# xd009642/xd-tts

Measured on AMD Instinct MI355X. Metric: mel-frames/s per GPU, 120-phoneme utterance (Tacotron2 decoder+postnet + 60-iter Griffin-Lim), end-to-end, higher is better.
Workload: dtype f32

## Files before the change

### include/xdtts.h

```cpp
#ifndef XDTTS_H
#define XDTTS_H

#include <stddef.h>
#include <stdint.h>

#ifdef __cplusplus
extern "C" {
#endif

typedef int32_t xdtts_status;
enum {
  XDTTS_OK = 0,
  XDTTS_ERR_BAD_ARG = 1,
  XDTTS_ERR_IO = 2,
  XDTTS_ERR_HIP = 3,
  XDTTS_ERR_OOM = 4,
  XDTTS_ERR_TOO_LONG = 5,
  XDTTS_ERR_NO_DEVICE = 6
};

typedef struct xdtts_tacotron2 xdtts_tacotron2;
typedef struct xdtts_griffinlim xdtts_griffinlim;

typedef struct {
  float gate_threshold;
  int32_t max_steps;
  int32_t fixed_steps;
  int32_t dropout_mode;
  uint32_t dropout_seed;
  int32_t max_chunk;
  uint32_t item_base;
  float fixed_frames_per_id;
  const uint8_t *dropout_masks;
  int32_t dropout_mask_steps;
} xdtts_infer_opts;

void xdtts_infer_opts_default(xdtts_infer_opts *opts);


xdtts_status xdtts_tacotron2_load(const char *dir, int32_t device_id, xdtts_tacotron2 **out);

#define XDTTS_DEVICE_DEFAULT (-1)
int32_t xdtts_default_device(void);

xdtts_status xdtts_model_dir_read(const char *dir, float *blob, size_t n_floats);

xdtts_status xdtts_model_dir_describe(const char *dir, char *buf, size_t cap, size_t *needed);

xdtts_status xdtts_tacotron2_load_synthetic(uint32_t seed, float rec_scale, int32_t device_id,
                                            xdtts_tacotron2 **out);

xdtts_status xdtts_tacotron2_load_blob(const float *blob, size_t n_floats, int32_t device_id,
                                       xdtts_tacotron2 **out);

xdtts_status xdtts_tacotron2_save(const xdtts_tacotron2 *h, const char *dir);

int32_t xdtts_tensor_count(void);
const char *xdtts_tensor_name(int32_t i);
int32_t xdtts_tensor_ndim(int32_t i);
int32_t xdtts_tensor_dim(int32_t i, int32_t d);
size_t xdtts_tensor_offset(int32_t i);
size_t xdtts_tensor_total(void);
xdtts_status xdtts_tacotron2_get_tensor(const xdtts_tacotron2 *h, int32_t i, float *out);

xdtts_status xdtts_tacotron2_infer_ids(xdtts_tacotron2 *h, const int64_t *ids, size_t n,
                                       const size_t *splits, size_t n_splits,
                                       const xdtts_infer_opts *opts, float **mel,
                                       size_t *n_frames);

xdtts_status xdtts_tacotron2_infer_batch(xdtts_tacotron2 *h, const int64_t *ids,
                                         const int32_t *lens, int32_t B, int32_t t_stride,
                                         const xdtts_infer_opts *opts,
                                         const int32_t *fixed_steps_per_item, float **mels,
                                         size_t *n_frames);

xdtts_status xdtts_tacotron2_encoder(xdtts_tacotron2 *h, const int64_t *ids, int32_t T,
                                     float *memory, float *processed_memory);
xdtts_status xdtts_tacotron2_decoder(xdtts_tacotron2 *h, const float *memory,
                                     const float *processed_memory, int32_t T, int32_t n_valid,
                                     const xdtts_infer_opts *opts, float *frames, float *gates,
                                     size_t *n_frames);
xdtts_status xdtts_tacotron2_decoder_step(xdtts_tacotron2 *h, const float *memory, const float *processed_memory,
                                          int32_t T, int32_t n_valid, const xdtts_infer_opts *opts, uint32_t step,
                                          const float *decoder_input, float *attention_hidden,
                                          float *attention_cell, float *decoder_hidden, float *decoder_cell,
                                          float *attention_weights, float *attention_weights_cum,
                                          float *attention_context, float *decoder_output,
                                          float *gate_prediction);

xdtts_status xdtts_tacotron2_decoder_steps(xdtts_tacotron2 *h, int32_t engine, int32_t B, const float *memory,
                                           const float *processed_memory, int32_t T, const int32_t *n_valid,
                                           const xdtts_infer_opts *opts, uint32_t step0, int32_t n_steps,
                                           const float *decoder_input, float *attention_hidden, float *attention_cell,
                                           float *decoder_hidden, float *decoder_cell, float *attention_weights,
                                           float *attention_weights_cum, float *attention_context, float *decoder_output,
                                           float *gate_prediction);

xdtts_status xdtts_tacotron2_engine_state(const xdtts_tacotron2 *h, int32_t *decoder_persistent,
                                          int32_t *encoder_cooperative, int32_t *batched_attention);
xdtts_status xdtts_tacotron2_engine_reset(xdtts_tacotron2 *h);
xdtts_status xdtts_tacotron2_small_batch_engine_state(const xdtts_tacotron2 *h, int32_t *state);

const char *xdtts_build_info(void);

xdtts_status xdtts_edge_floor_us(int32_t device_id, int32_t steps, int32_t T, int32_t tuned, double *us_per_step);

xdtts_status xdtts_tacotron2_postnet(xdtts_tacotron2 *h, const float *frames, int32_t F,
                                     float *mel_out);

xdtts_status xdtts_tacotron2_last_timings(const xdtts_tacotron2 *h, float ms[4], int32_t *steps);

void xdtts_tacotron2_free(xdtts_tacotron2 *h);


xdtts_status xdtts_mel_filter_bank(float sample_rate, size_t n_fft, size_t n_mels, float fmin,
                                   float fmax_or_nan, float *out);

xdtts_status xdtts_griffinlim_new(const float *mel_basis, size_t n_mels, size_t n_bins,
                                  size_t noverlap, float power, size_t iters, float momentum,
                                  int32_t device_id, xdtts_griffinlim **out);

typedef struct {
  int32_t nnls_iters;
  int32_t power_mode;
  int32_t mel_decompress;
  int32_t output_normalise;
  int32_t batch_shape;
  float rms_target;
} xdtts_griffinlim_opts;
void xdtts_griffinlim_opts_default(xdtts_griffinlim_opts *opts);
xdtts_status xdtts_griffinlim_set_opts(xdtts_griffinlim *g, const xdtts_griffinlim_opts *opts);
xdtts_status xdtts_griffinlim_get_opts(const xdtts_griffinlim *g, xdtts_griffinlim_opts *opts);

xdtts_status xdtts_griffinlim_set_seed(xdtts_griffinlim *g, uint32_t seed);

xdtts_status xdtts_griffinlim_infer(xdtts_griffinlim *g, const float *mel, size_t n_mels,
                                    size_t n_frames, float **audio, size_t *n_samples);

xdtts_status xdtts_griffinlim_infer_batch(xdtts_griffinlim *g, const float *const *mels, size_t n_mels,
                                          const size_t *n_frames, int32_t n_utt, float **audios,
                                          size_t *n_samples);

xdtts_status xdtts_griffinlim_infer_linear(xdtts_griffinlim *g, const float *S,
                                           const float *phase0, size_t n_frames, size_t iters,
                                           float **audio, size_t *n_samples);

xdtts_status xdtts_griffinlim_mel_to_linear(xdtts_griffinlim *g, const float *mel,
                                            size_t n_mels, size_t n_frames, float *S_out);

xdtts_status xdtts_griffinlim_step(xdtts_griffinlim *g, const float *S, float *angles,
                                   float *rebuilt, size_t n_frames, size_t n_iter);

xdtts_status xdtts_griffinlim_last_timings(const xdtts_griffinlim *g, float ms[3]);

void xdtts_griffinlim_free(xdtts_griffinlim *g);

xdtts_status xdtts_synthesize_ids(xdtts_tacotron2 *h, xdtts_griffinlim *g, const int64_t *ids,
                                  size_t n, const size_t *splits, size_t n_splits,
                                  const xdtts_infer_opts *opts, float **mel, size_t *n_frames,
                                  float **audio, size_t *n_samples);

xdtts_status xdtts_synthesize_batch(xdtts_tacotron2 *h, xdtts_griffinlim *g, const int64_t *ids,
                                    const int32_t *lens, int32_t B, int32_t t_stride,
                                    const int32_t *utt_chunks, int32_t n_utt,
                                    const xdtts_infer_opts *opts,
                                    const int32_t *fixed_steps_per_item, float **mels,
                                    size_t *n_frames, float **audios, size_t *n_samples);

xdtts_status xdtts_synthesize_sequence(xdtts_tacotron2 *h, xdtts_griffinlim *g, const int64_t *const *ids,
                                       const size_t *n_ids, const size_t *const *splits, const size_t *n_splits,
                                       int32_t n_utt, const xdtts_infer_opts *opts, float **mels,
                                       size_t *n_frames, float **audios, size_t *n_samples);

int32_t xdtts_symbol_count(void);
const char *xdtts_symbol_token(int32_t id);
int64_t xdtts_unit_id(const char *token, int32_t as_character);
int32_t xdtts_split_score(int64_t id);
xdtts_status xdtts_find_splits(const int64_t *ids, size_t n, size_t max_size, size_t *out,
                               size_t cap, size_t *n_out);

#define XDTTS_SAMPLE_RATE 22050
xdtts_status xdtts_audio_to_i16(const float *audio, size_t n, int16_t *pcm);
size_t xdtts_silence_samples(double seconds, uint32_t sample_rate);
size_t xdtts_silence_samples_duration(uint64_t secs, uint32_t nanos, uint32_t sample_rate);
xdtts_status xdtts_wav_write(const char *path, const int16_t *pcm, size_t n, uint32_t sample_rate);
xdtts_status xdtts_npy_write_f32(const char *path, const float *data, size_t rows, size_t cols);
double xdtts_real_time_factor(double compute_seconds, size_t n_samples);

void xdtts_free(void *p);
const char *xdtts_last_error(void);
int32_t xdtts_device_count(void);
xdtts_status xdtts_tacotron2_sync(xdtts_tacotron2 *h);

#ifdef __cplusplus
}
#endif
#endif
```

### xd-tts_amd/__init__.py

```python
import ctypes as C
import os

import numpy as np

_HERE = os.path.dirname(os.path.abspath(__file__))
LIB_PATH = os.environ.get("XDTTS_LIB") or os.path.join(_HERE, "libxdtts_hip.so")

N_MEL = 80
EMB = 512
ATT_DIM = 128

STATUS = {0: "OK", 1: "BAD_ARG", 2: "IO", 3: "HIP", 4: "OOM", 5: "TOO_LONG", 6: "NO_DEVICE"}
XDTTS_ERR_BAD_ARG, XDTTS_ERR_IO, XDTTS_ERR_HIP, XDTTS_ERR_OOM, XDTTS_ERR_TOO_LONG, XDTTS_ERR_NO_DEVICE = 1, 2, 3, 4, 5, 6


class XdttsError(RuntimeError):

    def __init__(self, status, message):
        super().__init__("xdtts status %d (%s): %s" % (status, STATUS.get(status, "?"), message))
        self.status = status


class GriffinLimOpts(C.Structure):

    _fields_ = [("nnls_iters", C.c_int32), ("power_mode", C.c_int32), ("mel_decompress", C.c_int32), ("output_normalise", C.c_int32), ("batch_shape", C.c_int32), ("rms_target", C.c_float)]


class InferOpts(C.Structure):
    _fields_ = [
        ("gate_threshold", C.c_float),
        ("max_steps", C.c_int32),
        ("fixed_steps", C.c_int32),
        ("dropout_mode", C.c_int32),
        ("dropout_seed", C.c_uint32),
        ("max_chunk", C.c_int32),
        ("item_base", C.c_uint32),
        ("fixed_frames_per_id", C.c_float),
        ("dropout_masks", C.c_void_p),
        ("dropout_mask_steps", C.c_int32),
    ]


_VP, _I32, _U32, _SZ, _F = C.c_void_p, C.c_int32, C.c_uint32, C.c_size_t, C.c_float
_PF = C.POINTER(C.c_float)
SYMBOLS = {
    "xdtts_infer_opts_default": (None, [C.POINTER(InferOpts)]),
    "xdtts_tacotron2_load": (_I32, [C.c_char_p, _I32, C.POINTER(_VP)]),
    "xdtts_model_dir_read": (_I32, [C.c_char_p, _VP, _SZ]),
    "xdtts_model_dir_describe": (_I32, [C.c_char_p, C.c_char_p, _SZ, C.POINTER(_SZ)]),
    "xdtts_tacotron2_load_synthetic": (_I32, [_U32, _F, _I32, C.POINTER(_VP)]),
    "xdtts_tacotron2_load_blob": (_I32, [_VP, _SZ, _I32, C.POINTER(_VP)]),
    "xdtts_tacotron2_save": (_I32, [_VP, C.c_char_p]),
    "xdtts_tensor_count": (_I32, []),
    "xdtts_tensor_name": (C.c_char_p, [_I32]),
    "xdtts_tensor_ndim": (_I32, [_I32]),
    "xdtts_tensor_dim": (_I32, [_I32, _I32]),
    "xdtts_tensor_offset": (_SZ, [_I32]),
    "xdtts_tensor_total": (_SZ, []),
    "xdtts_tacotron2_get_tensor": (_I32, [_VP, _I32, _VP]),
    "xdtts_tacotron2_infer_ids": (_I32, [_VP, _VP, _SZ, _VP, _SZ, C.POINTER(InferOpts), C.POINTER(_PF), C.POINTER(_SZ)]),
    "xdtts_tacotron2_infer_batch": (_I32, [_VP, _VP, _VP, _I32, _I32, C.POINTER(InferOpts), _VP, C.POINTER(_PF), C.POINTER(_SZ)]),
    "xdtts_tacotron2_encoder": (_I32, [_VP, _VP, _I32, _VP, _VP]),
    "xdtts_tacotron2_decoder": (_I32, [_VP, _VP, _VP, _I32, _I32, C.POINTER(InferOpts), _VP, _VP, C.POINTER(_SZ)]),
    "xdtts_tacotron2_decoder_step": (_I32, [_VP, _VP, _VP, _I32, _I32, C.POINTER(InferOpts), _U32] + [_VP] * 10),
    "xdtts_tacotron2_decoder_steps": (_I32, [_VP, _I32, _I32, _VP, _VP, _I32, _VP, C.POINTER(InferOpts), _U32, _I32] + [_VP] * 10),
    "xdtts_tacotron2_engine_state": (_I32, [_VP, C.POINTER(_I32), C.POINTER(_I32), C.POINTER(_I32)]),
    "xdtts_tacotron2_small_batch_engine_state": (_I32, [_VP, C.POINTER(_I32)]),
    "xdtts_tacotron2_engine_reset": (_I32, [_VP]),
    "xdtts_tacotron2_postnet": (_I32, [_VP, _VP, _I32, _VP]),
    "xdtts_tacotron2_last_timings": (_I32, [_VP, C.POINTER(C.c_float * 4), C.POINTER(_I32)]),
    "xdtts_tacotron2_free": (None, [_VP]),
    "xdtts_tacotron2_sync": (_I32, [_VP]),
    "xdtts_mel_filter_bank": (_I32, [_F, _SZ, _SZ, _F, _F, _VP]),
    "xdtts_griffinlim_new": (_I32, [_VP, _SZ, _SZ, _SZ, _F, _SZ, _F, _I32, C.POINTER(_VP)]),
    "xdtts_griffinlim_opts_default": (None, [_VP]),
    "xdtts_griffinlim_set_opts": (_I32, [_VP, _VP]),
    "xdtts_griffinlim_get_opts": (_I32, [_VP, _VP]),
    "xdtts_griffinlim_set_seed": (_I32, [_VP, _U32]),
    "xdtts_griffinlim_infer": (_I32, [_VP, _VP, _SZ, _SZ, C.POINTER(_PF), C.POINTER(_SZ)]),
    "xdtts_griffinlim_infer_batch": (_I32, [_VP, _VP, _SZ, _VP, _I32, _VP, _VP]),
    "xdtts_griffinlim_infer_linear": (_I32, [_VP, _VP, _VP, _SZ, _SZ, C.POINTER(_PF), C.POINTER(_SZ)]),
    "xdtts_griffinlim_mel_to_linear": (_I32, [_VP, _VP, _SZ, _SZ, _VP]),
    "xdtts_griffinlim_step": (_I32, [_VP, _VP, _VP, _VP, _SZ, _SZ]),
    "xdtts_griffinlim_last_timings": (_I32, [_VP, C.POINTER(C.c_float * 3)]),
    "xdtts_griffinlim_free": (None, [_VP]),
    "xdtts_synthesize_ids": (_I32, [_VP, _VP, _VP, _SZ, _VP, _SZ, C.POINTER(InferOpts), C.POINTER(_PF), C.POINTER(_SZ), C.POINTER(_PF), C.POINTER(_SZ)]),
    "xdtts_synthesize_batch": (_I32, [_VP, _VP, _VP, _VP, _I32, _I32, _VP, _I32, C.POINTER(InferOpts), _VP, _VP, _VP, _VP, _VP]),
    "xdtts_synthesize_sequence": (_I32, [_VP, _VP, _VP, _VP, _VP, _VP, _I32, C.POINTER(InferOpts), _VP, _VP, _VP, _VP]),
    "xdtts_symbol_count": (_I32, []),
    "xdtts_symbol_token": (C.c_char_p, [_I32]),
    "xdtts_unit_id": (C.c_int64, [C.c_char_p, _I32]),
    "xdtts_split_score": (_I32, [C.c_int64]),
    "xdtts_find_splits": (_I32, [_VP, _SZ, _SZ, _VP, _SZ, C.POINTER(_SZ)]),
    "xdtts_audio_to_i16": (_I32, [_VP, _SZ, _VP]),
    "xdtts_build_info": (C.c_char_p, []),
    "xdtts_edge_floor_us": (_I32, [C.c_int32, C.c_int32, C.c_int32, C.c_int32, C.POINTER(C.c_double)]),
    "xdtts_default_device": (C.c_int32, []),
    "xdtts_silence_samples": (_SZ, [C.c_double, _U32]),
    "xdtts_silence_samples_duration": (_SZ, [C.c_uint64, _U32, _U32]),
    "xdtts_wav_write": (_I32, [C.c_char_p, _VP, _SZ, _U32]),
    "xdtts_npy_write_f32": (_I32, [C.c_char_p, _VP, _SZ, _SZ]),
    "xdtts_real_time_factor": (C.c_double, [C.c_double, _SZ]),
    "xdtts_free": (None, [_VP]),
    "xdtts_last_error": (C.c_char_p, []),
    "xdtts_device_count": (_I32, []),
}


def _share_torch_hip_runtime():
    import importlib.util
    import sys

    if "torch" in sys.modules:
        return
    try:
        spec = importlib.util.find_spec("torch")
    except (ImportError, ValueError):
        spec = None
    if not spec or not spec.origin:
        return
    lib = os.path.join(os.path.dirname(spec.origin), "lib", "libamdhip64.so")
    if os.path.exists(lib):
        try:
            C.CDLL(lib, mode=C.RTLD_GLOBAL)
        except OSError:
            pass


def _load():
    _share_torch_hip_runtime()
    if not os.path.exists(LIB_PATH):
        raise ImportError(
            "%s not found: build it with `make -C %s` (or __graft_entry__.build()); there is no CPU fallback" % (LIB_PATH, _HERE)
        )
    lib = C.CDLL(LIB_PATH)
    for name, (res, args) in SYMBOLS.items():
        fn = getattr(lib, name)
        fn.restype = res
        fn.argtypes = args
    return lib


lib = _load()


def _check(status):
    if status != 0:
        raise XdttsError(status, lib.xdtts_last_error().decode("utf-8", "replace"))


def _ptr(a):
    return a.ctypes.data_as(C.c_void_p)


def default_opts(**kw):
    o = InferOpts()
    lib.xdtts_infer_opts_default(C.byref(o))
    masks = kw.pop("dropout_masks", None)
    for k, v in kw.items():
        setattr(o, k, v)
    if masks is not None:
        m = np.ascontiguousarray(masks, dtype=np.uint8)
        if m.ndim != 4 or m.shape[2:] != (2, 256):
            raise ValueError("dropout_masks must be (chunks, steps, 2, 256)")
        o._masks_keepalive = m
        o.dropout_masks = m.ctypes.data
        o.dropout_mask_steps = m.shape[1]
        o.dropout_mode = 2
    return o


def device_count():
    return lib.xdtts_device_count()


def tensor_table():
    out = []
    for i in range(lib.xdtts_tensor_count()):
        shape = tuple(lib.xdtts_tensor_dim(i, d) for d in range(lib.xdtts_tensor_ndim(i)))
        out.append((lib.xdtts_tensor_name(i).decode(), shape, lib.xdtts_tensor_offset(i)))
    return out


def read_model_dir(path):
    blob = np.empty(lib.xdtts_tensor_total(), dtype=np.float32)
    _check(lib.xdtts_model_dir_read(os.fsencode(path), _ptr(blob), blob.size))
    return {n: blob[off : off + int(np.prod(shape))].reshape(shape) for n, shape, off in tensor_table()}


def describe_model_dir(path):
    need = C.c_size_t()
    _check(lib.xdtts_model_dir_describe(os.fsencode(path), None, 0, C.byref(need)))
    buf = C.create_string_buffer(need.value)
    _check(lib.xdtts_model_dir_describe(os.fsencode(path), buf, need.value, None))
    out = {}
    for line in buf.value.decode().splitlines():
        f, rest = line.split(": inputs ", 1)
        i, o = rest.split(" ; outputs ", 1)
        out[f] = ([x for x in i.split(",") if x], [x for x in o.split(",") if x])
    return out


class _Pinned:

    def __init__(self, addr):
        self.addr = addr

    def __del__(self):
        if self.addr and lib is not None:
            lib.xdtts_free(C.cast(self.addr, _PF))
            self.addr = None


def _take(ptr, n, shape):
    addr = C.cast(ptr, C.c_void_p).value
    if not n or not addr:
        if addr:
            lib.xdtts_free(ptr)
        return np.zeros(shape, dtype=np.float32)
    buf = (C.c_float * int(n)).from_address(addr)
    buf._owner = _Pinned(addr)
    return np.frombuffer(buf, dtype=np.float32).reshape(shape)


def generate_id_list():
    return [lib.xdtts_symbol_token(i).decode() for i in range(lib.xdtts_symbol_count())]


def unit_id(token, as_character=False):
    i = lib.xdtts_unit_id(token.encode(), 1 if as_character else 0)
    return None if i < 0 else int(i)


def units_to_ids(tokens, as_character=False):
    out = [unit_id(t, as_character) for t in tokens]
    return np.array([i for i in out if i is not None], dtype=np.int64)


SAMPLE_RATE = 22050


def build_info():
    return dict(kv.split("=", 1) for kv in lib.xdtts_build_info().decode().split(" ") if "=" in kv)


def source_hash():
    import glob
    import hashlib

    here = os.path.dirname(os.path.abspath(__file__))
    files = sorted(glob.glob(os.path.join(here, "csrc", "*")) + [os.path.join(here, "..", "include", "xdtts.h")],
                   key=lambda p: os.path.relpath(p, here))
    h = hashlib.sha256()
    for f in files:
        with open(f, "rb") as fh:
            h.update(fh.read())
    return h.hexdigest()


DEVICE_DEFAULT = -1


def default_device():
    v = lib.xdtts_default_device()
    if v < 0:
        raise XdttsError(2, lib.xdtts_last_error().decode())
    return int(v)


def edge_floor_us(device_id=0, steps=2000, T=100, tuned=True):
    us = C.c_double()
    _check(lib.xdtts_edge_floor_us(device_id, steps, T, 1 if tuned else 0, C.byref(us)))
    return us.value


def audio_to_i16(audio):
    a = np.ascontiguousarray(audio, dtype=np.float32).ravel()
    out = np.empty(a.size, dtype=np.int16)
    _check(lib.xdtts_audio_to_i16(_ptr(a), a.size, _ptr(out)))
    return out


def silence_samples(seconds, sample_rate=SAMPLE_RATE):
    return int(lib.xdtts_silence_samples(float(seconds), int(sample_rate)))


def silence_samples_duration(secs, nanos, sample_rate=SAMPLE_RATE):
    return int(lib.xdtts_silence_samples_duration(int(secs), int(nanos), int(sample_rate)))


def write_wav(path, audio, sample_rate=SAMPLE_RATE):
    pcm = np.ascontiguousarray(audio) if np.asarray(audio).dtype == np.int16 else audio_to_i16(audio)
    _check(lib.xdtts_wav_write(os.fsencode(path), _ptr(pcm), pcm.size, int(sample_rate)))


def write_mel_npy(path, mel):
    m = np.ascontiguousarray(mel, dtype=np.float32)
    _check(lib.xdtts_npy_write_f32(os.fsencode(path), _ptr(m), m.shape[0], m.shape[1]))


def real_time_factor(compute_seconds, n_samples):
    return float(lib.xdtts_real_time_factor(float(compute_seconds), int(n_samples)))


def find_splits(ids, max_size=100):
    ids = np.ascontiguousarray(ids, dtype=np.int64)
    out = np.empty(max(ids.size, 1) + 2, dtype=np.uintp)
    n = C.c_size_t()
    _check(lib.xdtts_find_splits(_ptr(ids), ids.size, max_size, _ptr(out), out.size, C.byref(n)))
    return out[: n.value].astype(np.int64)


class Tacotron2:

    def __init__(self, handle):
        self._h = handle

    @classmethod
    def load(cls, path, device_id=0):
        h = C.c_void_p()
        _check(lib.xdtts_tacotron2_load(os.fsencode(path), device_id, C.byref(h)))
        return cls(h)

    @classmethod
    def synthetic(cls, seed=20240327, rec_scale=1.0, device_id=0):
        h = C.c_void_p()
        _check(lib.xdtts_tacotron2_load_synthetic(seed, rec_scale, device_id, C.byref(h)))
        return cls(h)

    @classmethod
    def from_blob(cls, blob, device_id=0):
        blob = np.ascontiguousarray(blob, dtype=np.float32)
        h = C.c_void_p()
        _check(lib.xdtts_tacotron2_load_blob(_ptr(blob), blob.size, device_id, C.byref(h)))
        return cls(h)

    def close(self):
        if self._h:
            lib.xdtts_tacotron2_free(self._h)
            self._h = None

    def __del__(self):
        try:
            self.close()
        except Exception:
            pass

    def save(self, path):
        _check(lib.xdtts_tacotron2_save(self._h, os.fsencode(path)))

    def blob(self):
        out = np.zeros(lib.xdtts_tensor_total(), dtype=np.float32)
        for i, (_n, shape, off) in enumerate(tensor_table()):
            t = np.empty(shape, dtype=np.float32)
            _check(lib.xdtts_tacotron2_get_tensor(self._h, i, _ptr(t)))
            out[off : off + t.size] = t.ravel()
        return out

    def get_tensor(self, name):
        for i, (n, shape, _off) in enumerate(tensor_table()):
            if n == name:
                out = np.empty(shape, dtype=np.float32)
                _check(lib.xdtts_tacotron2_get_tensor(self._h, i, _ptr(out)))
                return out
        raise KeyError(name)

    def infer(self, ids, splits=None, opts=None):
        ids = np.ascontiguousarray(ids, dtype=np.int64)
        sp = None if splits is None else np.ascontiguousarray(splits, dtype=np.uintp)
        mel, nf = _PF(), C.c_size_t()
        _check(
            lib.xdtts_tacotron2_infer_ids(
                self._h, _ptr(ids), ids.size, None if sp is None else _ptr(sp), 0 if sp is None else sp.size, C.byref(opts) if opts else None, C.byref(mel), C.byref(nf)
            )
        )
        return _take(mel, N_MEL * nf.value, (N_MEL, nf.value))

    def infer_units(self, tokens, opts=None, as_character=False):
        ids = units_to_ids(tokens, as_character)
        window = opts.max_chunk if opts else 100
        return self.infer(ids, splits=find_splits(ids, window), opts=opts)

    def infer_batch(self, ids_list, opts=None, fixed_steps=None):
        B = len(ids_list)
        lens = np.array([len(x) for x in ids_list], dtype=np.int32)
        stride = int(lens.max()) if B else 1
        ids = np.zeros((B, stride), dtype=np.int64)
        for b, x in enumerate(ids_list):
            ids[b, : len(x)] = x
        fs = None if fixed_steps is None else np.ascontiguousarray(fixed_steps, dtype=np.int32)
        mels = (_PF * B)()
        nf = (C.c_size_t * B)()
        _check(lib.xdtts_tacotron2_infer_batch(self._h, _ptr(ids), _ptr(lens), B, stride, C.byref(opts) if opts else None, None if fs is None else _ptr(fs), mels, nf))
        return [_take(mels[b], N_MEL * nf[b], (N_MEL, nf[b])) for b in range(B)]

    def encoder(self, ids):
        ids = np.ascontiguousarray(ids, dtype=np.int64)
        T = ids.size
        memory = np.empty((T, EMB), dtype=np.float32)
        pmem = np.empty((T, ATT_DIM), dtype=np.float32)
        _check(lib.xdtts_tacotron2_encoder(self._h, _ptr(ids), T, _ptr(memory), _ptr(pmem)))
        return memory, pmem

    def decoder(self, memory, pmem, n_valid, opts=None):
        memory = np.ascontiguousarray(memory, dtype=np.float32)
        pmem = np.ascontiguousarray(pmem, dtype=np.float32)
        o = opts if opts else default_opts()
        frames = np.empty((o.max_steps, N_MEL), dtype=np.float32)
        gates = np.empty(o.max_steps, dtype=np.float32)
        nf = C.c_size_t()
        _check(lib.xdtts_tacotron2_decoder(self._h, _ptr(memory), _ptr(pmem), memory.shape[0], n_valid, C.byref(o), _ptr(frames), _ptr(gates), C.byref(nf)))
        return frames[: nf.value].copy(), gates[: nf.value].copy()

    def decoder_step(self, memory, pmem, n_valid, state, decoder_input, step, opts=None):
        memory = np.ascontiguousarray(memory, dtype=np.float32)
        pmem = np.ascontiguousarray(pmem, dtype=np.float32)
        names = ("attention_hidden", "attention_cell", "decoder_hidden", "decoder_cell", "attention_weights", "attention_weights_cum", "attention_context")
        st = {k: np.array(state[k], dtype=np.float32, order="C") for k in names}
        din = np.ascontiguousarray(decoder_input, dtype=np.float32)
        out, gate = np.empty(N_MEL, dtype=np.float32), np.empty(1, dtype=np.float32)
        _check(lib.xdtts_tacotron2_decoder_step(self._h, _ptr(memory), _ptr(pmem), memory.shape[0], n_valid, C.byref(opts) if opts else None, step,
                                                _ptr(din), *[_ptr(st[k]) for k in names], _ptr(out), _ptr(gate)))
        return out, float(gate[0]), st

    ENGINES = {"launch": 0, "persistent": 1, "batched": 2, "persistent8": 3}

    def decoder_steps(self, engine, memory, pmem, n_valid, states, decoder_input, step0, n_steps=1, opts=None):
        memory = np.ascontiguousarray(memory, dtype=np.float32)
        pmem = np.ascontiguousarray(pmem, dtype=np.float32)
        B, T = memory.shape[0], memory.shape[1]
        nv = np.ascontiguousarray(n_valid, dtype=np.int32)
        names = ("attention_hidden", "attention_cell", "decoder_hidden", "decoder_cell", "attention_weights", "attention_weights_cum", "attention_context")
        st = {k: np.array(states[k], dtype=np.float32, order="C") for k in names}
        din = np.ascontiguousarray(decoder_input, dtype=np.float32)
        out, gate = np.empty((B, n_steps, N_MEL), dtype=np.float32), np.empty((B, n_steps), dtype=np.float32)
        _check(lib.xdtts_tacotron2_decoder_steps(self._h, self.ENGINES[engine], B, _ptr(memory), _ptr(pmem), T, _ptr(nv), C.byref(opts) if opts else None,
                                                 step0, n_steps, _ptr(din), *[_ptr(st[k]) for k in names], _ptr(out), _ptr(gate)))
        return out, gate, st

    def engine_state(self):
        a, b, c = C.c_int32(), C.c_int32(), C.c_int32()
        _check(lib.xdtts_tacotron2_engine_state(self._h, C.byref(a), C.byref(b), C.byref(c)))
        e = C.c_int32()
        _check(lib.xdtts_tacotron2_small_batch_engine_state(self._h, C.byref(e)))
        return {"decoder_persistent": a.value, "encoder_cooperative": b.value, "batched_attention": c.value, "decoder_persistent8": e.value}

    def engine_reset(self):
        _check(lib.xdtts_tacotron2_engine_reset(self._h))

    def postnet(self, frames):
        frames = np.ascontiguousarray(frames, dtype=np.float32)
        F = frames.shape[0]
        out = np.empty((N_MEL, F), dtype=np.float32)
        _check(lib.xdtts_tacotron2_postnet(self._h, _ptr(frames), F, _ptr(out)))
        return out

    def last_timings(self):
        ms = (C.c_float * 4)()
        steps = C.c_int32()
        _check(lib.xdtts_tacotron2_last_timings(self._h, C.byref(ms), C.byref(steps)))
        return {"encoder_ms": ms[0], "decoder_ms": ms[1], "postnet_ms": ms[2], "total_ms": ms[3], "steps": steps.value}


def create_mel_filter_bank(sample_rate, n_fft, n_mels, fmin, fmax=None):
    out = np.empty((n_mels, n_fft // 2 + 1), dtype=np.float32)
    _check(lib.xdtts_mel_filter_bank(sample_rate, n_fft, n_mels, fmin, float("nan") if fmax is None else fmax, _ptr(out)))
    return out


class GriffinLim:

    def __init__(self, mel_basis, noverlap, power, iters, momentum, device_id=0, seed=0):
        basis = np.ascontiguousarray(mel_basis, dtype=np.float32)
        self._h = C.c_void_p()
        _check(lib.xdtts_griffinlim_new(_ptr(basis), basis.shape[0], basis.shape[1], noverlap, power, iters, momentum, device_id, C.byref(self._h)))
        self.n_bins = basis.shape[1]
        self.set_seed(seed)

    def set_seed(self, seed):
        _check(lib.xdtts_griffinlim_set_seed(self._h, seed))

    def set_opts(self, **kw):
        o = self.get_opts()
        for k, v in kw.items():
            setattr(o, k, v)
        _check(lib.xdtts_griffinlim_set_opts(self._h, C.byref(o)))

    def get_opts(self):
        o = GriffinLimOpts()
        _check(lib.xdtts_griffinlim_get_opts(self._h, C.byref(o)))
        return o

    def close(self):
        if self._h:
            lib.xdtts_griffinlim_free(self._h)
            self._h = None

    def __del__(self):
        try:
            self.close()
        except Exception:
            pass

    def infer(self, mel):
        mel = np.ascontiguousarray(mel, dtype=np.float32)
        audio, n = _PF(), C.c_size_t()
        _check(lib.xdtts_griffinlim_infer(self._h, _ptr(mel), mel.shape[0], mel.shape[1], C.byref(audio), C.byref(n)))
        return _take(audio, n.value, (n.value,))

    def infer_batch(self, mels):
        ms = [np.ascontiguousarray(m, dtype=np.float32) for m in mels]
        n = len(ms)
        ptrs = (C.c_void_p * n)(*[m.ctypes.data for m in ms])
        nf = (C.c_size_t * n)(*[m.shape[1] for m in ms])
        audios = (_PF * n)()
        ns = (C.c_size_t * n)()
        _check(lib.xdtts_griffinlim_infer_batch(self._h, ptrs, ms[0].shape[0], nf, n, audios, ns))
        return [_take(audios[u], ns[u], (ns[u],)) for u in range(n)]

    def infer_linear(self, S, phase0=None, iters=0):
        S = np.ascontiguousarray(S, dtype=np.float32)
        p0 = None if phase0 is None else np.ascontiguousarray(phase0, dtype=np.float32)
        audio, n = _PF(), C.c_size_t()
        _check(lib.xdtts_griffinlim_infer_linear(self._h, _ptr(S), None if p0 is None else _ptr(p0), S.shape[1], iters, C.byref(audio), C.byref(n)))
        return _take(audio, n.value, (n.value,))

    def step(self, S, angles, rebuilt, n_iter=1):
        S = np.ascontiguousarray(S, dtype=np.float32)
        a = np.array(angles, dtype=np.float32, order="C")
        r = np.array(rebuilt, dtype=np.float32, order="C")
        _check(lib.xdtts_griffinlim_step(self._h, _ptr(S), _ptr(a), _ptr(r), S.shape[1], n_iter))
        return a, r

    def mel_to_linear(self, mel):
        mel = np.ascontiguousarray(mel, dtype=np.float32)
        S = np.empty((self.n_bins, mel.shape[1]), dtype=np.float32)
        _check(lib.xdtts_griffinlim_mel_to_linear(self._h, _ptr(mel), mel.shape[0], mel.shape[1], _ptr(S)))
        return S

    def last_timings(self):
        ms = (C.c_float * 3)()
        _check(lib.xdtts_griffinlim_last_timings(self._h, C.byref(ms)))
        return {"mel_to_linear_ms": ms[0], "iterations_ms": ms[1], "total_ms": ms[2]}


def create_griffin_lim(device_id=0, iters=30, seed=0):
    mel_basis = create_mel_filter_bank(22050.0, 1024, 80, 0.0, 8000.0)
    return GriffinLim(mel_basis, 1024 - 256, 1.7, iters, 0.99, device_id=device_id, seed=seed)


def synthesize(tacotron2, vocoder, ids, splits=None, opts=None):
    ids = np.ascontiguousarray(ids, dtype=np.int64)
    sp = None if splits is None else np.ascontiguousarray(splits, dtype=np.uintp)
    mel, nf, audio, ns = _PF(), C.c_size_t(), _PF(), C.c_size_t()
    _check(
        lib.xdtts_synthesize_ids(
            tacotron2._h, vocoder._h, _ptr(ids), ids.size, None if sp is None else _ptr(sp), 0 if sp is None else sp.size, C.byref(opts) if opts else None, C.byref(mel), C.byref(nf), C.byref(audio), C.byref(ns)
        )
    )
    return _take(mel, N_MEL * nf.value, (N_MEL, nf.value)), _take(audio, ns.value, (ns.value,))


def synthesize_batch(tacotron2, vocoder, utterance_chunks, opts=None, fixed_steps=None, want_mels=True):
    chunks = [c for u in utterance_chunks for c in u]
    B, n_utt = len(chunks), len(utterance_chunks)
    lens = np.array([len(x) for x in chunks], dtype=np.int32)
    stride = int(lens.max()) if B else 1
    ids = np.zeros((B, stride), dtype=np.int64)
    for b, x in enumerate(chunks):
        ids[b, : len(x)] = x
    uc = np.array([len(u) for u in utterance_chunks], dtype=np.int32)
    fs = None if fixed_steps is None else np.ascontiguousarray([s for u in fixed_steps for s in u], dtype=np.int32)
    mels = (_PF * n_utt)() if want_mels else None
    audios = (_PF * n_utt)()
    nf, ns = (C.c_size_t * n_utt)(), (C.c_size_t * n_utt)()
    _check(
        lib.xdtts_synthesize_batch(
            tacotron2._h, vocoder._h, _ptr(ids), _ptr(lens), B, stride, _ptr(uc), n_utt, C.byref(opts) if opts else None, None if fs is None else _ptr(fs), mels, nf, audios, ns
        )
    )
    out_m = [_take(mels[u], N_MEL * nf[u], (N_MEL, nf[u])) for u in range(n_utt)] if want_mels else None
    return out_m, [_take(audios[u], ns[u], (ns[u],)) for u in range(n_utt)]


def synthesize_sequence(tacotron2, vocoder, ids_list, splits_list=None, opts=None, want_mels=True):
    n = len(ids_list)
    idv = [np.ascontiguousarray(x, dtype=np.int64) for x in ids_list]
    spv = [None if (splits_list is None or splits_list[u] is None) else np.ascontiguousarray(splits_list[u], dtype=np.uintp) for u in range(n)]
    ids_p = (C.c_void_p * n)(*[x.ctypes.data for x in idv])
    n_ids = (C.c_size_t * n)(*[x.size for x in idv])
    sp_p = (C.c_void_p * n)(*[(None if s is None else s.ctypes.data) for s in spv])
    n_sp = (C.c_size_t * n)(*[(0 if s is None else s.size) for s in spv])
    mels = (_PF * n)() if want_mels else None
    audios = (_PF * n)()
    nf, ns = (C.c_size_t * n)(), (C.c_size_t * n)()
    _check(lib.xdtts_synthesize_sequence(tacotron2._h, vocoder._h, ids_p, n_ids, sp_p, n_sp, n, C.byref(opts) if opts else None, mels, nf, audios, ns))
    out_m = [_take(mels[u], N_MEL * nf[u], (N_MEL, nf[u])) for u in range(n)] if want_mels else None
    return out_m, [_take(audios[u], ns[u], (ns[u],)) for u in range(n)]
```

### xd-tts_amd/csrc/api_tacotron2.cpp

```cpp
#include <algorithm>
#include <cmath>
#include <memory>

#include "tacotron2_handle.h"

#include "edge_floor.hip"

using namespace xdtts;

extern "C" {

void xdtts_infer_opts_default(xdtts_infer_opts *o) {
  if (!o) return;
  o->gate_threshold = 0.6f;
  o->max_steps = 1000;
  o->fixed_steps = 0;
  o->dropout_mode = 1;
  o->dropout_seed = 0;
  o->max_chunk = 100;
  o->item_base = 0;
  o->fixed_frames_per_id = 0.f;
  o->dropout_masks = nullptr;
  o->dropout_mask_steps = 0;
}

const char *xdtts_last_error(void) { return last_error(); }

int32_t xdtts_device_count(void) {
  int n = 0;
  if (hipGetDeviceCount(&n) != hipSuccess) return 0;
  return n;
}

void xdtts_free(void *p) {
  if (p) pinned_release(p);
}

int32_t xdtts_tensor_count(void) { return (int32_t)tensor_table().size(); }
const char *xdtts_tensor_name(int32_t i) {
  return i >= 0 && i < xdtts_tensor_count() ? tensor_table()[i].name : nullptr;
}
int32_t xdtts_tensor_ndim(int32_t i) { return i >= 0 && i < xdtts_tensor_count() ? tensor_table()[i].ndim : 0; }
int32_t xdtts_tensor_dim(int32_t i, int32_t d) {
  return i >= 0 && i < xdtts_tensor_count() && d >= 0 && d < 3 ? tensor_table()[i].dims[d] : 0;
}
size_t xdtts_tensor_offset(int32_t i) { return i >= 0 && i < xdtts_tensor_count() ? tensor_table()[i].offset : 0; }
size_t xdtts_tensor_total(void) { return tensor_total(); }

static xdtts_status make_handle(std::vector<float> &&blob, int32_t device_id, xdtts_tacotron2 **out) {
  return guard([&] {
    if (!out) fail(XDTTS_ERR_BAD_ARG, "out handle pointer is null");
    *out = nullptr;
    auto h = std::make_unique<xdtts_tacotron2>();
    h->blob = std::move(blob);
    h->init(device_id);
    *out = h.release();
  });
}

xdtts_status xdtts_tacotron2_load(const char *dir, int32_t device_id, xdtts_tacotron2 **out) {
  std::vector<float> blob;
  xdtts_status st = guard([&] {
    if (!dir) fail(XDTTS_ERR_BAD_ARG, "dir is null");
    device_id = select_device(device_id);
    load_model_dir(dir, blob);
  });
  if (st != XDTTS_OK) return st;
  return make_handle(std::move(blob), device_id, out);
}

int32_t xdtts_default_device(void) {
  int32_t v = 0;
  return guard([&] { v = default_device(); }) == XDTTS_OK ? v : -1;
}

xdtts_status xdtts_model_dir_read(const char *dir, float *blob, size_t n_floats) {
  return guard([&] {
    if (!dir || !blob) fail(XDTTS_ERR_BAD_ARG, "null argument");
    if (n_floats != tensor_total()) fail(XDTTS_ERR_BAD_ARG, "blob has %zu floats, expected %zu", n_floats, tensor_total());
    std::vector<float> v;
    load_model_dir(dir, v);
    std::memcpy(blob, v.data(), v.size() * sizeof(float));
  });
}

xdtts_status xdtts_model_dir_describe(const char *dir, char *buf, size_t cap, size_t *needed) {
  return guard([&] {
    if (!dir || (!buf && cap)) fail(XDTTS_ERR_BAD_ARG, "null argument");
    const std::string d = describe_onnx_dir(dir);
    if (needed) *needed = d.size() + 1;
    if (cap) {
      const size_t n = std::min(cap - 1, d.size());
      std::memcpy(buf, d.data(), n);
      buf[n] = 0;
    }
  });
}

xdtts_status xdtts_tacotron2_load_synthetic(uint32_t seed, float rec_scale, int32_t device_id,
                                            xdtts_tacotron2 **out) {
  std::vector<float> blob;
  xdtts_status st = guard([&] {
    device_id = select_device(device_id);
    synthetic_blob(seed, rec_scale, blob);
  });
  if (st != XDTTS_OK) return st;
  return make_handle(std::move(blob), device_id, out);
}

xdtts_status xdtts_tacotron2_load_blob(const float *blob, size_t n_floats, int32_t device_id,
                                       xdtts_tacotron2 **out) {
  std::vector<float> v;
  xdtts_status st = guard([&] {
    if (!blob) fail(XDTTS_ERR_BAD_ARG, "blob is null");
    if (n_floats != tensor_total()) fail(XDTTS_ERR_BAD_ARG, "blob has %zu floats, expected %zu", n_floats, tensor_total());
    device_id = select_device(device_id);
    v.assign(blob, blob + n_floats);
  });
  if (st != XDTTS_OK) return st;
  return make_handle(std::move(v), device_id, out);
}

xdtts_status xdtts_tacotron2_save(const xdtts_tacotron2 *h, const char *dir) {
  return guard([&] {
    if (!h || !dir) fail(XDTTS_ERR_BAD_ARG, "null argument");
    save_container(dir, h->blob);
  });
}

xdtts_status xdtts_tacotron2_get_tensor(const xdtts_tacotron2 *h, int32_t i, float *out) {
  return guard([&] {
    if (!h || !out || i < 0 || i >= xdtts_tensor_count()) fail(XDTTS_ERR_BAD_ARG, "bad tensor request");
    const TensorInfo &t = tensor_table()[i];
    std::memcpy(out, h->blob.data() + t.offset, t.numel * sizeof(float));
  });
}

void xdtts_tacotron2_free(xdtts_tacotron2 *h) {
  if (!h) return;
  (void)hipSetDevice(h->device);
  if (h->stream) (void)hipStreamSynchronize(h->stream);
  delete h;
}

xdtts_status xdtts_tacotron2_sync(xdtts_tacotron2 *h) {
  return guard([&] {
    if (!h) fail(XDTTS_ERR_BAD_ARG, "null handle");
    HIP_CHECK(hipStreamSynchronize(h->stream));
  });
}

xdtts_status xdtts_tacotron2_infer_ids(xdtts_tacotron2 *h, const int64_t *ids, size_t n, const size_t *splits,
                                       size_t n_splits, const xdtts_infer_opts *opts, float **mel,
                                       size_t *n_frames) {
  return guard([&] {
    if (!h || !mel || !n_frames) fail(XDTTS_ERR_BAD_ARG, "null argument");
    *mel = nullptr;
    *n_frames = 0;
    std::lock_guard<std::mutex> lk(h->mu);
    const xdtts_infer_opts o = resolve_opts(opts);
    std::vector<int64_t> padded;
    std::vector<int> lens;
    chunks_from_splits(ids, n, splits, n_splits, o.max_chunk, padded, lens);
    int total = 0;
    h->infer_batch_device(padded.data(), lens.data(), (int)lens.size(), o.max_chunk, o, nullptr, &total);
    PinnedGuard host((size_t)N_MEL * total);
    HIP_CHECK(hipMemcpyAsync(host.p, h->mel_dev.p, (size_t)N_MEL * total * sizeof(float), hipMemcpyDeviceToHost, h->stream));
    h->finish_timings();
    *mel = host.release();
    *n_frames = (size_t)total;
  });
}

xdtts_status xdtts_tacotron2_infer_batch(xdtts_tacotron2 *h, const int64_t *ids, const int32_t *lens, int32_t B,
                                         int32_t t_stride, const xdtts_infer_opts *opts,
                                         const int32_t *fixed_steps_per_item, float **mels, size_t *n_frames) {
  return guard([&] {
    if (!h || !ids || !lens || !mels || !n_frames) fail(XDTTS_ERR_BAD_ARG, "null argument");
    std::lock_guard<std::mutex> lk(h->mu);
    const xdtts_infer_opts o = resolve_opts(opts);
    if (B <= 0) fail(XDTTS_ERR_BAD_ARG, "batch %d out of range", B);
    for (int b = 0; b < B; ++b) mels[b] = nullptr;
    const int T = o.max_chunk;
    if (t_stride <= 0) fail(XDTTS_ERR_BAD_ARG, "t_stride must be positive");
    const std::vector<int64_t> padded = pad_batch_ids(ids, lens, B, t_stride, T);
    int total = 0;
    std::vector<int> F = h->infer_batch_device(padded.data(), lens, B, T, o, fixed_steps_per_item, &total, true);
    PinnedSlab slab((size_t)N_MEL * total);
    Drain drain(h->stream);
    HIP_CHECK(hipMemcpyAsync(slab.base, h->mel_dev.p, (size_t)N_MEL * total * sizeof(float), hipMemcpyDeviceToHost, h->stream));
    h->finish_timings();
    size_t off = 0;
    for (int b = 0; b < B; ++b) {
      mels[b] = slab.piece(off);
      n_frames[b] = (size_t)F[b];
      off += (size_t)N_MEL * F[b];
    }
    slab.hand_over();
  });
}

xdtts_status xdtts_tacotron2_encoder(xdtts_tacotron2 *h, const int64_t *ids, int32_t T, float *memory,
                                     float *processed_memory) {
  return guard([&] {
    if (!h || !ids || !memory || !processed_memory) fail(XDTTS_ERR_BAD_ARG, "null argument");
    if (T <= 0 || T > T_MAX) fail(XDTTS_ERR_BAD_ARG, "T %d out of range", T);
    for (int t = 0; t < T; ++t)
      if (ids[t] < 0 || ids[t] >= N_SYMBOLS) fail(XDTTS_ERR_BAD_ARG, "id out of range");
    std::lock_guard<std::mutex> lk(h->mu);
    HIP_CHECK(hipSetDevice(h->device));
    h->ids.upload(ids, T, h->stream);
    std::lock_guard<ChipLock> chip(chip_mutex(h->device));
    h->run_encoder(1, T);
    HIP_CHECK(hipMemcpyAsync(memory, h->memory.p, (size_t)T * EMB * sizeof(float), hipMemcpyDeviceToHost, h->stream));
    HIP_CHECK(hipMemcpyAsync(processed_memory, h->pmem.p, (size_t)T * ATT_DIM * sizeof(float), hipMemcpyDeviceToHost, h->stream));
    HIP_CHECK(hipStreamSynchronize(h->stream));
    h->check_encoder_exchange();
  });
}

xdtts_status xdtts_tacotron2_decoder(xdtts_tacotron2 *h, const float *memory, const float *processed_memory,
                                     int32_t T, int32_t n_valid, const xdtts_infer_opts *opts, float *frames,
                                     float *gates, size_t *n_frames) {
  return guard([&] {
    if (!h || !memory || !processed_memory || !frames || !n_frames) fail(XDTTS_ERR_BAD_ARG, "null argument");
    if (T <= 0 || T > T_MAX || n_valid <= 0 || n_valid > T) fail(XDTTS_ERR_BAD_ARG, "bad T/n_valid");
    std::lock_guard<std::mutex> lk(h->mu);
    HIP_CHECK(hipSetDevice(h->device));
    const xdtts_infer_opts o = resolve_opts(opts);
    h->memory.upload(memory, (size_t)T * EMB, h->stream);
    h->pmem.upload(processed_memory, (size_t)T * ATT_DIM, h->stream);
    int nv = n_valid;
    h->n_valid.upload(&nv, 1, h->stream);
    HIP_CHECK(hipStreamSynchronize(h->stream));
    std::vector<int> lim(1, std::min(o.fixed_steps > 0 ? o.fixed_steps : o.max_steps, o.max_steps));
    h->upload_dropout_masks(o, 1, lim.data());
    DecoderBufs d = h->decoder_bufs(1, T, h->memory.p, h->pmem.p, o);
    HIP_CHECK(hipEventRecord(h->ev.e[0], h->stream));
    HIP_CHECK(hipEventRecord(h->ev.e[1], h->stream));
    h->last_steps = h->run_decoder(d, lim);
    HIP_CHECK(hipEventRecord(h->ev.e[2], h->stream));
    HIP_CHECK(hipEventRecord(h->ev.e[3], h->stream));
    const int F = h->host_ctl[xdtts_tacotron2::HOST_NF];
    HIP_CHECK(hipMemcpyAsync(frames, d.frames, (size_t)F * N_MEL * sizeof(float), hipMemcpyDeviceToHost, h->stream));
    if (gates) HIP_CHECK(hipMemcpyAsync(gates, d.gates, (size_t)F * sizeof(float), hipMemcpyDeviceToHost, h->stream));
    h->finish_timings();
    *n_frames = (size_t)F;
  });
}

xdtts_status xdtts_tacotron2_decoder_steps(xdtts_tacotron2 *h, int32_t engine, int32_t B, const float *memory, const float *processed_memory,
                                           int32_t T, const int32_t *n_valid, const xdtts_infer_opts *opts, uint32_t step0, int32_t n_steps,
                                           const float *decoder_input, float *attention_hidden, float *attention_cell, float *decoder_hidden,
                                           float *decoder_cell, float *attention_weights, float *attention_weights_cum, float *attention_context,
                                           float *decoder_output, float *gate_prediction) {
  return guard([&] {
    if (!h || !memory || !processed_memory || !n_valid || !decoder_input || !attention_hidden || !attention_cell || !decoder_hidden ||
        !decoder_cell || !attention_weights || !attention_weights_cum || !attention_context || !decoder_output || !gate_prediction)
      fail(XDTTS_ERR_BAD_ARG, "null argument");
    if (engine < 0 || engine > 3)
      fail(XDTTS_ERR_BAD_ARG, "engine %d out of range (0 launch-per-stage, 1 persistent, 2 batched MFMA, 3 persistent MFMA)", engine);
    if (engine == 3 && (B > P8_B_MAX || T > PERSIST_T_MAX))
      fail(XDTTS_ERR_BAD_ARG, "the persistent MFMA engine takes at most %d chunks of at most %d encoder steps", P8_B_MAX, PERSIST_T_MAX);
    if (B <= 0 || B > 64) fail(XDTTS_ERR_BAD_ARG, "batch %d out of range (1..64)", B);
    if (T <= 0 || T > T_MAX) fail(XDTTS_ERR_BAD_ARG, "T %d out of range", T);
    if (n_steps <= 0 || n_steps > 100000 || (uint64_t)step0 + (uint64_t)n_steps > (1u << 30)) fail(XDTTS_ERR_BAD_ARG, "bad step range");
    for (int b = 0; b < B; ++b)
      if (n_valid[b] <= 0 || n_valid[b] > T) fail(XDTTS_ERR_BAD_ARG, "chunk %d: bad n_valid %d", b, n_valid[b]);
    if (engine == 1 && (B > PERSIST_B_MAX || T > PERSIST_T_MAX))
      fail(XDTTS_ERR_BAD_ARG, "the persistent engine takes at most %d chunks of at most %d encoder steps", PERSIST_B_MAX, PERSIST_T_MAX);
    if (engine == 1) {
      for (int b = 0; b < B; ++b)
        for (int j = 0; j < EMB; ++j) {
          double c = 0;
          for (int t = 0; t < T; ++t) c += (double)attention_weights[(size_t)b * T + t] * memory[((size_t)b * T + t) * EMB + j];
          if (std::fabs(c - attention_context[(size_t)b * EMB + j]) > 1e-4 + 1e-4 * std::fabs(c))
            fail(XDTTS_ERR_BAD_ARG, "engine 1 needs attention_context = attention_weights . memory (chunk %d, column %d: %g vs %g)", b, j,
                 (double)attention_context[(size_t)b * EMB + j], c);
        }
    }
    std::lock_guard<std::mutex> lk(h->mu);
    HIP_CHECK(hipSetDevice(h->device));
    xdtts_infer_opts o = resolve_opts(opts);
    const int end = (int)step0 + n_steps;
    o.max_steps = end + 1;
    hipStream_t st = h->stream;
    h->memory.upload(memory, (size_t)B * T * EMB, st);
    h->pmem.upload(processed_memory, (size_t)B * T * ATT_DIM, st);
    h->n_valid.upload(n_valid, B, st);
    std::vector<int> lim((size_t)B, end);
    h->upload_dropout_masks(o, B, lim.data());
    if (engine == 2) h->w.ensure_batched_layout(h->blob, st);
    DecoderBufs d = h->decoder_bufs(B, T, h->memory.p, h->pmem.p, o, engine == 2 ? 1 : 0);
    d.use_gate = 0;
    h->limits.upload(lim.data(), lim.size(), st);
    h->lim_on_dev = lim;
    launch_decoder_init(d, h->limits.p, st);
    h->dec_in_dev.upload(decoder_input, (size_t)B * N_MEL, st);
    const size_t nh = (size_t)B * ATT_RNN, nt = (size_t)B * T, nc = (size_t)B * EMB;
    h->state_stage.alloc(4 * nh + 2 * nt + nc);
    float *s_ah = h->state_stage.p, *s_ac = s_ah + nh, *s_dh = s_ac + nh, *s_dc = s_dh + nh, *s_aw = s_dc + nh, *s_awc = s_aw + nt, *s_ctx = s_awc + nt;
    auto up = [&](float *dst, const float *src, size_t n) { HIP_CHECK(hipMemcpyAsync(dst, src, n * sizeof(float), hipMemcpyHostToDevice, st)); };
    auto dd = [&](float *dst, const float *src, size_t n) { HIP_CHECK(hipMemcpyAsync(dst, src, n * sizeof(float), hipMemcpyDeviceToDevice, st)); };
    up(s_ah, attention_hidden, nh);
    up(s_ac, attention_cell, nh);
    up(s_dh, decoder_hidden, nh);
    up(s_dc, decoder_cell, nh);
    up(s_aw, attention_weights, nt);
    up(s_awc, attention_weights_cum, nt);
    up(s_ctx, attention_context, nc);
    const int s0 = (int)step0;
    HIP_CHECK(hipMemcpyAsync(d.ctl, &s0, sizeof(int), hipMemcpyHostToDevice, st));
    HIP_CHECK(hipStreamSynchronize(st));
    dd(d.aw, s_aw, nt);
    dd(d.awc, s_awc, nt);
    dd(d.ctx, s_ctx, nc);
    if (engine == 2) {
      launch_frag_convert(s_ah, d.att_hf[0], B, d.Bpad, ATT_RNN, 0, st);
      launch_frag_convert(s_dh, d.dec_hf[0], B, d.Bpad, DEC_RNN, 0, st);
      launch_frag_convert(s_ac, d.att_c, B, d.Bpad, ATT_RNN, 0, st);
      launch_frag_convert(s_dc, d.dec_c, B, d.Bpad, DEC_RNN, 0, st);
      launch_frag_convert(s_ctx, d.ctxf, B, d.Bpad, EMB, 0, st);
    } else {
      dd(d.att_h[0], s_ah, nh);
      dd(d.att_c, s_ac, nh);
      dd(d.dec_h[0], s_dh, nh);
      dd(d.dec_c, s_dc, nh);
    }
    d.dec_in = h->dec_in_dev.p;
    int fin = 0;
    if (engine == 1) {
      if (!decoder_persistent_supported(h->device, PERSIST_B_MAX, PERSIST_T_MAX))
        fail(XDTTS_ERR_HIP, "persistent engine not available on this device (its 256-workgroup grid cannot be co-resident)");
      std::lock_guard<ChipLock> chip(chip_mutex(h->device));
      launch_decoder_prenet(d, h->w, st);
      d.dec_in = nullptr;
      h->dec_exchange.alloc(persist_granule_words(B));
      PersistBufs g = persist_bufs(h->dec_exchange.p, h->dec_err.p, B);
      launch_persist_seed_at(d, g, h->limits.p, s0, st);
      try {
        launch_decoder_persistent(d, h->w, g, n_steps, st);
      } catch (const CoopRefused &) {
        (void)hipStreamSynchronize(st);
        fail(XDTTS_ERR_HIP, "persistent engine not available on this device (cooperative launch refused)");
      }
      if (fetch_and_clear_error_word(h->dec_err.p, st)) fail(XDTTS_ERR_HIP, "persistent decoder exchange timed out (grid not co-resident)");
    } else if (engine == 3) {
      if (!decoder_p8_supported(h->device, B, PERSIST_T_MAX))
        fail(XDTTS_ERR_HIP, "persistent MFMA engine not available on this device (its 256-workgroup grid cannot be co-resident)");
      std::lock_guard<ChipLock> chip(chip_mutex(h->device));
      launch_decoder_prenet(d, h->w, st);
      d.dec_in = nullptr;
      h->dec_exchange.alloc(p8_exchange_words(B, n_steps));
      P8Bufs g = p8_bufs(h->dec_exchange.p, h->dec_err.p, B, n_steps);
      launch_p8_seed_at(d, g, h->limits.p, s0, st);
      try {
        launch_decoder_p8(d, h->w, g, n_steps, st);
      } catch (const CoopRefused &) {
        (void)hipStreamSynchronize(st);
        fail(XDTTS_ERR_HIP, "persistent MFMA engine not available on this device (cooperative launch refused)");
      }
      if (fetch_and_clear_error_word(h->dec_err.p, st)) fail(XDTTS_ERR_HIP, "persistent MFMA decoder exchange timed out (grid not co-resident)");
    } else {
      std::unique_lock<ChipLock> chip;
      if (d.hg) chip = std::unique_lock<ChipLock>(chip_mutex(h->device));
      if (engine == 0) launch_decoder_location(d, h->w, st);
      launch_decoder_early(d, h->w, 0, st);
      launch_decoder_prologue(d, h->w, st);
      for (int i = 0; i < n_steps; ++i) {
        launch_decoder_step_at(d, h->w, i, st);
        d.dec_in = nullptr;
      }
      launch_decoder_advance(d, n_steps, st);
      launch_decoder_flush(d, h->w, st);
      fin = n_steps & 1;
      if (d.ep_g && fetch_and_clear_error_word(h->dec_err.p, st)) fail(XDTTS_ERR_HIP, "batched attention exchange timed out (grid not co-resident)");
    }
    if (engine == 2) {
      launch_frag_convert(s_ah, d.att_hf[fin], B, d.Bpad, ATT_RNN, 1, st);
      launch_frag_convert(s_dh, d.dec_hf[fin], B, d.Bpad, DEC_RNN, 1, st);
      launch_frag_convert(s_ac, d.att_c, B, d.Bpad, ATT_RNN, 1, st);
      launch_frag_convert(s_dc, d.dec_c, B, d.Bpad, DEC_RNN, 1, st);
    }
    auto down = [&](float *dst, const float *src, size_t n) { HIP_CHECK(hipMemcpyAsync(dst, src, n * sizeof(float), hipMemcpyDeviceToHost, st)); };
    down(attention_hidden, engine == 2 ? s_ah : d.att_h[fin], nh);
    down(attention_cell, engine == 2 ? s_ac : d.att_c, nh);
    down(decoder_hidden, engine == 2 ? s_dh : d.dec_h[fin], nh);
    down(decoder_cell, engine == 2 ? s_dc : d.dec_c, nh);
    down(attention_weights, d.aw, nt);
    down(attention_weights_cum, engine == 2 && (n_steps & 1) ? d.awc2 : d.awc, nt);
    down(attention_context, d.ctx, nc);
    for (int b = 0; b < B; ++b) {
      down(decoder_output + (size_t)b * n_steps * N_MEL, d.frames + ((size_t)b * d.max_steps + step0) * N_MEL, (size_t)n_steps * N_MEL);
      down(gate_prediction + (size_t)b * n_steps, d.gates + (size_t)b * d.max_steps + step0, (size_t)n_steps);
    }
    HIP_CHECK(hipStreamSynchronize(st));
  });
}

xdtts_status xdtts_tacotron2_decoder_step(xdtts_tacotron2 *h, const float *memory, const float *processed_memory, int32_t T,
                                          int32_t n_valid, const xdtts_infer_opts *opts, uint32_t step, const float *decoder_input,
                                          float *attention_hidden, float *attention_cell, float *decoder_hidden, float *decoder_cell,
                                          float *attention_weights, float *attention_weights_cum, float *attention_context,
                                          float *decoder_output, float *gate_prediction) {
  return xdtts_tacotron2_decoder_steps(h, 0, 1, memory, processed_memory, T, &n_valid, opts, step, 1, decoder_input, attention_hidden,
                                       attention_cell, decoder_hidden, decoder_cell, attention_weights, attention_weights_cum,
                                       attention_context, decoder_output, gate_prediction);
}

xdtts_status xdtts_tacotron2_engine_state(const xdtts_tacotron2 *h, int32_t *decoder_persistent, int32_t *encoder_cooperative,
                                          int32_t *batched_attention) {
  return guard([&] {
    if (!h) fail(XDTTS_ERR_BAD_ARG, "null handle");
    std::lock_guard<std::mutex> lk(h->mu);
    if (decoder_persistent) *decoder_persistent = h->pair_gate.abi_state();
    if (encoder_cooperative) *encoder_cooperative = h->enc_gate.state != EngineGate::OFF ? 1 : 0;
    if (batched_attention) *batched_attention = h->att_fused();
  });
}

xdtts_status xdtts_tacotron2_small_batch_engine_state(const xdtts_tacotron2 *h, int32_t *state) {
  return guard([&] {
    if (!h || !state) fail(XDTTS_ERR_BAD_ARG, "null argument");
    std::lock_guard<std::mutex> lk(h->mu);
    *state = h->p8_gate.abi_state();
  });
}

xdtts_status xdtts_tacotron2_engine_reset(xdtts_tacotron2 *h) {
  return guard([&] {
    if (!h) fail(XDTTS_ERR_BAD_ARG, "null handle");
    std::lock_guard<std::mutex> lk(h->mu);
    h->pair_gate.reset();
    h->p8_gate.reset();
    h->enc_gate.reset();
    h->att_gate.reset();
    h->att_form = env::int_or(env::ATT_FUSED, 2);
  });
}

xdtts_status xdtts_edge_floor_us(int32_t device_id, int32_t steps, int32_t T, int32_t tuned, double *us_per_step) {
  return guard([&] {
    if (!us_per_step || steps < 1 || steps > 1000000 || T < 1 || T > 128) fail(XDTTS_ERR_BAD_ARG, "bad argument");
    device_id = select_device(device_id);
    std::lock_guard<ChipLock> chip(chip_mutex(device_id));
    const double us = xdtts_edge_floor::measure(device_id, steps, T, xdtts_edge_floor::kernel_delays(tuned ? 1 : 0), 5, false);
    if (us < 0) fail(XDTTS_ERR_HIP, "edge-floor skeleton: grid not co-resident on this device, or an exchange failed");
    *us_per_step = us;
  });
}

xdtts_status xdtts_tacotron2_postnet(xdtts_tacotron2 *h, const float *frames, int32_t F, float *mel_out) {
  return guard([&] {
    if (!h || !frames || !mel_out || F <= 0) fail(XDTTS_ERR_BAD_ARG, "bad argument");
    std::lock_guard<std::mutex> lk(h->mu);
    HIP_CHECK(hipSetDevice(h->device));
    h->frames.upload(frames, (size_t)F * N_MEL, h->stream);
    HIP_CHECK(hipStreamSynchronize(h->stream));
    h->mel_dev.alloc((size_t)N_MEL * F);
    const long zero = 0;
    h->run_postnet(h->frames.p, 0, &F, &zero, 1, h->mel_dev.p, F);
    HIP_CHECK(hipMemcpyAsync(mel_out, h->mel_dev.p, (size_t)N_MEL * F * sizeof(float), hipMemcpyDeviceToHost, h->stream));
    HIP_CHECK(hipStreamSynchronize(h->stream));
  });
}

xdtts_status xdtts_tacotron2_last_timings(const xdtts_tacotron2 *h, float ms[4], int32_t *steps) {
  return guard([&] {
    if (!h || !ms) fail(XDTTS_ERR_BAD_ARG, "null argument");
    for (int i = 0; i < 4; ++i) ms[i] = h->last_ms[i];
    if (steps) *steps = h->last_steps;
  });
}

}
```

### xd-tts_amd/csrc/decoder_persistent.hip

```cpp
#include <type_traits>

#include "device_utils.h"
#include "kernels.h"

namespace xdtts {

namespace {

typedef unsigned long long u64;

constexpr int PT = 512;
constexpr int NW = PT / 64;
constexpr int P_NCU = ATT_RNN / 4;
constexpr int TP = PERSIST_T_MAX;
constexpr int ATTN_CU = 8, PRE_CU = 16;
constexpr int EP_LD = TP, MEL_GL = 96;
#ifndef XDTTS_MEL_ST
#define XDTTS_MEL_ST 1
#endif
constexpr int MEL_ST = XDTTS_MEL_ST;
constexpr int GS = PERSIST_B_MAX;
constexpr unsigned P_SPIN_LIMIT = 1u << 21;
constexpr unsigned ACT_BIT = 0x80000000u;
constexpr int PERSIST_LAZY_DEFAULT = 9;

constexpr int WPAD = TP + 32;
static_assert(ATT_RNN == DEC_RNN && P_NCU == 256, "one workgroup per 4 + 4 hidden units");

__device__ __forceinline__ void publish(u64 *slot, unsigned tag, float v) {
  __hip_atomic_store(slot, ((u64)tag << 32) | (u64)__float_as_uint(v), __ATOMIC_RELAXED, __HIP_MEMORY_SCOPE_AGENT);
}
__device__ __forceinline__ u64 peek(const u64 *slot) {
  return __hip_atomic_load(slot, __ATOMIC_RELAXED, __HIP_MEMORY_SCOPE_AGENT);
}
struct PollCtl {
  int *err;
  unsigned limit;
};
__device__ __forceinline__ bool give_up(unsigned &spins, const PollCtl &pc) {
  if (++spins > pc.limit || ((spins & 127u) == 0 && __hip_atomic_load(pc.err, __ATOMIC_RELAXED, __HIP_MEMORY_SCOPE_AGENT))) {
    atomicExch(pc.err, 1);
    return true;
  }
  __builtin_amdgcn_s_sleep(1);
  return false;
}
template <int N, bool PRE = false>
__device__ __forceinline__ unsigned gather(const u64 *base, unsigned idx, unsigned stride, unsigned want,
                                           const bool (&need)[N], float (&out)[N], unsigned (&tag)[N], const PollCtl &err,
                                           const u64 *pre = nullptr) {
  bool done[N];
#pragma unroll
  for (int i = 0; i < N; ++i) {
    done[i] = !need[i];
    out[i] = 0.f;
    tag[i] = 0u;
  }
  if (PRE) {
    bool all = true;
#pragma unroll
    for (int i = 0; i < N; ++i)
      if (!done[i]) {
        const unsigned t = (unsigned)(pre[i] >> 32);
        if ((t & ~ACT_BIT) == want) {
          out[i] = __uint_as_float((unsigned)pre[i]);
          tag[i] = t;
          done[i] = true;
        } else {
          all = false;
        }
      }
    if (all) return 0u;
  }
  unsigned spins = 0;
  for (;;) {
    u64 v[N];
#pragma unroll
    for (int i = 0; i < N; ++i)
      if (!done[i]) v[i] = peek(base + (idx + (unsigned)i * stride));
    bool all = true;
#pragma unroll
    for (int i = 0; i < N; ++i)
      if (!done[i]) {
        const unsigned t = (unsigned)(v[i] >> 32);
        if ((t & ~ACT_BIT) == want) {
          out[i] = __uint_as_float((unsigned)v[i]);
          tag[i] = t;
          done[i] = true;
        } else {
          all = false;
        }
      }
    if (all || give_up(spins, err)) return spins;
  }
}

__device__ __forceinline__ void lazy_wait(int n) {
  for (int i = 0; i < n; ++i) __builtin_amdgcn_s_sleep(4);
}
__device__ __forceinline__ void straggle(bool me, int s, int at) {
  if (me && s % 6 == at)
    for (int i = 0; i < 2; ++i) __builtin_amdgcn_s_sleep(127);
}
__device__ __forceinline__ float4 lds4(const float *p) { return *reinterpret_cast<const float4 *>(p); }
__device__ __forceinline__ void chunk_fence() { asm volatile("" ::: "memory"); }
__device__ __forceinline__ unsigned opaque(unsigned v) {
  asm volatile("" : "+v"(v));
  return v;
}

constexpr int persist_lds_floats(int pb) {
  const int common = pb * (PRENET + TP + ATT_RNN + DEC_RNN + 16) + 8 + 32 + 16 * pb;
  const int attn = 2 * TP * 16 + 2 * TP + 16 + NW * 64 + 2 * WPAD + 62 * 16 + 64 + 16 + 8 * PT * 4;
  const int pre = N_MEL * PRENET + MEL_GL + 2 * PRENET + 8 + 6 * PT * 4;
  return common + (attn > pre ? attn : pre);
}

#ifdef XDTTS_PERSIST_PROFILE
#define PROF_MARK(i)                                       \
  do {                                                     \
    if (tid == 0) {                                        \
      const u64 now_ = wall_clock64();                     \
      s_prof[i] += now_ - prof_last;                       \
      prof_last = now_;                                    \
    }                                                      \
  } while (0)
#define PROF_POLLS(e, n)                                                   \
  do {                                                                     \
    const float m_ = wave_max((float)(n));                                 \
    if ((tid & 63) == 0) atomicAdd(&s_prof[16 + (e)], (u64)m_);            \
  } while (0)
#define PROF_WHEN(e)                                       \
  do {                                                     \
    if (tid == 0) s_prof[20 + (e)] += wall_clock64();      \
  } while (0)
#else
#define PROF_MARK(i) do { } while (0)
#define PROF_POLLS(e, n) do { (void)(n); } while (0)
#define PROF_WHEN(e) do { } while (0)
#endif

struct PersistWeights {
  const float4 *att_w, *dec_w, *q_w, *proj_w;
  const float *att_b, *dec_b, *v_w, *loc_fused, *proj_b, *pre0T, *pre1T;
};

template <int PB, bool SKEW = false, bool GATE = false>
__global__ __launch_bounds__(PT) void k_decoder_persistent(DecoderBufs d, PersistBufs g, PersistWeights w, int nsteps) {
  __shared__ __attribute__((aligned(16))) float smem[persist_lds_floats(PB)];
  const int c = blockIdx.x, tid = threadIdx.x, lane = tid & 63, wave = tid >> 6;
  const int T = d.T;
  const PollCtl pc{g.err, g.spins > 0 ? (unsigned)g.spins : P_SPIN_LIMIT};
  if (g.fault && c == g.fault - 1) return;
  const unsigned L4 = opaque(4u * (unsigned)lane);
  float *s_x = smem;
  float *s_e = s_x + PB * PRENET;
  float *s_hatt = s_e + PB * TP;
  float *s_hdec = s_hatt + PB * ATT_RNN;
  float *s_g = s_hdec + PB * DEC_RNN;
  int *s_act = reinterpret_cast<int *>(s_g + PB * 16);
  float *s_bias = s_g + PB * 16 + 8;
  float *s_cell = s_bias + 32;
  float *role = s_cell + 16 * PB;
  float *s_pm = role;
  float *s_loc = s_pm + TP * 16;
  float *s_aw = s_loc + TP * 16;
  float *s_awc = s_aw + TP;
  float *s_q = s_awc + TP;
  float *s_part = s_q + 16;
  float *s_wpad = s_part + NW * 64;
  float *s_G = s_wpad + 2 * WPAD;
  float *s_cown = s_G + 62 * 16;
  float *s_vv = s_cown + 64;
  float *s_qw = s_vv + 16;
  float *s_W0 = role;
  float *s_mel = s_W0 + N_MEL * PRENET;
  float *s_l1 = s_mel + MEL_GL;
  float *s_pb = s_l1 + 2 * PRENET;
  float *s_pw = s_pb + 8;

  float4 wa[2][ATT_COLS / 256], wd[2][DEC_COLS / 256];
#pragma unroll
  for (int r = 0; r < 2; ++r) {
    const int row = 16 * c + wave + NW * r;
#pragma unroll
    for (int k = 0; k < ATT_COLS / 256; ++k) wa[r][k] = ld_stream(w.att_w + (size_t)row * (ATT_COLS / 4) + lane + 64 * k);
#pragma unroll
    for (int k = 0; k < DEC_COLS / 256; ++k) wd[r][k] = ld_stream(w.dec_w + (size_t)row * (DEC_COLS / 4) + lane + 64 * k);
    if (lane == 0) {
      s_bias[wave + NW * r] = w.att_b[row];
      s_bias[16 + wave + NW * r] = w.dec_b[row];
    }
  }
  const bool attn = c < ATTN_CU * PB, pre = !attn && c < (ATTN_CU + PRE_CU) * PB;
  const int rb = attn ? c / ATTN_CU : (pre ? (c - ATTN_CU * PB) / PRE_CU : 0);
  const int rk = attn ? c % ATTN_CU : (c - ATTN_CU * PB) % PRE_CU;
  const int prow = rk + 16 * wave;
  const bool prow_ok = pre && wave < 6 && prow <= N_MEL;

  const int step0 = d.ctl[0];
  if (GATE && PB == 1 && !(step0 < d.nframes[0])) return;
  if (tid < PB) {
    s_act[tid] = 0;
    s_act[2 + tid] = step0 < d.nframes[tid];
  }
#pragma unroll
  for (int b = 0; b < PB; ++b) {
#pragma unroll
    for (int h = 0; h < 2; ++h) {
      s_hatt[b * ATT_RNN + tid + PT * h] = d.att_h[0][b * ATT_RNN + tid + PT * h];
      s_hdec[b * DEC_RNN + tid + PT * h] = d.dec_h[0][b * DEC_RNN + tid + PT * h];
    }
  }
  float wreg[PB][2];
  int nv[PB];
#pragma unroll
  for (int b = 0; b < PB; ++b) {
    wreg[b][0] = lane < T ? d.aw[b * T + lane] : 0.f;
    wreg[b][1] = lane + 64 < T ? d.aw[b * T + lane + 64] : 0.f;
    nv[b] = d.n_valid[b];
  }
  const int cb = tid >> 2, cu = tid & 3;
  const bool cell = tid < 4 * PB;
  if (cell) {
    s_cell[tid] = d.att_c[cb * ATT_RNN + 4 * c + cu];
    s_cell[4 * PB + tid] = d.dec_c[cb * DEC_RNN + 4 * c + cu];
    s_cell[8 * PB + tid] = d.att_h[0][cb * ATT_RNN + 4 * c + cu];
    s_cell[12 * PB + tid] = d.dec_h[0][cb * DEC_RNN + 4 * c + cu];
  }
  int nf_r = 0;
  if (attn) {
    for (int i = tid; i < TP * 16; i += PT) {
      const int t = i >> 4, dd = i & 15;
      s_pm[i] = t < T ? d.pmem[((size_t)rb * T + t) * ATT_DIM + 16 * rk + dd] : 0.f;
    }
    if (tid < TP) {
      s_aw[tid] = tid < T ? d.aw[rb * T + tid] : 0.f;
      s_awc[tid] = tid < T ? d.awc[rb * T + tid] : 0.f;
    }
    for (int i = tid; i < 62 * 16; i += PT) s_G[i] = w.loc_fused[(size_t)(i >> 4) * ATT_DIM + 16 * rk + (i & 15)];
    if (tid < 16) s_vv[tid] = w.v_w[16 * rk + tid];
#pragma unroll
    for (int r = 0; r < 2; ++r)
#pragma unroll
      for (int j = 0; j < 4; ++j)
        *reinterpret_cast<float4 *>(s_qw + 4 * ((4 * r + j) * PT + tid)) = w.q_w[(unsigned)((16 * rk + wave + NW * r) * (ATT_RNN / 4) + lane + 64 * j)];
  }
  if (pre) {
    for (int i = tid; i < N_MEL * PRENET; i += PT) s_W0[(((i / PRENET) >> 2) * PRENET + i % PRENET) * 4 + ((i / PRENET) & 3)] = w.pre0T[i];
    if (prow_ok) {
      if (lane == 0) s_pb[wave] = w.proj_b[prow];
#pragma unroll
      for (int j = 0; j < 6; ++j)
        *reinterpret_cast<float4 *>(s_pw + 4 * (j * PT + tid)) = w.proj_w[(unsigned)(prow * (PROJ_IN / 4) + lane + 64 * j)];
    }
    nf_r = d.nframes[rb];
  }
  constexpr bool ROLE_REGS = PB == 1;
  float rw[ROLE_REGS ? 40 : 1];
  if (ROLE_REGS) {
#pragma unroll
    for (int k = 0; k < 40; ++k) rw[ROLE_REGS ? k : 0] = 0.f;
    if (attn) {
#pragma unroll
      for (int r = 0; r < 2; ++r)
#pragma unroll
        for (int j = 0; j < 4; ++j) {
          const float4 q = w.q_w[(unsigned)((16 * rk + wave + NW * r) * (ATT_RNN / 4) + lane + 64 * j)];
          rw[ROLE_REGS ? 16 * r + 4 * j + 0 : 0] = q.x;
          rw[ROLE_REGS ? 16 * r + 4 * j + 1 : 0] = q.y;
          rw[ROLE_REGS ? 16 * r + 4 * j + 2 : 0] = q.z;
          rw[ROLE_REGS ? 16 * r + 4 * j + 3 : 0] = q.w;
        }
    } else if (pre) {
#pragma unroll
      for (int k = 0; k < N_MEL / 2; ++k) rw[ROLE_REGS ? k : 0] = w.pre0T[(unsigned)(((tid >> 8) * (N_MEL / 2) + k) * PRENET + (tid & 255))];
    }
  }
  float w1r[2][4];
#pragma unroll
  for (int r = 0; r < 2; ++r)
#pragma unroll
    for (int k = 0; k < 4; ++k) w1r[r][k] = pre ? w.pre1T[(unsigned)((lane + 64 * k) * PRENET + 16 * rk + wave + NW * r)] : 0.f;
  const uint32_t item = d.item_base + (uint32_t)rb;
  __syncthreads();

  float pma[PB][2][2], pmd[PB][2][2], pmp[2] = {0.f, 0.f};
  if (d.ctx_fold) {
#pragma unroll
    for (int b = 0; b < PB; ++b)
#pragma unroll
      for (int h = 0; h < 2; ++h) {
        const int t = lane + 64 * h;
        const float *F = d.ctx_fold + (size_t)b * CTXF_ROWS * CTXF_LD + t;
#pragma unroll
        for (int r = 0; r < 2; ++r) {
          const int row = 16 * c + wave + NW * r;
          pma[b][r][h] = t < T ? F[(size_t)row * CTXF_LD] : 0.f;
          pmd[b][r][h] = t < T ? F[(size_t)(4 * ATT_RNN + row) * CTXF_LD] : 0.f;
        }
        if (prow_ok && b == rb) pmp[h] = t < T ? F[(size_t)(4 * ATT_RNN + 4 * DEC_RNN + prow) * CTXF_LD] : 0.f;
      }
  } else {
    float4 pw4 = make_float4(0.f, 0.f, 0.f, 0.f), pw5 = pw4;
    if (prow_ok) {
      pw4 = lds4(s_pw + 4 * (4 * PT + tid));
      pw5 = lds4(s_pw + 4 * (5 * PT + tid));
    }
#pragma unroll
    for (int b = 0; b < PB; ++b) {
      const float4 *m4 = reinterpret_cast<const float4 *>(d.memory + (size_t)b * T * EMB);
#pragma unroll
      for (int h = 0; h < 2; ++h) {
        float ra[2] = {0.f, 0.f}, rd[2] = {0.f, 0.f}, rp = 0.f;
        for (int tt = 0; tt < 64 && tt + 64 * h < T; ++tt) {
          const int t = tt + 64 * h;
          const float4 m0 = m4[(size_t)t * (EMB / 4) + lane], m1 = m4[(size_t)t * (EMB / 4) + 64 + lane];
#pragma unroll
          for (int r = 0; r < 2; ++r) {
            const float va = wave_sum(dot4(wa[r][2], m1, dot4(wa[r][1], m0, 0.f)));
            const float vd = wave_sum(dot4(wd[r][5], m1, dot4(wd[r][4], m0, 0.f)));
            if (lane == tt) {
              ra[r] = va;
              rd[r] = vd;
            }
          }
          if (pre && b == rb) {
            const float vp = wave_sum(dot4(pw5, m1, dot4(pw4, m0, 0.f)));
            if (lane == tt) rp = vp;
          }
        }
#pragma unroll
        for (int r = 0; r < 2; ++r) {
          pma[b][r][h] = ra[r];
          pmd[b][r][h] = rd[r];
        }
        if (pre && b == rb) pmp[h] = rp;
      }
    }
  }

  float aacc[PB][2], dacc[PB][2];
  auto att_bulk = [&](unsigned L4, bool all) {
#pragma unroll
    for (int b = 0; b < PB; ++b) {
      if (!all && !s_act[b]) continue;
      const float w0 = wreg[b][0], w1 = wreg[b][1];
      float a0 = fmaf(pma[b][0][1], w1, pma[b][0][0] * w0), a1 = fmaf(pma[b][1][1], w1, pma[b][1][0] * w0);
#pragma unroll
      for (int k = 3; k < 7; ++k) {
        const float4 v = lds4(s_hatt + b * ATT_RNN + 256 * (k - 3) + L4);
        a0 = dot4(wa[0][k], v, a0);
        a1 = dot4(wa[1][k], v, a1);
      }
      aacc[b][0] = a0;
      aacc[b][1] = a1;
      chunk_fence();
    }
  };
  auto dec_bulk_h = [&](unsigned L4, bool all) {
#pragma unroll
    for (int b = 0; b < PB; ++b) {
      if (!all && !s_act[b]) continue;
      float a0 = 0.f, a1 = 0.f;
#pragma unroll
      for (int k = 6; k < 10; ++k) {
        const float4 v = lds4(s_hdec + b * DEC_RNN + 256 * (k - 6) + L4);
        a0 = dot4(wd[0][k], v, a0);
        a1 = dot4(wd[1][k], v, a1);
      }
      dacc[b][0] = a0;
      dacc[b][1] = a1;
      chunk_fence();
    }
  };
  auto location = [&](int tid) {
    typedef float f32x4 __attribute__((ext_vector_type(4)));
    for (int i = tid; i < 2 * WPAD; i += PT) {
      const int ch = i / WPAD, t = i % WPAD - (LOC_K - 1) / 2;
      s_wpad[i] = (t >= 0 && t < T) ? (ch ? s_awc[t] : s_aw[t]) : 0.f;
    }
    __syncthreads();
    {
      const unsigned l = (unsigned)tid & 63u, li = l & 15u, lg = l >> 4, t0 = 16u * ((unsigned)tid >> 6);
      float av[16], bv[16];
#pragma unroll
      for (int kk = 0; kk < 16; ++kk) {
        const unsigned q = 4u * kk + lg, qa = q < 2u * LOC_K ? q : 2u * LOC_K - 1u, ch = qa >= (unsigned)LOC_K ? 1u : 0u;
        av[kk] = s_wpad[ch * WPAD + t0 + li + (qa - ch * LOC_K)];
        bv[kk] = q < 2u * LOC_K ? s_G[qa * 16u + li] : 0.f;
      }
      f32x4 acc0 = (f32x4){0.f, 0.f, 0.f, 0.f}, acc1 = acc0;
#pragma unroll
      for (int kk = 0; kk < 16; kk += 2) {
        acc0 = __builtin_amdgcn_mfma_f32_16x16x4f32(av[kk], bv[kk], acc0, 0, 0, 0);
        acc1 = __builtin_amdgcn_mfma_f32_16x16x4f32(av[kk + 1], bv[kk + 1], acc1, 0, 0, 0);
      }
#pragma unroll
      for (int j = 0; j < 4; ++j) s_loc[(t0 + 4u * lg + j) * 16u + li] = acc0[j] + acc1[j];
    }
    __syncthreads();
  };
  att_bulk(L4, true);
  dec_bulk_h(L4, true);
  if (attn) location(tid);

#ifdef XDTTS_PERSIST_PROFILE
  __shared__ u64 s_prof[24];
  if (tid < 24) s_prof[tid] = 0;
  u64 prof_last = wall_clock64();
  __syncthreads();
#endif
  int s = step0;
  const int s_stop = step0 + nsteps;
  if constexpr (SKEW) {
    static_assert(PB == 2, "the skewed loop is the pair kernel");
    const int tid_k = tid;
    const bool lag = g.slow && c == g.slow - 1;
    unsigned drop1 = 0u, drop2 = 0u;
    u64 pf[2] = {0ull, 0ull};
    auto issue_x = [&](auto B, int s) {
      constexpr int b = decltype(B)::value;
      const int tid = tid_k + (int)opaque(0u);
      pf[0] = tid < 256 ? peek(g.x + (unsigned)(((s & 1) * GS + b) * PRENET + (tid & 255))) : 0ull;
      pf[1] = 0ull;
    };
    auto issue_h = [&](const u64 *base, auto B, int s) {
      constexpr int b = decltype(B)::value;
      const int tid = tid_k + (int)opaque(0u);
      pf[0] = peek(base + (unsigned)(((s & 1) * GS + b) * ATT_RNN + tid));
      pf[1] = peek(base + (unsigned)(((s & 1) * GS + b) * ATT_RNN + tid + PT));
    };
    auto issue_ep = [&](auto B, int s) {
      constexpr int b = decltype(B)::value;
      const int tid = tid_k + (int)opaque(0u), t = tid >> 2, j = tid & 3;
      pf[0] = t < T ? peek(g.ep + (unsigned)((((s & 1) * GS + b) * ATTN_CU + j) * EP_LD + t)) : 0ull;
      pf[1] = t < T ? peek(g.ep + (unsigned)((((s & 1) * GS + b) * ATTN_CU + j + 4) * EP_LD + t)) : 0ull;
    };
    auto issue_mel = [&](auto B, int s) {
      constexpr int b = decltype(B)::value;
      const int tid = tid_k + (int)opaque(0u);
      pf[0] = (pre && rb == b && tid < N_MEL + 1) ? peek(g.mel + (unsigned)((((s & 1) * GS + b) * MEL_GL + tid) * MEL_ST)) : 0ull;
      pf[1] = 0ull;
    };
    auto I0 = std::integral_constant<int, 0>{};
    auto I1 = std::integral_constant<int, 1>{};
    auto att_bulk1 = [&](auto B, unsigned L4) {
      constexpr int b = decltype(B)::value;
      const float w0 = wreg[b][0], w1 = wreg[b][1];
      float a0 = fmaf(pma[b][0][1], w1, pma[b][0][0] * w0), a1 = fmaf(pma[b][1][1], w1, pma[b][1][0] * w0);
#pragma unroll
      for (int k = 3; k < 7; ++k) {
        const float4 v = lds4(s_hatt + b * ATT_RNN + 256 * (k - 3) + L4);
        a0 = dot4(wa[0][k], v, a0);
        a1 = dot4(wa[1][k], v, a1);
      }
      aacc[b][0] = a0;
      aacc[b][1] = a1;
    };
    auto dec_bulk_h1 = [&](auto B, unsigned L4) {
      constexpr int b = decltype(B)::value;
      float a0 = 0.f, a1 = 0.f;
#pragma unroll
      for (int k = 6; k < 10; ++k) {
        const float4 v = lds4(s_hdec + b * DEC_RNN + 256 * (k - 6) + L4);
        a0 = dot4(wd[0][k], v, a0);
        a1 = dot4(wd[1][k], v, a1);
      }
      dacc[b][0] = a0;
      dacc[b][1] = a1;
    };
    auto ph1 = [&](auto B, int s, auto nxt) -> bool {
      constexpr int b = decltype(B)::value;
      const int tid = tid_k + (int)opaque(0u), lane = tid & 63, wave = tid >> 6;
      const unsigned L4 = 4u * (unsigned)lane;
      const int p = s & 1;
      const unsigned want = (unsigned)(s + 1);
      if (b == 0) straggle(lag, s, 0);
      {
        const int i = tid & 255;
        const bool need[1] = {tid < 256};
        float v[1];
        unsigned tg[1];
        gather<1, true>(g.x, (unsigned)((p * GS + b) * PRENET + i), 0u, want, need, v, tg, pc, pf);
        if (need[0]) {
          s_x[b * PRENET + i] = v[0];
          if (i == 0) s_act[b] = (tg[0] & ACT_BIT) ? 1 : 0;
        }
        if (tid == PT - 1) s_act[4] = __hip_atomic_load(g.err, __ATOMIC_RELAXED, __HIP_MEMORY_SCOPE_AGENT);
      }
      __syncthreads();
      const bool on = s_act[b] != 0 && s_act[4] == 0;
      if (!on) return false;
      {
        const float4 v = lds4(s_x + b * PRENET + L4);
        const float a0 = wave_sum(dot4(wa[0][0], v, aacc[b][0]));
        const float a1 = wave_sum(dot4(wa[1][0], v, aacc[b][1]));
        if (lane == 0) {
          s_g[b * 16 + wave] = a0 + s_bias[wave];
          s_g[b * 16 + wave + NW] = a1 + s_bias[wave + NW];
        }
      }
      __syncthreads();
      if (tid < 4 * PB && (tid >> 2) == b) {
        const int cu = tid & 3;
        const float *gp = s_g + b * 16 + 4 * cu;
        const float ig = fast_sigmoid(gp[0]), fg = fast_sigmoid(gp[1]), gg = fast_tanh(gp[2]), og = fast_sigmoid(gp[3]);
        const float cn = fmaf(fg, s_cell[tid], ig * gg), hn = og * fast_tanh(cn);
        publish(g.hatt + (unsigned)((p * GS + b) * ATT_RNN + 4 * c + cu), want, hn);
        s_cell[tid] = cn;
        s_cell[8 * PB + tid] = hn;
      }
      nxt();
      PROF_MARK(5 * b + 0);
      if (b == 0) straggle(lag, s, 1);
      __builtin_amdgcn_sched_barrier(0);
      return true;
    };
    auto ph2 = [&](auto B, int s, auto nxt) {
      constexpr int b = decltype(B)::value;
      const int tid = tid_k + (int)opaque(0u), lane = tid & 63, wave = tid >> 6;
      const unsigned L4 = 4u * (unsigned)lane, TID = (unsigned)tid;
      const int p = s & 1;
      const unsigned want = (unsigned)(s + 1);
      const bool mine = attn && rb == b;
      float4 lp4 = make_float4(0.f, 0.f, 0.f, 0.f), v4 = lp4;
      if (mine) {
        const float4 l4 = lds4(s_loc + 4 * TID), p4 = lds4(s_pm + 4 * TID);
        lp4 = make_float4(l4.x + p4.x, l4.y + p4.y, l4.z + p4.z, l4.w + p4.w);
        v4 = lds4(s_vv + 4 * (tid & 3));
      }
      {
        const bool need[2] = {true, true};
        float v[2];
        unsigned tg[2];
        gather<2, true>(g.hatt, (unsigned)((p * GS + b) * ATT_RNN + tid), PT, want, need, v, tg, pc, pf);
        s_hatt[b * ATT_RNN + TID] = v[0];
        s_hatt[b * ATT_RNN + TID + PT] = v[1];
      }
      __syncthreads();
      if (mine) {
        float q0 = 0.f, q1 = 0.f;
#pragma unroll
        for (int j = 0; j < 4; ++j) {
          const float4 v = lds4(s_hatt + b * ATT_RNN + 256 * j + L4);
          q0 = dot4(lds4(s_qw + 4 * (j * PT + TID)), v, q0);
          q1 = dot4(lds4(s_qw + 4 * ((4 + j) * PT + TID)), v, q1);
        }
        q0 = wave_sum(q0);
        q1 = wave_sum(q1);
        if (lane == 0) {
          s_q[wave] = q0;
          s_q[wave + NW] = q1;
        }
        __syncthreads();
        const int t = tid >> 2, dq = 4 * (tid & 3);
        const float4 q4 = lds4(s_q + dq);
        float e = v4.x * fast_tanh(q4.x + lp4.x);
        e = fmaf(v4.y, fast_tanh(q4.y + lp4.y), e);
        e = fmaf(v4.z, fast_tanh(q4.z + lp4.z), e);
        e = fmaf(v4.w, fast_tanh(q4.w + lp4.w), e);
        e += dpp_move<0xB1, 0xf>(0.f, e);
        e += dpp_move<0x4E, 0xf>(0.f, e);
        if ((tid & 3) == 0 && t < T) publish(g.ep + (unsigned)(((p * GS + b) * ATTN_CU + rk) * EP_LD + t), want, e);
      }
      {
        float a0 = dacc[b][0], a1 = dacc[b][1];
#pragma unroll
        for (int k = 0; k < 4; ++k) {
          const float4 v = lds4(s_hatt + b * ATT_RNN + 256 * k + L4);
          a0 = dot4(wd[0][k], v, a0);
          a1 = dot4(wd[1][k], v, a1);
        }
        dacc[b][0] = a0;
        dacc[b][1] = a1;
      }
      nxt();
      PROF_MARK(5 * b + 1);
      if (b == 0) straggle(lag, s, 2);
      __builtin_amdgcn_sched_barrier(0);
    };
    auto ph3 = [&](auto B, int s, auto nxt) {
      constexpr int b = decltype(B)::value;
      const int tid = tid_k + (int)opaque(0u), lane = tid & 63, wave = tid >> 6;
      const unsigned L4 = 4u * (unsigned)lane;
      const int p = s & 1;
      const unsigned want = (unsigned)(s + 1);
      const bool mine = attn && rb == b;
      {
        const int t = tid >> 2, j = tid & 3;
        const bool need[2] = {t < T, t < T};
        float v[2];
        unsigned tg[2];
        gather<2, true>(g.ep, (unsigned)(((p * GS + b) * ATTN_CU + j) * EP_LD + t), 4u * EP_LD, want, need, v, tg, pc, pf);
        float e = v[0] + v[1];
        e += dpp_move<0xB1, 0xf>(0.f, e);
        e += dpp_move<0x4E, 0xf>(0.f, e);
        if (j == 0) s_e[b * TP + t] = (t < T && t < nv[b]) ? e : -INFINITY;
      }
      __syncthreads();
      {
        const float e0 = s_e[b * TP + lane], e1 = s_e[b * TP + lane + 64];
        const float m = wave_max(fmaxf(e0, e1));
        const float x0 = fast_exp(e0 - m), x1 = fast_exp(e1 - m);
        const float rs = __builtin_amdgcn_rcpf(wave_sum(x0 + x1));
        wreg[b][0] = x0 * rs;
        wreg[b][1] = x1 * rs;
      }
      if (mine && wave == 0) {
        s_aw[lane] = wreg[b][0];
        s_awc[lane] += wreg[b][0];
        s_aw[lane + 64] = wreg[b][1];
        s_awc[lane + 64] += wreg[b][1];
      }
      if (b == 0) straggle(lag, s, 3);
      {
        const float w0 = wreg[b][0], w1 = wreg[b][1];
        float a0 = fmaf(pmd[b][0][1], w1, fmaf(pmd[b][0][0], w0, dacc[b][0]));
        float a1 = fmaf(pmd[b][1][1], w1, fmaf(pmd[b][1][0], w0, dacc[b][1]));
        a0 = wave_sum(a0);
        a1 = wave_sum(a1);
        if (lane == 0) {
          s_g[b * 16 + wave] = a0 + s_bias[16 + wave];
          s_g[b * 16 + wave + NW] = a1 + s_bias[16 + wave + NW];
        }
      }
      __syncthreads();
      if (tid < 4 * PB && (tid >> 2) == b) {
        const int cu = tid & 3;
        const float *gp = s_g + b * 16 + 4 * cu;
        const float ig = fast_sigmoid(gp[0]), fg = fast_sigmoid(gp[1]), gg = fast_tanh(gp[2]), og = fast_sigmoid(gp[3]);
        const float cn = fmaf(fg, s_cell[4 * PB + tid], ig * gg), hn = og * fast_tanh(cn);
        publish(g.hdec + (unsigned)((p * GS + b) * DEC_RNN + 4 * c + cu), want, hn);
        s_cell[4 * PB + tid] = cn;
        s_cell[12 * PB + tid] = hn;
      }
      att_bulk1(B, L4);
      nxt();
      PROF_MARK(5 * b + 2);
      if (b == 0) straggle(lag, s, 4);
      __builtin_amdgcn_sched_barrier(0);
    };
    auto ph4 = [&](auto B, int s, auto nxt) {
      constexpr int b = decltype(B)::value;
      const int tid = tid_k + (int)opaque(0u), lane = tid & 63, wave = tid >> 6;
      const unsigned L4 = 4u * (unsigned)lane, TID = (unsigned)tid;
      const int p = s & 1;
      const unsigned want = (unsigned)(s + 1);
      const bool mine = pre && rb == b;
      const int prow = rk + 16 * wave;
      const bool prow_ok = mine && wave < 6 && prow <= N_MEL;
      if (mine) {
        drop1 = 0u;
        drop2 = 0u;
        if (d.dropout_mode) {
#pragma unroll
          for (int k = 0; k < 4; ++k)
            drop1 |= (prenet_dropped(d.dropout_mode, d.dropout_seed, item, d.drop_masks, d.drop_steps, rb, s + 1, 0, lane + 64 * k) ? 1u : 0u) << k;
#pragma unroll
          for (int r = 0; r < 2; ++r)
            drop2 |= (prenet_dropped(d.dropout_mode, d.dropout_seed, item, d.drop_masks, d.drop_steps, rb, s + 1, 1, 16 * rk + wave + NW * r) ? 1u : 0u) << r;
        }
      }
      {
        const bool need[2] = {true, true};
        float v[2];
        unsigned tg[2];
        gather<2, true>(g.hdec, (unsigned)((p * GS + b) * DEC_RNN + tid), PT, want, need, v, tg, pc, pf);
        s_hdec[b * DEC_RNN + TID] = v[0];
        s_hdec[b * DEC_RNN + TID + PT] = v[1];
      }
      __syncthreads();
      if (prow_ok) {
        float a = 0.f;
#pragma unroll
        for (int j = 0; j < 4; ++j) a = dot4(lds4(s_pw + 4 * (j * PT + TID)), lds4(s_hdec + b * DEC_RNN + 256 * j + L4), a);
        a = fmaf(pmp[1], wreg[b][1], fmaf(pmp[0], wreg[b][0], a));
        a = wave_sum(a);
        if (lane == 0) publish(g.mel + (unsigned)(((p * GS + b) * MEL_GL + prow) * MEL_ST), want, a + s_pb[wave]);
      }
      dec_bulk_h1(B, L4);
      nxt();
      if (attn && rb == b) location(tid);
      PROF_MARK(5 * b + 3);
      if (b == 0) straggle(lag, s, 5);
      __builtin_amdgcn_sched_barrier(0);
    };
    auto ph5 = [&](auto B, int s, auto nxt) {
      constexpr int b = decltype(B)::value;
      if (!(pre && rb == b)) {
        nxt();
        return;
      }
      PROF_MARK(10 + 3 * b);
      const int tid = tid_k + (int)opaque(0u), lane = tid & 63, wave = tid >> 6;
      const unsigned L4 = 4u * (unsigned)lane, TID = (unsigned)tid;
      const int p = s & 1;
      const unsigned want = (unsigned)(s + 1);
      if (tid < N_MEL + 1) {
        const bool need[1] = {true};
        float v[1];
        unsigned tg[1];
        gather<1, true>(g.mel, (unsigned)(((p * GS + b) * MEL_GL + tid) * MEL_ST), 0, want, need, v, tg, pc, pf);
        s_mel[tid] = v[0];
      }
      __syncthreads();
      PROF_MARK(11 + 3 * b);
      const float gate = s_mel[N_MEL];
      const bool fired = GATE ? gate_fires(gate, d.gate_lo, d.gate_hi, d.gate_threshold) : (d.use_gate && gate_sigmoid(gate) > d.gate_threshold);
      if (rk == 0) {
        if (tid < N_MEL) d.frames[((size_t)b * d.max_steps + s) * N_MEL + tid] = s_mel[tid];
        if (tid == 0) {
          d.gates[(size_t)b * d.max_steps + s] = gate;
          if (fired) d.nframes[b] = s + 1;
        }
      }
      if (fired) nf_r = s + 1;
      const bool more = s + 1 < nf_r;
      float xo[2] = {0.f, 0.f};
      if (more) {
        const unsigned HM = (unsigned)((tid >> 8) * (N_MEL / 2));
        float acc = 0.f;
#pragma unroll
        for (int k = 0; k < N_MEL / 2; k += 4) {
          const float4 w4 = lds4(s_W0 + 4u * (((HM + k) >> 2) * PRENET + (TID & 255u))), m = lds4(s_mel + HM + k);
          acc = fmaf(w4.x, m.x, acc);
          acc = fmaf(w4.y, m.y, acc);
          acc = fmaf(w4.z, m.z, acc);
          acc = fmaf(w4.w, m.w, acc);
        }
        s_l1[TID] = acc;
        __syncthreads();
        float pk[4];
#pragma unroll
        for (int k = 0; k < 4; ++k) {
          const float v = fmaxf(s_l1[(L4 >> 2) + 64 * k] + s_l1[PRENET + (L4 >> 2) + 64 * k], 0.f);
          pk[k] = (drop1 >> k) & 1u ? 0.f : (d.dropout_mode ? 2.f * v : v);
        }
#pragma unroll
        for (int r = 0; r < 2; ++r) {
          float a = 0.f;
#pragma unroll
          for (int k = 0; k < 4; ++k) a = fmaf(w1r[r][k], pk[k], a);
          a = fmaxf(wave_sum(a), 0.f);
          xo[r] = (drop2 >> r) & 1u ? 0.f : (d.dropout_mode ? 2.f * a : a);
        }
      }
      if (lane < 2) s_mel[MEL_GL - 16 + wave + NW * lane] = lane ? xo[1] : xo[0];
      __syncthreads();
      if (tid < 16)
        publish(g.x + (unsigned)(((p ^ 1) * GS + b) * PRENET + 16 * rk + tid), (want + 1u) | (more ? ACT_BIT : 0u),
                s_mel[MEL_GL - 16 + tid]);
      nxt();
      PROF_MARK(5 * b + 4);
    };
    bool tail1 = false;
    if (s_act[2] != 0 && s_act[3] != 0) {
      issue_x(I0, s);
      for (;; ++s) {
        bool a0 = s < s_stop;
        if (a0) a0 = ph1(I0, s, [&] { if (tail1) issue_h(g.hdec, I1, s - 1); else issue_h(g.hatt, I0, s); });
        if (tail1) ph4(I1, s - 1, [&] { if (a0) issue_h(g.hatt, I0, s); });
        if (a0) ph2(I0, s, [&] { if (tail1) issue_mel(I1, s - 1); else issue_ep(I0, s); });
        if (tail1) {
          ph5(I1, s - 1, [&] { if (a0) issue_ep(I0, s); });
          tail1 = false;
        }
        if (!a0) break;
        ph3(I0, s, [&] { issue_x(I1, s); });
        const bool a1 = ph1(I1, s, [&] { issue_h(g.hdec, I0, s); });
        if (!a1) issue_h(g.hdec, I0, s);
        ph4(I0, s, [&] { if (a1) issue_h(g.hatt, I1, s); else issue_mel(I0, s); });
        if (a1) ph2(I1, s, [&] { issue_mel(I0, s); });
        ph5(I0, s, [&] { if (a1) issue_ep(I1, s); });
        if (!a1) {
          ++s;
          break;
        }
        ph3(I1, s, [&] { issue_x(I0, s + 1); });
        tail1 = true;
      }
    }
  } else
  for (; s < s_stop; ++s) {
    const int tid_it = tid + (int)opaque(0u);
    {
    const int tid = tid_it, lane = tid & 63, wave = tid >> 6;
    const unsigned L4 = 4u * (unsigned)lane, TID = (unsigned)tid;
    const int cb = tid >> 2, cu = tid & 3;
    const bool cell = tid < 4 * PB;
    const int prow = rk + 16 * wave;
    const bool prow_ok = pre && wave < 6 && prow <= N_MEL;
    const int p = s & 1;
    const unsigned want = (unsigned)(s + 1);
    const bool lag = g.slow && c == g.slow - 1;
    straggle(lag, s, 0);
    PROF_MARK(0);
    {
      const int b0 = tid >> 8, i = tid & 255;
      const bool need[2] = {b0 < PB && s_act[2 + (b0 < PB ? b0 : 0)] != 0, false};
      float v[2];
      unsigned tg[2];
      lazy_wait(pre ? g.xfirst : g.xlazy);
      const unsigned np_ = gather<2>(g.x, (unsigned)((p * GS + b0) * PRENET + i), 2u * PRENET, want, need, v, tg, pc);
      PROF_POLLS(0, np_);
#pragma unroll
      for (int j = 0; j < 2; ++j)
        if (need[j]) {
          s_x[(b0 + 2 * j) * PRENET + i] = v[j];
          if (i == 0) s_act[b0 + 2 * j] = (tg[j] & ACT_BIT) ? 1 : 0;
        }
      if (tid == PT - 1) s_act[4] = __hip_atomic_load(g.err, __ATOMIC_RELAXED, __HIP_MEMORY_SCOPE_AGENT);
    }
    __syncthreads();
    bool act[PB], any = false;
#pragma unroll
    for (int b = 0; b < PB; ++b) {
      act[b] = s_act[b] != 0;
      any = any || act[b];
    }
    if (tid < PB) s_act[2 + tid] = s_act[tid];
    PROF_MARK(1);
    PROF_WHEN(2);
    if (!any || s_act[4] != 0 || (PB == 2 && g.shrink && !(act[0] && act[1]))) break;
    const bool act_r = s_act[rb] != 0;
#pragma unroll
    for (int b = 0; b < PB; ++b)
      if (act[b]) {
        const float4 v = lds4(s_x + b * PRENET + L4);
        const float a0 = wave_sum(dot4(wa[0][0], v, aacc[b][0]));
        const float a1 = wave_sum(dot4(wa[1][0], v, aacc[b][1]));
        if (lane == 0) {
          s_g[b * 16 + wave] = a0 + s_bias[wave];
          s_g[b * 16 + wave + NW] = a1 + s_bias[wave + NW];
        }
      }
    __syncthreads();
    if (cell && s_act[cb]) {
      const float *gp = s_g + cb * 16 + 4 * cu;
      const float ig = fast_sigmoid(gp[0]), fg = fast_sigmoid(gp[1]), gg = fast_tanh(gp[2]), og = fast_sigmoid(gp[3]);
      const float cn = fmaf(fg, s_cell[tid], ig * gg), hn = og * fast_tanh(cn);
      publish(g.hatt + (unsigned)((p * GS + cb) * ATT_RNN + 4 * c + cu), want, hn);
      s_cell[tid] = cn;
      s_cell[8 * PB + tid] = hn;
    }
    PROF_MARK(2);
    PROF_WHEN(0);
    straggle(lag, s, 1);
    __builtin_amdgcn_sched_barrier(0);
    float4 lp4 = make_float4(0.f, 0.f, 0.f, 0.f), v4 = lp4;
    if (attn && act_r) {
      const float4 l4 = lds4(s_loc + 4 * TID), p4 = lds4(s_pm + 4 * TID);
      lp4 = make_float4(l4.x + p4.x, l4.y + p4.y, l4.z + p4.z, l4.w + p4.w);
      v4 = lds4(s_vv + 4 * (tid & 3));
    }
    {
      bool need[2 * PB];
#pragma unroll
      for (int i = 0; i < 2 * PB; ++i) need[i] = act[i >> 1];
      float v[2 * PB];
      unsigned tg[2 * PB];
      lazy_wait(attn ? g.first : g.lazy);
      const unsigned np_ = gather<2 * PB>(g.hatt, (unsigned)(p * GS * ATT_RNN + tid), PT, want, need, v, tg, pc);
      PROF_POLLS(1, np_);
#pragma unroll
      for (int i = 0; i < 2 * PB; ++i)
        if (need[i]) s_hatt[TID + PT * i] = v[i];
    }
    __syncthreads();
    PROF_MARK(3);
    if (attn && act_r) {
      float q0 = 0.f, q1 = 0.f;
#pragma unroll
      for (int j = 0; j < 4; ++j) {
        const float4 v = lds4(s_hatt + rb * ATT_RNN + 256 * j + L4);
        if (ROLE_REGS) {
          q0 = dot4(make_float4(rw[ROLE_REGS ? 4 * j : 0], rw[ROLE_REGS ? 4 * j + 1 : 0], rw[ROLE_REGS ? 4 * j + 2 : 0], rw[ROLE_REGS ? 4 * j + 3 : 0]), v, q0);
          q1 = dot4(make_float4(rw[ROLE_REGS ? 16 + 4 * j : 0], rw[ROLE_REGS ? 17 + 4 * j : 0], rw[ROLE_REGS ? 18 + 4 * j : 0], rw[ROLE_REGS ? 19 + 4 * j : 0]), v, q1);
        } else {
          q0 = dot4(lds4(s_qw + 4 * (j * PT + TID)), v, q0);
          q1 = dot4(lds4(s_qw + 4 * ((4 + j) * PT + TID)), v, q1);
        }
      }
      q0 = wave_sum(q0);
      q1 = wave_sum(q1);
      if (lane == 0) {
        s_q[wave] = q0;
        s_q[wave + NW] = q1;
      }
      __syncthreads();
      PROF_MARK(15);
      const int t = tid >> 2, dq = 4 * (tid & 3);
      const float4 q4 = lds4(s_q + dq);
      float e = v4.x * fast_tanh(q4.x + lp4.x);
      e = fmaf(v4.y, fast_tanh(q4.y + lp4.y), e);
      e = fmaf(v4.z, fast_tanh(q4.z + lp4.z), e);
      e = fmaf(v4.w, fast_tanh(q4.w + lp4.w), e);
      e += dpp_move<0xB1, 0xf>(0.f, e);
      e += dpp_move<0x4E, 0xf>(0.f, e);
      if ((tid & 3) == 0 && t < T) publish(g.ep + (unsigned)(((p * GS + rb) * ATTN_CU + rk) * EP_LD + t), want, e);
    }
#pragma unroll
    for (int b = 0; b < PB; ++b)
      if (act[b]) {
        float a0 = dacc[b][0], a1 = dacc[b][1];
#pragma unroll
        for (int k = 0; k < 4; ++k) {
          const float4 v = lds4(s_hatt + b * ATT_RNN + 256 * k + L4);
          a0 = dot4(wd[0][k], v, a0);
          a1 = dot4(wd[1][k], v, a1);
        }
        dacc[b][0] = a0;
        dacc[b][1] = a1;
        chunk_fence();
      }
    PROF_MARK(4);
    straggle(lag, s, 2);
    __builtin_amdgcn_sched_barrier(0);
    {
      const int t = tid >> 2, j = tid & 3;
      bool need[2 * PB];
#pragma unroll
      for (int i = 0; i < 2 * PB; ++i) need[i] = act[i >> 1] && t < T;
      float v[2 * PB];
      unsigned tg[2 * PB];
      lazy_wait(attn ? g.efirst : g.clazy);
      const unsigned np_ = gather<2 * PB>(g.ep, (unsigned)((p * GS * ATTN_CU + j) * EP_LD + t), 4u * EP_LD, want, need, v, tg, pc);
      PROF_POLLS(2, np_);
#pragma unroll
      for (int b = 0; b < PB; ++b) {
        float e = v[2 * b] + v[2 * b + 1];
        e += dpp_move<0xB1, 0xf>(0.f, e);
        e += dpp_move<0x4E, 0xf>(0.f, e);
        if (j == 0 && act[b]) s_e[b * TP + t] = (t < T && t < nv[b]) ? e : -INFINITY;
      }
    }
    __syncthreads();
    PROF_MARK(5);
    PROF_WHEN(3);
#pragma unroll
    for (int b = 0; b < PB; ++b)
      if (act[b]) {
        const float e0 = s_e[b * TP + lane], e1 = s_e[b * TP + lane + 64];
        const float m = wave_max(fmaxf(e0, e1));
        const float x0 = fast_exp(e0 - m), x1 = fast_exp(e1 - m);
        const float rs = __builtin_amdgcn_rcpf(wave_sum(x0 + x1));
        wreg[b][0] = x0 * rs;
        wreg[b][1] = x1 * rs;
      }
    if (attn && act_r && wave == 0) {
      s_aw[lane] = wreg[rb][0];
      s_awc[lane] += wreg[rb][0];
      s_aw[lane + 64] = wreg[rb][1];
      s_awc[lane + 64] += wreg[rb][1];
    }
    PROF_MARK(6);
    straggle(lag, s, 3);
    __builtin_amdgcn_sched_barrier(0);
#pragma unroll
    for (int b = 0; b < PB; ++b)
      if (act[b]) {
        const float w0 = wreg[b][0], w1 = wreg[b][1];
        float a0 = fmaf(pmd[b][0][1], w1, fmaf(pmd[b][0][0], w0, dacc[b][0]));
        float a1 = fmaf(pmd[b][1][1], w1, fmaf(pmd[b][1][0], w0, dacc[b][1]));
        a0 = wave_sum(a0);
        a1 = wave_sum(a1);
        if (lane == 0) {
          s_g[b * 16 + wave] = a0 + s_bias[16 + wave];
          s_g[b * 16 + wave + NW] = a1 + s_bias[16 + wave + NW];
        }
      }
    __syncthreads();
    if (cell && s_act[cb]) {
      const float *gp = s_g + cb * 16 + 4 * cu;
      const float ig = fast_sigmoid(gp[0]), fg = fast_sigmoid(gp[1]), gg = fast_tanh(gp[2]), og = fast_sigmoid(gp[3]);
      const float cn = fmaf(fg, s_cell[4 * PB + tid], ig * gg), hn = og * fast_tanh(cn);
      publish(g.hdec + (unsigned)((p * GS + cb) * DEC_RNN + 4 * c + cu), want, hn);
      s_cell[4 * PB + tid] = cn;
      s_cell[12 * PB + tid] = hn;
    }
    att_bulk(L4, false);
    PROF_MARK(7);
    PROF_WHEN(1);
    straggle(lag, s, 4);
    __builtin_amdgcn_sched_barrier(0);
    unsigned drop1 = 0u, drop2 = 0u;
    if (pre && act_r) {
      if (d.dropout_mode) {
#pragma unroll
        for (int k = 0; k < 4; ++k)
          drop1 |= (prenet_dropped(d.dropout_mode, d.dropout_seed, item, d.drop_masks, d.drop_steps, rb, s + 1, 0, lane + 64 * k) ? 1u : 0u) << k;
#pragma unroll
        for (int r = 0; r < 2; ++r)
          drop2 |= (prenet_dropped(d.dropout_mode, d.dropout_seed, item, d.drop_masks, d.drop_steps, rb, s + 1, 1, 16 * rk + wave + NW * r) ? 1u : 0u) << r;
      }
    }
    {
      bool need[2 * PB];
#pragma unroll
      for (int i = 0; i < 2 * PB; ++i) need[i] = act[i >> 1];
      float v[2 * PB];
      unsigned tg[2 * PB];
      lazy_wait(pre ? g.pfirst : g.lazy);
      const unsigned np_ = gather<2 * PB>(g.hdec, (unsigned)(p * GS * DEC_RNN + tid), PT, want, need, v, tg, pc);
      PROF_POLLS(3, np_);
#pragma unroll
      for (int i = 0; i < 2 * PB; ++i)
        if (need[i]) s_hdec[TID + PT * i] = v[i];
    }
    __syncthreads();
    PROF_MARK(8);
    if (prow_ok && act_r) {
      float a = 0.f;
#pragma unroll
      for (int j = 0; j < 4; ++j) a = dot4(lds4(s_pw + 4 * (j * PT + TID)), lds4(s_hdec + rb * DEC_RNN + 256 * j + L4), a);
      a = fmaf(pmp[1], wreg[rb][1], fmaf(pmp[0], wreg[rb][0], a));
      a = wave_sum(a);
      if (lane == 0) publish(g.mel + (unsigned)(((p * GS + rb) * MEL_GL + prow) * MEL_ST), want, a + s_pb[wave]);
    }
    dec_bulk_h(L4, false);
    if (attn && act_r) location(tid);
    PROF_MARK(9);
    straggle(lag, s, 5);
    __builtin_amdgcn_sched_barrier(0);
    if (pre && act_r) {
      bool nxt = false;
      if (act_r) {
        if (tid < N_MEL + 1) {
          const bool need[1] = {true};
          float v[1];
          unsigned tg[1];
          gather<1>(g.mel, (unsigned)(((p * GS + rb) * MEL_GL + tid) * MEL_ST), 0, want, need, v, tg, pc);
          s_mel[tid] = v[0];
        }
        __syncthreads();
        PROF_MARK(11);
        const float gate = s_mel[N_MEL];
        const bool fired = GATE ? gate_fires(gate, d.gate_lo, d.gate_hi, d.gate_threshold) : (d.use_gate && gate_sigmoid(gate) > d.gate_threshold);
        if (rk == 0) {
          if (tid < N_MEL) d.frames[((size_t)rb * d.max_steps + s) * N_MEL + tid] = s_mel[tid];
          if (tid == 0) {
            d.gates[(size_t)rb * d.max_steps + s] = gate;
            if (fired) d.nframes[rb] = s + 1;
          }
        }
        if (fired) nf_r = s + 1;
        nxt = s + 1 < nf_r;
      }
      float xo[2] = {0.f, 0.f};
      if (nxt) {
        const unsigned HM = (unsigned)((tid >> 8) * (N_MEL / 2));
        float acc = 0.f;
        if (ROLE_REGS) {
#pragma unroll
          for (int k = 0; k < N_MEL / 2; k += 4) {
            const float4 m = lds4(s_mel + HM + k);
            acc = fmaf(rw[ROLE_REGS ? k : 0], m.x, acc);
            acc = fmaf(rw[ROLE_REGS ? k + 1 : 0], m.y, acc);
            acc = fmaf(rw[ROLE_REGS ? k + 2 : 0], m.z, acc);
            acc = fmaf(rw[ROLE_REGS ? k + 3 : 0], m.w, acc);
          }
        } else {
#pragma unroll
          for (int k = 0; k < N_MEL / 2; k += 4) {
            const float4 w4 = lds4(s_W0 + 4u * (((HM + k) >> 2) * PRENET + (TID & 255u))), m = lds4(s_mel + HM + k);
            acc = fmaf(w4.x, m.x, acc);
            acc = fmaf(w4.y, m.y, acc);
            acc = fmaf(w4.z, m.z, acc);
            acc = fmaf(w4.w, m.w, acc);
          }
        }
        PROF_MARK(12);
        s_l1[TID] = acc;
        __syncthreads();
        PROF_MARK(13);
        float pk[4];
#pragma unroll
        for (int k = 0; k < 4; ++k) {
          const float v = fmaxf(s_l1[(L4 >> 2) + 64 * k] + s_l1[PRENET + (L4 >> 2) + 64 * k], 0.f);
          pk[k] = (drop1 >> k) & 1u ? 0.f : (d.dropout_mode ? 2.f * v : v);
        }
#pragma unroll
        for (int r = 0; r < 2; ++r) {
          float a = 0.f;
#pragma unroll
          for (int k = 0; k < 4; ++k) a = fmaf(w1r[r][k], pk[k], a);
          a = fmaxf(wave_sum(a), 0.f);
          xo[r] = (drop2 >> r) & 1u ? 0.f : (d.dropout_mode ? 2.f * a : a);
        }
      }
      PROF_MARK(14);
      if (lane < 2) s_mel[MEL_GL - 16 + wave + NW * lane] = lane ? xo[1] : xo[0];
      __syncthreads();
      if (tid < 16)
        publish(g.x + (unsigned)(((p ^ 1) * GS + rb) * PRENET + 16 * rk + tid), (want + 1u) | (nxt ? ACT_BIT : 0u),
                s_mel[MEL_GL - 16 + tid]);
    }
    PROF_MARK(10);
    }
  }
#ifdef XDTTS_PERSIST_PROFILE
  __syncthreads();
  if (g.prof && tid < 24) g.prof[c * 24 + tid] = s_prof[tid];
#endif

  if (cell) {
    d.att_c[cb * ATT_RNN + 4 * c + cu] = s_cell[tid];
    d.dec_c[cb * DEC_RNN + 4 * c + cu] = s_cell[4 * PB + tid];
    d.att_h[0][cb * ATT_RNN + 4 * c + cu] = s_cell[8 * PB + tid];
    d.dec_h[0][cb * DEC_RNN + 4 * c + cu] = s_cell[12 * PB + tid];
  }
  if (attn) {
    {
      const int col = tid & 63, q = tid >> 6;
      float acc = 0.f;
      for (int t = q; t < T; t += NW) acc = fmaf(s_aw[t], d.memory[((size_t)rb * T + t) * EMB + 64 * rk + col], acc);
      __syncthreads();
      s_part[tid] = acc;
      __syncthreads();
      if (tid < 64) {
        float v = 0.f;
#pragma unroll
        for (int u = 0; u < NW; ++u) v += s_part[u * 64 + tid];
        d.ctx[rb * EMB + 64 * rk + tid] = v;
      }
    }
    if (rk == 0 && tid < T) {
      d.aw[rb * T + tid] = s_aw[tid];
      d.awc[rb * T + tid] = s_awc[tid];
    }
  }
  if (c == 0 && tid == 0) d.ctl[0] = s;
}

__global__ void k_persist_seed(PersistBufs g, const int *limits, int B, unsigned words) {
  const int b = blockIdx.x, i = threadIdx.x;
  for (unsigned w = (unsigned)(b * PRENET + i); w < words; w += (unsigned)(B * PRENET)) g.x[w] = 0ull;
  publish(g.x + (size_t)b * PRENET + i, 1u | (limits[b] > 0 ? ACT_BIT : 0u), 0.f);
}

__global__ void k_persist_seed_at(PersistBufs g, const int *limits, const float *x, int step) {
  const int b = blockIdx.x, i = threadIdx.x;
  publish(g.x + (size_t)(((step & 1) * GS + b) * PRENET + i), (unsigned)(step + 1) | (limits[b] > step ? ACT_BIT : 0u), x[b * PRENET + i]);
}

__global__ void k_pack_ctx_rows(const float4 *__restrict__ att_w, const float4 *__restrict__ dec_w, const float4 *__restrict__ proj_w,
                                float4 *__restrict__ out) {
  const int n = blockIdx.x, q = threadIdx.x;
  float4 v = make_float4(0.f, 0.f, 0.f, 0.f);
  if (n < 4 * ATT_RNN) v = att_w[(size_t)n * (ATT_COLS / 4) + PRENET / 4 + q];
  else if (n < 4 * ATT_RNN + 4 * DEC_RNN) v = dec_w[(size_t)(n - 4 * ATT_RNN) * (DEC_COLS / 4) + ATT_RNN / 4 + q];
  else if (n <= 4 * ATT_RNN + 4 * DEC_RNN + N_MEL) v = proj_w[(size_t)(n - 4 * ATT_RNN - 4 * DEC_RNN) * (PROJ_IN / 4) + DEC_RNN / 4 + q];
  out[(size_t)n * (EMB / 4) + q] = v;
}

template <int PB, bool SKEW = false>
void launch_pb(const DecoderBufs &d, const PersistBufs &g, const PersistWeights &pw, int nsteps, hipStream_t s) {
  const void *fn = d.use_gate ? reinterpret_cast<const void *>(k_decoder_persistent<PB, SKEW, true>) : reinterpret_cast<const void *>(k_decoder_persistent<PB, SKEW, false>);
  COOP_CHECK(launch_coresident(true, fn, dim3(P_NCU), dim3(PT), 0, s, d, g, pw, nsteps));
}

}

void launch_pack_ctx_rows(const float *att_w, const float *dec_w, const float *proj_w, float *ctx_w, hipStream_t s) {
  static_assert(CTXF_ROWS >= 4 * ATT_RNN + 4 * DEC_RNN + N_MEL + 1 && CTXF_LD >= PERSIST_T_MAX, "context-fold table shape");
  hipLaunchKernelGGL(k_pack_ctx_rows, dim3(CTXF_ROWS), dim3(EMB / 4), 0, s, reinterpret_cast<const float4 *>(att_w),
                     reinterpret_cast<const float4 *>(dec_w), reinterpret_cast<const float4 *>(proj_w), reinterpret_cast<float4 *>(ctx_w));
  HIP_CHECK(hipGetLastError());
}

size_t persist_granule_words(int B) {
  (void)B;
  return (size_t)2 * GS * (PRENET + ATT_RNN + ATTN_CU * EP_LD + DEC_RNN + MEL_GL * MEL_ST);
}

PersistBufs persist_bufs(unsigned long long *base, int *err, int B) {
  PersistBufs g{};
  g.x = base;
  (void)B;
  g.hatt = g.x + (size_t)2 * GS * PRENET;
  g.ep = g.hatt + (size_t)2 * GS * ATT_RNN;
  g.hdec = g.ep + (size_t)2 * GS * ATTN_CU * EP_LD;
  g.mel = g.hdec + (size_t)2 * GS * DEC_RNN;
  g.err = err;
  g.lazy = PERSIST_LAZY_DEFAULT;
  g.xlazy = 0;
  g.clazy = 4;
  g.shrink = 0;
  g.spins = 0;
  g.fault = 0;
  g.slow = 0;
  g.pfirst = 0;
  g.xfirst = 4;
  g.efirst = 3;
  g.skew = 1;
  g.both_run = 0;
  g.first = 4;
  return g;
}

PersistBufs persist_view(const PersistBufs &g, int b0) {
  PersistBufs v = g;
  v.x += (size_t)b0 * PRENET;
  v.hatt += (size_t)b0 * ATT_RNN;
  v.ep += (size_t)b0 * ATTN_CU * EP_LD;
  v.hdec += (size_t)b0 * DEC_RNN;
  v.mel += (size_t)b0 * MEL_GL * MEL_ST;
  return v;
}

bool decoder_persistent_supported(int device, int B, int T) {
  if (B < 1 || B > PERSIST_B_MAX || T > PERSIST_T_MAX) return false;
  hipDeviceProp_t prop;
  if (hipGetDeviceProperties(&prop, device) != hipSuccess) return false;
  if (prop.multiProcessorCount < P_NCU) return false;
  int per_cu = 0;
  if (hipOccupancyMaxActiveBlocksPerMultiprocessor(&per_cu, k_decoder_persistent<PERSIST_B_MAX, false, true>, PT, 0) != hipSuccess)
    return false;
  return per_cu >= 1;
}

void launch_persist_seed(const DecoderBufs &d, const PersistBufs &g, const int *limits_dev, hipStream_t s) {
  hipLaunchKernelGGL(k_persist_seed, dim3(d.B), dim3(PRENET), 0, s, g, limits_dev, d.B, (unsigned)persist_granule_words(d.B));
  HIP_CHECK(hipGetLastError());
}

void launch_persist_seed_at(const DecoderBufs &d, const PersistBufs &g, const int *limits_dev, int step, hipStream_t s) {
  HIP_CHECK(hipMemsetAsync(g.x, 0, persist_granule_words(d.B) * sizeof(unsigned long long), s));
  hipLaunchKernelGGL(k_persist_seed_at, dim3(d.B), dim3(PRENET), 0, s, g, limits_dev, d.x, step);
  HIP_CHECK(hipGetLastError());
}

void launch_decoder_persistent(const DecoderBufs &d, const DeviceWeights &w, const PersistBufs &g, int nsteps,
                               hipStream_t s) {
  PersistWeights pw{};
  pw.att_w = reinterpret_cast<const float4 *>(w.att_w.p);
  pw.dec_w = reinterpret_cast<const float4 *>(w.dec_w.p);
  pw.q_w = reinterpret_cast<const float4 *>(w.q_w.p);
  pw.proj_w = reinterpret_cast<const float4 *>(w.proj_w.p);
  pw.att_b = w.att_b.p;
  pw.dec_b = w.dec_b.p;
  pw.v_w = w.v_w.p;
  pw.loc_fused = w.loc_fused.p;
  pw.proj_b = w.proj_b.p;
  pw.pre0T = w.pre0T.p;
  pw.pre1T = w.pre1T.p;
  switch (d.B) {
    case 1: launch_pb<1>(d, g, pw, nsteps, s); break;
    case 2:
      if (g.skew && (g.shrink || g.both_run)) launch_pb<2, true>(d, g, pw, nsteps, s);
      else launch_pb<2>(d, g, pw, nsteps, s);
      break;
    default: fail(XDTTS_ERR_BAD_ARG, "persistent decoder: %d chunks (max %d)", d.B, PERSIST_B_MAX);
  }
}

}
```

### xd-tts_amd/csrc/edge_floor.hip

```cpp
#include <hip/hip_runtime.h>
#include <cstdio>
#include <cstdlib>

namespace xdtts_edge_floor {
typedef unsigned long long u64;
constexpr int NCU = 256, NT = 512, NATT = 8, NPRE = 16, EP_LD = 128;
constexpr unsigned SPIN_LIMIT = 1u << 20;

struct Gran {
  u64 *x, *hatt, *ep, *hdec, *mel;
  int *err;
  float *sink;
};
__device__ __forceinline__ float expect(int step, int kind, int idx) { return (float)((step * 31 + kind * 7 + idx) & 1023); }
__device__ __forceinline__ void publish(u64 *slot, int step, float v) {
  __hip_atomic_store(slot, ((u64)(unsigned)(step + 1) << 32) | (u64)__float_as_uint(v), __ATOMIC_RELAXED, __HIP_MEMORY_SCOPE_AGENT);
}
template <int N>
__device__ __forceinline__ void gather(const u64 *base, int idx, int stride, int step, float (&out)[N], int *err) {
  bool done[N];
#pragma unroll
  for (int i = 0; i < N; ++i) done[i] = false;
  unsigned spins = 0;
  for (;;) {
    u64 v[N];
#pragma unroll
    for (int i = 0; i < N; ++i)
      if (!done[i]) v[i] = __hip_atomic_load(base + idx + i * stride, __ATOMIC_RELAXED, __HIP_MEMORY_SCOPE_AGENT);
    bool all = true;
#pragma unroll
    for (int i = 0; i < N; ++i)
      if (!done[i]) {
        if ((unsigned)(v[i] >> 32) == (unsigned)(step + 1)) {
          out[i] = __uint_as_float((unsigned)v[i]);
          done[i] = true;
        } else {
          all = false;
        }
      }
    if (all) return;
    if (++spins > SPIN_LIMIT || ((spins & 127u) == 0 && __hip_atomic_load(err, __ATOMIC_RELAXED, __HIP_MEMORY_SCOPE_AGENT))) {
      atomicExch(err, 1);
      return;
    }
    __builtin_amdgcn_s_sleep(1);
  }
}

struct Delays {
  int tuned, lazy, first, clazy, efirst, pfirst, xfirst, xlazy;
};
__device__ __forceinline__ void pause(int n) {
  for (int i = 0; i < n; ++i) __builtin_amdgcn_s_sleep(4);
}
__global__ __launch_bounds__(NT) void k_skeleton5(Gran g, int nsteps, int T, Delays dl) {
  const int c = blockIdx.x, tid = threadIdx.x;
  __shared__ float s_x[256], s_hatt[1024], s_hdec[1024], s_e[EP_LD], s_mel[96];
  const bool attn = c < NATT, pre = c >= NATT && c < NATT + NPRE;
  const int rk = attn ? c : c - NATT;
  float bad = 0.f;
  for (int s = 0; s < nsteps; ++s) {
    const int p = s & 1;
    if (dl.tuned) pause(pre ? dl.xfirst : dl.xlazy);
    if (tid < 256) {
      float v[1];
      gather<1>(g.x, p * 256 + tid, 0, s, v, g.err);
      bad += fabsf(v[0] - expect(s, 0, tid));
      s_x[tid] = v[0];
    }
    __syncthreads();
    if (tid < 4) publish(g.hatt + p * 1024 + 4 * c + tid, s, expect(s, 1, 4 * c + tid) + 0.f * s_x[tid]);
    if (dl.tuned) pause(attn ? dl.first : dl.lazy);
    {
      float v[2];
      gather<2>(g.hatt, p * 1024 + tid, NT, s, v, g.err);
      bad += fabsf(v[0] - expect(s, 1, tid)) + fabsf(v[1] - expect(s, 1, tid + NT));
      s_hatt[tid] = v[0];
      s_hatt[tid + NT] = v[1];
    }
    __syncthreads();
    if (attn && tid < T) publish(g.ep + (p * NATT + rk) * EP_LD + tid, s, expect(s, 2, rk * EP_LD + tid) + 0.f * s_hatt[tid]);
    if (dl.tuned) pause(attn ? dl.efirst : dl.clazy);
    {
      const int t = tid >> 2, j = tid & 3;
      float v[2] = {0.f, 0.f};
      if (t < T) {
        gather<2>(g.ep, (p * NATT + j) * EP_LD + t, 4 * EP_LD, s, v, g.err);
        bad += fabsf(v[0] - expect(s, 2, j * EP_LD + t)) + fabsf(v[1] - expect(s, 2, (j + 4) * EP_LD + t));
      }
      if (j == 0 && t < EP_LD) s_e[t] = v[0] + v[1];
    }
    __syncthreads();
    if (tid < 4) publish(g.hdec + p * 1024 + 4 * c + tid, s, expect(s, 3, 4 * c + tid) + 0.f * s_e[tid]);
    if (dl.tuned) pause(pre ? dl.pfirst : dl.lazy);
    {
      float v[2];
      gather<2>(g.hdec, p * 1024 + tid, NT, s, v, g.err);
      bad += fabsf(v[0] - expect(s, 3, tid)) + fabsf(v[1] - expect(s, 3, tid + NT));
      s_hdec[tid] = v[0];
      s_hdec[tid + NT] = v[1];
    }
    __syncthreads();
    if (pre) {
      if (tid < 6 && rk + 16 * tid < 81) publish(g.mel + p * 96 + rk + 16 * tid, s, expect(s, 4, rk + 16 * tid) + 0.f * s_hdec[tid]);
      if (tid < 81) {
        float v[1];
        gather<1>(g.mel, p * 96 + tid, 0, s, v, g.err);
        bad += fabsf(v[0] - expect(s, 4, tid));
        s_mel[tid] = v[0];
      }
      __syncthreads();
      if (tid < 16) publish(g.x + (p ^ 1) * 256 + 16 * rk + tid, s + 1, expect(s + 1, 0, 16 * rk + tid) + 0.f * s_mel[tid]);
    }
  }
  if (bad != 0.f) atomicExch(g.err, 2);
  g.sink[c * NT + tid] = bad;
}

__global__ void k_seed(Gran g) {
  publish(g.x + threadIdx.x, 0, expect(0, 0, threadIdx.x));
}


inline double measure(int device, int nsteps, int T, Delays dl, int reps, bool verbose) {
#define EF_CK(x) do { if ((x) != hipSuccess) return -1.0; } while (0)
  hipDeviceProp_t prop;
  EF_CK(hipSetDevice(device));
  EF_CK(hipGetDeviceProperties(&prop, device));
  int per_cu = 0;
  EF_CK(hipOccupancyMaxActiveBlocksPerMultiprocessor(&per_cu, k_skeleton5, NT, 0));
  if (prop.multiProcessorCount < NCU || per_cu < 1 || T < 1 || T > EP_LD || nsteps < 1) return -1.0;
  const size_t words = 2 * (256 + 1024 + NATT * EP_LD + 1024 + 96);
  u64 *buf = nullptr;
  int *err = nullptr;
  float *sink = nullptr;
  hipEvent_t e0 = nullptr, e1 = nullptr;
  hipStream_t st = nullptr;
  double best = 1e30;
  bool ok = hipStreamCreateWithFlags(&st, hipStreamNonBlocking) == hipSuccess && hipMalloc(&buf, words * 8) == hipSuccess &&
            hipMalloc(&err, 4) == hipSuccess && hipMalloc(&sink, sizeof(float) * NCU * NT) == hipSuccess &&
            hipEventCreate(&e0) == hipSuccess && hipEventCreate(&e1) == hipSuccess;
  Gran g{};
  if (ok) {
    g.x = buf;
    g.hatt = g.x + 2 * 256;
    g.ep = g.hatt + 2 * 1024;
    g.hdec = g.ep + 2 * NATT * EP_LD;
    g.mel = g.hdec + 2 * 1024;
    g.err = err;
    g.sink = sink;
  }
  for (int rep = 0; ok && rep < reps + 1; ++rep) {
    ok = hipMemsetAsync(buf, 0, words * 8, st) == hipSuccess && hipMemsetAsync(err, 0, 4, st) == hipSuccess;
    if (!ok) break;
    hipLaunchKernelGGL(k_seed, dim3(1), dim3(256), 0, st, g);
    ok = hipStreamSynchronize(st) == hipSuccess && hipEventRecord(e0, st) == hipSuccess;
    if (!ok) break;
    hipLaunchKernelGGL(k_skeleton5, dim3(NCU), dim3(NT), 0, st, g, nsteps, T, dl);
    float ms = 0;
    int herr = 0;
    ok = hipEventRecord(e1, st) == hipSuccess && hipStreamSynchronize(st) == hipSuccess && hipEventElapsedTime(&ms, e0, e1) == hipSuccess &&
         hipMemcpyAsync(&herr, err, 4, hipMemcpyDeviceToHost, st) == hipSuccess && hipStreamSynchronize(st) == hipSuccess;
    if (!ok) break;
    const double us = ms * 1e3 / nsteps;
    if (verbose)
      printf("rep %d: %d steps (T = %d), %.3f ms, %.3f us per step (5 edges: %.3f us per edge), err=%d\n", rep, nsteps, T, ms, us, us / 5, herr);
    if (herr) ok = false;
    if (rep > 0 && !herr && us < best) best = us;
  }
  if (buf) (void)hipFree(buf);
  if (err) (void)hipFree(err);
  if (sink) (void)hipFree(sink);
  if (e0) (void)hipEventDestroy(e0);
  if (e1) (void)hipEventDestroy(e1);
  if (st) (void)hipStreamDestroy(st);
#undef EF_CK
  return ok && best < 1e29 ? best : -1.0;
}
inline Delays kernel_delays(int tuned) { return Delays{tuned, 9, 4, 4, 3, 0, 4, 0}; }

}
```

### xd-tts_amd/csrc/kernels.h

```cpp
#pragma once
#include "common.h"
#include "weights.h"

namespace xdtts {

struct DecoderBufs {
  int B, T;
  const float *memory;
  const float *pmem;
  const int *n_valid;
  float *att_h[2];
  float *att_c;
  float *dec_h[2];
  float *dec_c;
  float *aw, *awc;
  float *ctx;
  float *x;
  float *loc;
  float *e_part;
  float *pmel;
  float *frames;
  float *gates;
  int *nframes;
  int *ctl;
  int max_steps;
  int use_gate;
  float gate_threshold;
  float gate_lo, gate_hi;
  int dropout_mode;
  uint32_t dropout_seed, item_base;
  const unsigned char *drop_masks;
  int drop_steps;
  float *xf, *ctxf, *att_hf[2], *dec_hf[2];
  int Bpad;
  float *awc2;
  const int *item_perm;
  const float *ctx_fold;
  const float *dec_in;
  const float *pmem_t;
  unsigned long long *ep_g;
  int *att_err;
  unsigned long long *hg;
  float *att_part;
  unsigned long long *hdg, *melg;
  float *dec_part;
  int att_spins, att_fault;
  int tail_fault;
  int att_slow;
};
constexpr int ATT_EXCHANGE_BLOCKS = 8;
void launch_dimgroup_transpose(const float *in, float *out, int B, int T, hipStream_t s);

void launch_decoder_steps(const DecoderBufs &d, const DeviceWeights &w, int nsteps, hipStream_t s);
void launch_decoder_step_at(const DecoderBufs &d, const DeviceWeights &w, int i, hipStream_t s);
void launch_decoder_advance(const DecoderBufs &d, int n, hipStream_t s);
void launch_decoder_early(const DecoderBufs &d, const DeviceWeights &w, int i, hipStream_t s);
bool decoder_two_launch(const DecoderBufs &d);
void launch_decoder_prologue(const DecoderBufs &d, const DeviceWeights &w, hipStream_t s);
void launch_decoder_location(const DecoderBufs &d, const DeviceWeights &w, hipStream_t s);
void launch_decoder_prenet(const DecoderBufs &d, const DeviceWeights &w, hipStream_t s);
void launch_frag_convert(float *rowmajor, float *frag, int B, int Bpad, int n, int dir, hipStream_t s);
void launch_decoder_flush(const DecoderBufs &d, const DeviceWeights &w, hipStream_t s);
size_t decoder_pmel_floats(int B);
void launch_decoder_init(const DecoderBufs &d, const int *limits_dev, hipStream_t s);

constexpr int CTXF_ROWS = 2 * 4096 + 128, CTXF_LD = 128;
void launch_pack_ctx_rows(const float *att_w, const float *dec_w, const float *proj_w, float *ctx_w, hipStream_t s);
constexpr int PERSIST_B_MAX = 2;
constexpr int PERSIST_T_MAX = 128;
struct PersistBufs {
  unsigned long long *x, *hatt, *ep, *hdec, *mel;
  int *err;
  int spins, fault;
  int slow;
  int skew;
  int both_run;
  int shrink;
  int first;
  int efirst;
  int xfirst;
  int pfirst;
  int xlazy, clazy;
  int lazy;
  unsigned long long *prof;
};
size_t persist_granule_words(int B);
PersistBufs persist_bufs(unsigned long long *base, int *err, int B);
PersistBufs persist_view(const PersistBufs &g, int b0);
bool decoder_persistent_supported(int device, int B, int T);
void launch_persist_seed(const DecoderBufs &d, const PersistBufs &g, const int *limits_dev, hipStream_t s);
void launch_persist_seed_at(const DecoderBufs &d, const PersistBufs &g, const int *limits_dev, int step, hipStream_t s);
void launch_decoder_persistent(const DecoderBufs &d, const DeviceWeights &w, const PersistBufs &g, int nsteps,
                               hipStream_t s);

constexpr int P8_B_MAX = 16;
constexpr int P8_STEPS_MAX = 16384;
struct P8Bufs {
  unsigned *rx, *rhatt, *rctx, *rhdec;
  unsigned long long *ep, *mel;
  int *err;
  int spins, fault;
  int delay[6];
  int ring_steps;
  unsigned long long *prof;
};
size_t p8_exchange_words(int B, int nsteps);
P8Bufs p8_bufs(unsigned long long *base, int *err, int B, int nsteps);
bool decoder_p8_supported(int device, int B, int T);
void launch_p8_seed(const DecoderBufs &d, const P8Bufs &g, const int *limits_dev, hipStream_t s);
void launch_p8_seed_at(const DecoderBufs &d, const P8Bufs &g, const int *limits_dev, int step, hipStream_t s);
void launch_decoder_p8(const DecoderBufs &d, const DeviceWeights &w, const P8Bufs &g, int nsteps, hipStream_t s);
struct P8Weights {
  const float4 *att_w, *dec_w, *q_w, *proj_w;
  const float *att_b, *dec_b, *v_w, *loc_fused, *proj_b, *pre0T, *pre1T;
};
bool decoder_p16_supported(int device, int T);
void launch_decoder_p16(const DecoderBufs &d, const P8Weights &w, const P8Bufs &g, int nsteps, hipStream_t s);

struct GemmArgs {
  const float *A;
  long lda, strideA;
  const float *W;
  const float *bias;
  float *C;
  long ldc, strideC;
  const float *R;
  long ldr, strideR;
  int M, N, K, batch;
  int ragged;
  int Mz[64];
  long Cz[64];
  int act;
  int transpose_out;
  int ldc_rows;
  float p;
  float alpha, beta;
  int r_before_act;
  int xcd_rows;
  int splitk;
  float *ws;
  unsigned *cnt;
  int tile;
};
int gemm_splitk_plan(const GemmArgs &g, size_t *ws_floats, size_t *tiles, int *tile);
constexpr int GEMM_RAGGED_MAX = 64;
void launch_gemm_nt(const GemmArgs &g, hipStream_t s);

void launch_embed(const int64_t *ids, const float *emb, float *xpad, int B, int T, int pad, hipStream_t s);
void launch_bilstm(const float *xproj, const float *whhT_fwd, const float *whhT_bwd, float *memory,
                   int B, int T, hipStream_t s);

size_t bilstm_coop_exchange_words(int B);
void launch_bilstm_coop(const float *xproj, const float *whhT_fwd, const float *whhT_bwd, float *memory,
                        unsigned long long *exchange, int *err, int B, int T, int group, hipStream_t s);

struct GlBufs {
  int F, n_fft, hop, nb;
  float *S;
  float2 *ang, *ang2;
  float2 *tprev;
  float *frames;
  float *wss_inv;
  const float2 *tw;
  const float *win;
};
constexpr int GLP_TF_MAX = 8;
struct GlSeg {
  int fbase;
  int F;
  int f0;
  int n_own;
  int first;
  int last;
  int abase;
  int pad;
};
struct GlPersist {
  const GlSeg *segs;
  unsigned long long *xch;
  int *err;
  unsigned epoch;
  int nblk, TF;
  int per_cu;
  int spins;
  int slow;
  int poll_delay;
  int gen_phase;
  unsigned seed;
  float2 *ang_out, *tprev_out;
  unsigned long long *prof;
};
bool gl_persistent_plan(int F, int n_cu, int *TF, int *nblk);
size_t gl_persistent_xch_words(int nblk);
bool gl_persistent_supported(int device, int *n_cu, int *per_cu4);
void launch_gl_persistent(const GlBufs &g, const GlPersist &p, const float2 *ang_in, const float2 *tprev_in, int n_iter,
                          float alpha, float *audio, hipStream_t s);
void launch_gl_exp_transpose(const float *mel_80xF, float *out_Fx80, int n_mels, int F, int mode, hipStream_t s);
void launch_gl_pow_rows(const float *in, int ld, float *out, int nb, int F, float p, hipStream_t s);
constexpr int GLN_PARTS = 64;
constexpr int GLN_SCRATCH = 2 * GLN_PARTS;
void launch_gl_output_normalise(float *y, const int2 *tab_dev, int n_utt, int first, int n_max, int mode, float target,
                                float *parts, hipStream_t s);
void launch_gl_phase_init(const GlBufs &g, uint32_t seed, const float *phase0_dev, hipStream_t s);
void launch_gl_phase_init_batch(const GlBufs &g, uint32_t seed, const int *frame_local, hipStream_t s);
void launch_gl_prepare(const GlBufs &g, hipStream_t s);
void launch_gl_iterations(const GlBufs &g, int n_iter, float alpha, float *audio, hipStream_t s);
const float2 *launch_gl_iterate(const GlBufs &g, int n_iter, float alpha, hipStream_t s);
void launch_gl_final(const GlBufs &g, const float2 *ang, float *audio, hipStream_t s);
void launch_gl_state_import(const GlBufs &g, const float *ang_in, const float *reb_in, hipStream_t s);
void launch_gl_state_export(const GlBufs &g, const float2 *ang, const float2 *tprev, float *ang_out, float *reb_out,
                            hipStream_t s);
void launch_transpose(const float *in, float *out, int rows, int cols, hipStream_t s);
void launch_copy_rows(const float *src, size_t src_stride, float *dst, size_t dst_stride, const int *rows, int n, int cols,
                      hipStream_t s);

}
```

### xd-tts_amd/csrc/weights.cpp

```cpp
#include "weights.h"
#include "kernels.h"

#include <cmath>
#include <fstream>

namespace xdtts {

namespace {

struct TableBuilder {
  std::vector<TensorInfo> t;
  size_t total = 0;
  void add(const std::string &name, int ndim, int d0, int d1, int d2, double fan_in, int kind,
           int rec) {
    TensorInfo ti{};
    std::snprintf(ti.name, sizeof ti.name, "%s", name.c_str());
    ti.ndim = ndim;
    ti.dims[0] = d0;
    ti.dims[1] = d1;
    ti.dims[2] = d2;
    ti.numel = (size_t)d0 * (ndim > 1 ? d1 : 1) * (ndim > 2 ? d2 : 1);
    ti.offset = total;
    ti.bound = (float)(1.0 / std::sqrt(fan_in));
    ti.kind = kind;
    ti.rec = rec;
    total += ti.numel;
    t.push_back(ti);
  }
  void conv_bn(const std::string &p, int co, int ci, int k) {
    double fan = (double)ci * k;
    add(p + ".conv.weight", 3, co, ci, k, fan, 0, 0);
    add(p + ".conv.bias", 1, co, 1, 1, fan, 0, 0);
    add(p + ".bn.weight", 1, co, 1, 1, 1, 1, 0);
    add(p + ".bn.bias", 1, co, 1, 1, 1, 2, 0);
    add(p + ".bn.running_mean", 1, co, 1, 1, 1, 3, 0);
    add(p + ".bn.running_var", 1, co, 1, 1, 1, 4, 0);
  }
  void lstm(const std::string &p, int hidden, int in, int rec) {
    add(p + ".weight_ih", 2, 4 * hidden, in, 1, hidden, 0, 0);
    add(p + ".weight_hh", 2, 4 * hidden, hidden, 1, hidden, 0, rec);
    add(p + ".bias_ih", 1, 4 * hidden, 1, 1, hidden, 0, 0);
    add(p + ".bias_hh", 1, 4 * hidden, 1, 1, hidden, 0, 0);
  }
};

TableBuilder build_table() {
  TableBuilder b;
  b.add("embedding.weight", 2, N_SYMBOLS, EMB, 1, (double)(N_SYMBOLS + EMB) / 6.0, 0, 0);
  for (int i = 0; i < ENC_CONVS; ++i)
    b.conv_bn("encoder.convolutions." + std::to_string(i), EMB, EMB, ENC_K);
  b.lstm("encoder.lstm.fwd", ENC_H, EMB, 0);
  b.lstm("encoder.lstm.bwd", ENC_H, EMB, 0);
  b.add("attention.memory_layer.weight", 2, ATT_DIM, EMB, 1, EMB, 0, 0);
  b.add("prenet.0.weight", 2, PRENET, N_MEL, 1, N_MEL, 0, 0);
  b.add("prenet.1.weight", 2, PRENET, PRENET, 1, PRENET, 0, 0);
  b.lstm("attention_rnn", ATT_RNN, ATT_IN, 1);
  b.add("attention.query_layer.weight", 2, ATT_DIM, ATT_RNN, 1, ATT_RNN, 0, 0);
  b.add("attention.v.weight", 1, ATT_DIM, 1, 1, ATT_DIM, 0, 0);
  b.add("attention.location_conv.weight", 3, LOC_F, 2, LOC_K, 2.0 * LOC_K, 0, 0);
  b.add("attention.location_dense.weight", 2, ATT_DIM, LOC_F, 1, LOC_F, 0, 0);
  b.lstm("decoder_rnn", DEC_RNN, DEC_IN, 1);
  b.add("linear_projection.weight", 2, N_MEL, PROJ_IN, 1, PROJ_IN, 0, 0);
  b.add("linear_projection.bias", 1, N_MEL, 1, 1, PROJ_IN, 0, 0);
  b.add("gate_layer.weight", 1, PROJ_IN, 1, 1, PROJ_IN, 0, 0);
  b.add("gate_layer.bias", 1, 1, 1, 1, PROJ_IN, 0, 0);
  for (int i = 0; i < POST_CONVS; ++i) {
    int ci = i == 0 ? N_MEL : POST_CH;
    int co = i == POST_CONVS - 1 ? N_MEL : POST_CH;
    b.conv_bn("postnet.convolutions." + std::to_string(i), co, ci, POST_K);
  }
  return b;
}

const TableBuilder &table() {
  static const TableBuilder b = build_table();
  return b;
}

const float *T(const std::vector<float> &blob, const std::string &name) {
  int i = tensor_index(name.c_str());
  if (i < 0) fail(XDTTS_ERR_BAD_ARG, "unknown tensor %s", name.c_str());
  return blob.data() + tensor_table()[i].offset;
}

void fold_conv(const std::vector<float> &blob, const std::string &p, int co, int ci, int k,
               ConvGemm &out, hipStream_t s) {
  const float *w = T(blob, p + ".conv.weight"), *b = T(blob, p + ".conv.bias");
  const float *g = T(blob, p + ".bn.weight"), *be = T(blob, p + ".bn.bias");
  const float *mu = T(blob, p + ".bn.running_mean"), *var = T(blob, p + ".bn.running_var");
  std::vector<float> wg((size_t)co * k * ci), bg(co);
  for (int o = 0; o < co; ++o) {
    double scale = (double)g[o] / std::sqrt((double)var[o] + 1e-5);
    for (int c = 0; c < ci; ++c)
      for (int j = 0; j < k; ++j)
        wg[((size_t)o * k + j) * ci + c] = (float)((double)w[((size_t)o * ci + c) * k + j] * scale);
    bg[o] = (float)(((double)b[o] - (double)mu[o]) * scale + (double)be[o]);
  }
  out.co = co;
  out.ci = ci;
  out.k = k;
  out.w.upload(wg.data(), wg.size(), s);
  out.b.upload(bg.data(), bg.size(), s);
  HIP_CHECK(hipStreamSynchronize(s));
}

void pack_lstm(const std::vector<float> &blob, const std::string &p, int hidden, int nin,
               DevBuf<float> &w, DevBuf<float> &b, hipStream_t s) {
  const float *wih = T(blob, p + ".weight_ih"), *whh = T(blob, p + ".weight_hh");
  const float *bih = T(blob, p + ".bias_ih"), *bhh = T(blob, p + ".bias_hh");
  const int cols = nin + hidden;
  std::vector<float> pw((size_t)hidden * 4 * cols), pb((size_t)hidden * 4);
  for (int u = 0; u < hidden; ++u)
    for (int g = 0; g < 4; ++g) {
      float *dst = pw.data() + ((size_t)u * 4 + g) * cols;
      const int r = g * hidden + u;
      std::memcpy(dst, wih + (size_t)r * nin, sizeof(float) * nin);
      std::memcpy(dst + nin, whh + (size_t)r * hidden, sizeof(float) * hidden);
      pb[(size_t)u * 4 + g] = bih[r] + bhh[r];
    }
  w.upload(pw.data(), pw.size(), s);
  b.upload(pb.data(), pb.size(), s);
  HIP_CHECK(hipStreamSynchronize(s));
}

void upload_transposed(const float *src, int rows, int cols, DevBuf<float> &dst, hipStream_t s) {
  std::vector<float> t((size_t)rows * cols);
  for (int r = 0; r < rows; ++r)
    for (int c = 0; c < cols; ++c) t[(size_t)c * rows + r] = src[(size_t)r * cols + c];
  dst.upload(t.data(), t.size(), s);
  HIP_CHECK(hipStreamSynchronize(s));
}

constexpr char MAGIC[8] = {'X', 'D', 'T', 'W', '0', '0', '0', '1'};
struct DiskEntry {
  char name[64];
  uint32_t ndim;
  uint32_t dims[3];
  uint64_t offset, numel;
};

}

const std::vector<TensorInfo> &tensor_table() { return table().t; }
size_t tensor_total() { return table().total; }
int tensor_index(const char *name) {
  const auto &t = tensor_table();
  for (size_t i = 0; i < t.size(); ++i)
    if (!std::strcmp(t[i].name, name)) return (int)i;
  return -1;
}

void synthetic_blob(uint32_t seed, float rec_scale, std::vector<float> &blob) {
  const auto &tab = tensor_table();
  blob.resize(tensor_total());
  for (size_t i = 0; i < tab.size(); ++i) {
    const TensorInfo &t = tab[i];
    float *w = blob.data() + t.offset;
    for (size_t j = 0; j < t.numel; ++j) {
      const float u = rng_uniform(seed, (uint32_t)i, (uint32_t)j);
      const float s = 2.0f * u - 1.0f;
      float v;
      switch (t.kind) {
        case 0: v = t.bound * s; break;
        case 1: v = std::fmaf(0.1f, s, 1.0f); break;
        case 2: v = 0.1f * s; break;
        case 3: v = 0.1f * s; break;
        default: v = std::fmaf(0.2f, u, 1.0f); break;
      }
      if (t.rec) v *= rec_scale;
      w[j] = v;
    }
  }
}

void save_container(const std::string &dir, const std::vector<float> &blob) {
  const auto &tab = tensor_table();
  std::ofstream f(dir + "/tacotron2.xdtw", std::ios::binary);
  if (!f) fail(XDTTS_ERR_IO, "cannot open %s/tacotron2.xdtw for writing", dir.c_str());
  uint32_t n = (uint32_t)tab.size();
  f.write(MAGIC, 8);
  f.write((const char *)&n, 4);
  for (const auto &t : tab) {
    DiskEntry e{};
    std::memcpy(e.name, t.name, sizeof e.name);
    e.ndim = (uint32_t)t.ndim;
    for (int d = 0; d < 3; ++d) e.dims[d] = (uint32_t)t.dims[d];
    e.offset = t.offset;
    e.numel = t.numel;
    f.write((const char *)&e, sizeof e);
  }
  f.write((const char *)blob.data(), (std::streamsize)(blob.size() * sizeof(float)));
  if (!f) fail(XDTTS_ERR_IO, "short write to %s/tacotron2.xdtw", dir.c_str());
}

void load_model_dir(const std::string &dir, std::vector<float> &blob) {
  if (std::ifstream(dir + "/tacotron2.xdtw", std::ios::binary)) return load_container(dir, blob);
  if (onnx_model_dir(dir)) return load_onnx_dir(dir, blob);
  fail(XDTTS_ERR_IO, "loading tacotron2 weights: %s holds neither tacotron2.xdtw nor encoder.onnx / decoder_iter.onnx / postnet.onnx "
                     "(the reference's model directory, src/tacotron2/mod.rs:246-259)", dir.c_str());
}

void load_container(const std::string &dir, std::vector<float> &blob) {
  const std::string path = dir + "/tacotron2.xdtw";
  std::ifstream f(path, std::ios::binary);
  if (!f) fail(XDTTS_ERR_IO, "loading tacotron2 weights: cannot open %s", path.c_str());
  char magic[8];
  uint32_t n = 0;
  f.read(magic, 8);
  f.read((char *)&n, 4);
  if (!f || std::memcmp(magic, MAGIC, 8) != 0 || n == 0 || n > 4096)
    fail(XDTTS_ERR_IO, "loading tacotron2 weights: %s is not an XDTW0001 container", path.c_str());
  std::vector<DiskEntry> ent(n);
  f.read((char *)ent.data(), (std::streamsize)(sizeof(DiskEntry) * n));
  if (!f) fail(XDTTS_ERR_IO, "loading tacotron2 weights: truncated header in %s", path.c_str());
  const std::streamoff data0 = f.tellg();
  const auto &tab = tensor_table();
  blob.assign(tensor_total(), 0.0f);
  std::vector<char> seen(tab.size(), 0);
  for (const auto &e : ent) {
    char nm[65];
    std::memcpy(nm, e.name, 64);
    nm[64] = 0;
    int i = tensor_index(nm);
    if (i < 0) continue;
    const TensorInfo &t = tab[i];
    bool ok = (int)e.ndim == t.ndim && e.numel == t.numel;
    for (int d = 0; d < t.ndim && ok; ++d) ok = (int)e.dims[d] == t.dims[d];
    if (!ok) fail(XDTTS_ERR_IO, "loading tacotron2 weights: tensor %s has the wrong shape", nm);
    f.seekg(data0 + (std::streamoff)(e.offset * sizeof(float)));
    f.read((char *)(blob.data() + t.offset), (std::streamsize)(t.numel * sizeof(float)));
    if (!f) fail(XDTTS_ERR_IO, "loading tacotron2 weights: tensor %s is truncated", nm);
    seen[i] = 1;
  }
  for (size_t i = 0; i < tab.size(); ++i)
    if (!seen[i]) fail(XDTTS_ERR_IO, "loading tacotron2 weights: tensor %s is missing", tab[i].name);
}

namespace {
void pack_lstm_mfma(const std::vector<float> &blob, const std::string &p, int hidden, int nin, DevBuf<float> &out,
                    hipStream_t s) {
  const float *wih = T(blob, p + ".weight_ih"), *whh = T(blob, p + ".weight_hh");
  const int cols = nin + hidden, KW = cols / MFMA_WAVES, JJ = KW / 16;
  std::vector<float> m((size_t)hidden * 4 * cols);
  auto W = [&](int unit, int gate, int c) {
    const int r = gate * hidden + unit;
    return c < nin ? wih[(size_t)r * nin + c] : whh[(size_t)r * hidden + (c - nin)];
  };
  for (int blk = 0; blk < hidden / 4; ++blk)
    for (int wv = 0; wv < MFMA_WAVES; ++wv)
      for (int jj = 0; jj < JJ; ++jj)
        for (int lane = 0; lane < 64; ++lane) {
          const int i = lane & 15, g4 = lane >> 4;
          float *dst = m.data() + ((((size_t)blk * MFMA_WAVES + wv) * JJ + jj) * 64 + lane) * 4;
          for (int c = 0; c < 4; ++c) dst[c] = W(blk * 4 + (i >> 2), i & 3, wv * KW + 16 * jj + 4 * g4 + c);
        }
  out.upload(m.data(), m.size(), s);
  HIP_CHECK(hipStreamSynchronize(s));
}
}

void DeviceWeights::ensure_batched_layout(const std::vector<float> &blob, hipStream_t s) {
  if (att_wm.p && dec_wm.p) return;
  pack_lstm_mfma(blob, "attention_rnn", ATT_RNN, ATT_IN, att_wm, s);
  pack_lstm_mfma(blob, "decoder_rnn", DEC_RNN, DEC_IN, dec_wm, s);
}

void DeviceWeights::upload(const std::vector<float> &blob, hipStream_t s) {
  if (blob.size() != tensor_total())
    fail(XDTTS_ERR_BAD_ARG, "weight blob has %zu floats, expected %zu", blob.size(), tensor_total());
  emb.upload(T(blob, "embedding.weight"), (size_t)N_SYMBOLS * EMB, s);
  for (int i = 0; i < ENC_CONVS; ++i)
    fold_conv(blob, "encoder.convolutions." + std::to_string(i), EMB, EMB, ENC_K, enc_conv[i], s);
  for (int d = 0; d < 2; ++d) {
    const std::string p = d ? "encoder.lstm.bwd" : "encoder.lstm.fwd";
    enc_wih[d].upload(T(blob, p + ".weight_ih"), (size_t)4 * ENC_H * EMB, s);
    std::vector<float> b(4 * ENC_H);
    const float *bih = T(blob, p + ".bias_ih"), *bhh = T(blob, p + ".bias_hh");
    for (int r = 0; r < 4 * ENC_H; ++r) b[r] = bih[r] + bhh[r];
    enc_bias[d].upload(b.data(), b.size(), s);
    HIP_CHECK(hipStreamSynchronize(s));
    upload_transposed(T(blob, p + ".weight_hh"), 4 * ENC_H, ENC_H, enc_whhT[d], s);
  }
  mem_w.upload(T(blob, "attention.memory_layer.weight"), (size_t)ATT_DIM * EMB, s);
  upload_transposed(T(blob, "prenet.0.weight"), PRENET, N_MEL, pre0T, s);
  upload_transposed(T(blob, "prenet.1.weight"), PRENET, PRENET, pre1T, s);
  pack_lstm(blob, "attention_rnn", ATT_RNN, ATT_IN, att_w, att_b, s);
  q_w.upload(T(blob, "attention.query_layer.weight"), (size_t)ATT_DIM * ATT_RNN, s);
  {
    const float *wq = T(blob, "attention.query_layer.weight");
    std::vector<float> q4((size_t)256 * ATT_DIM * 4);
    for (int blk = 0; blk < 256; ++blk)
      for (int a = 0; a < ATT_DIM; ++a)
        for (int i = 0; i < 4; ++i) q4[((size_t)blk * ATT_DIM + a) * 4 + i] = wq[(size_t)a * ATT_RNN + 4 * blk + i];
    q_w4.upload(q4.data(), q4.size(), s);
    HIP_CHECK(hipStreamSynchronize(s));
  }
  v_w.upload(T(blob, "attention.v.weight"), ATT_DIM, s);
  upload_transposed(T(blob, "attention.location_conv.weight"), LOC_F, 2 * LOC_K, loc_conv, s);
  upload_transposed(T(blob, "attention.location_dense.weight"), ATT_DIM, LOC_F, loc_denseT, s);
  {
    const float *cv = T(blob, "attention.location_conv.weight"), *dn = T(blob, "attention.location_dense.weight");
    std::vector<float> gf((size_t)2 * LOC_K * ATT_DIM);
    for (int ck = 0; ck < 2 * LOC_K; ++ck)
      for (int a = 0; a < ATT_DIM; ++a) {
        double acc = 0.0;
        for (int f = 0; f < LOC_F; ++f) acc += (double)dn[(size_t)a * LOC_F + f] * (double)cv[(size_t)f * 2 * LOC_K + ck];
        gf[(size_t)ck * ATT_DIM + a] = (float)acc;
      }
    loc_fused.upload(gf.data(), gf.size(), s);
    HIP_CHECK(hipStreamSynchronize(s));
  }
  pack_lstm(blob, "decoder_rnn", DEC_RNN, DEC_IN, dec_w, dec_b, s);
  {
    std::vector<float> pw((size_t)(N_MEL + 1) * PROJ_IN), pb(N_MEL + 1);
    std::memcpy(pw.data(), T(blob, "linear_projection.weight"), sizeof(float) * N_MEL * PROJ_IN);
    std::memcpy(pw.data() + (size_t)N_MEL * PROJ_IN, T(blob, "gate_layer.weight"), sizeof(float) * PROJ_IN);
    std::memcpy(pb.data(), T(blob, "linear_projection.bias"), sizeof(float) * N_MEL);
    pb[N_MEL] = T(blob, "gate_layer.bias")[0];
    proj_w.upload(pw.data(), pw.size(), s);
    std::vector<float> wh4((size_t)256 * 84 * 4, 0.f), wc((size_t)8 * (N_MEL + 1) * 64);
    for (int blk = 0; blk < 256; ++blk)
      for (int m = 0; m <= N_MEL; ++m)
        for (int i = 0; i < 4; ++i) wh4[((size_t)blk * 84 + m) * 4 + i] = pw[(size_t)m * PROJ_IN + 4 * blk + i];
    for (int cb = 0; cb < 8; ++cb)
      for (int m = 0; m <= N_MEL; ++m)
        for (int c = 0; c < 64; ++c) wc[((size_t)cb * (N_MEL + 1) + m) * 64 + c] = pw[(size_t)m * PROJ_IN + DEC_RNN + 64 * cb + c];
    proj_wh4.upload(wh4.data(), wh4.size(), s);
    proj_wc.upload(wc.data(), wc.size(), s);
    proj_b.upload(pb.data(), pb.size(), s);
    HIP_CHECK(hipStreamSynchronize(s));
  }
  ctx_w.alloc((size_t)CTXF_ROWS * EMB);
  launch_pack_ctx_rows(att_w.p, dec_w.p, proj_w.p, ctx_w.p, s);
  for (int i = 0; i < POST_CONVS; ++i) {
    int ci = i == 0 ? N_MEL : POST_CH;
    int co = i == POST_CONVS - 1 ? N_MEL : POST_CH;
    fold_conv(blob, "postnet.convolutions." + std::to_string(i), co, ci, POST_K, post_conv[i], s);
  }
  HIP_CHECK(hipStreamSynchronize(s));
}

}
```

### xd-tts_amd/csrc/weights.h

```cpp
#pragma once
#include "common.h"

namespace xdtts {

struct TensorInfo {
  char name[64];
  int ndim;
  int dims[3];
  size_t numel, offset;
  float bound;
  int kind;
  int rec;
};

const std::vector<TensorInfo> &tensor_table();
size_t tensor_total();
int tensor_index(const char *name);

void synthetic_blob(uint32_t seed, float rec_scale, std::vector<float> &blob);
void load_container(const std::string &dir, std::vector<float> &blob);
bool onnx_model_dir(const std::string &dir);
void load_onnx_dir(const std::string &dir, std::vector<float> &blob);
std::string describe_onnx_dir(const std::string &dir);
void load_model_dir(const std::string &dir, std::vector<float> &blob);
void save_container(const std::string &dir, const std::vector<float> &blob);

struct ConvGemm {
  DevBuf<float> w, b;
  int co = 0, ci = 0, k = 0;
};

#ifndef XDTTS_MFMA_WAVES
#define XDTTS_MFMA_WAVES 8
#endif
constexpr int MFMA_WAVES = XDTTS_MFMA_WAVES;
#ifndef XDTTS_BATCH_MFMA_MIN
#define XDTTS_BATCH_MFMA_MIN 5
#endif
constexpr int BATCH_MFMA_MIN = XDTTS_BATCH_MFMA_MIN;

struct DeviceWeights {
  DevBuf<float> emb;
  ConvGemm enc_conv[ENC_CONVS];
  DevBuf<float> enc_wih[2], enc_bias[2];
  DevBuf<float> enc_whhT[2];
  DevBuf<float> mem_w;
  DevBuf<float> pre0T, pre1T;
  DevBuf<float> att_w, att_b;
  DevBuf<float> q_w, v_w, loc_conv, loc_denseT;
  DevBuf<float> loc_fused;
  DevBuf<float> dec_w, dec_b;
  DevBuf<float> proj_w, proj_b;
  DevBuf<float> ctx_w;
  DevBuf<float> q_w4;
  DevBuf<float> proj_wh4;
  DevBuf<float> proj_wc;
  ConvGemm post_conv[POST_CONVS];
  DevBuf<float> att_wm, dec_wm;
  void upload(const std::vector<float> &blob, hipStream_t s);
  void ensure_batched_layout(const std::vector<float> &blob, hipStream_t s);
};

}
```

Before: 130,000.

## Fold prenet layer-1 into the linear projection to skip mel gather

```diff
diff --git a/include/xdtts.h b/include/xdtts.h
--- a/include/xdtts.h
+++ b/include/xdtts.h
@@ -62,6 +62,7 @@
 size_t xdtts_tensor_offset(int32_t i);
 size_t xdtts_tensor_total(void);
 xdtts_status xdtts_tacotron2_get_tensor(const xdtts_tacotron2 *h, int32_t i, float *out);
+xdtts_status xdtts_prenet_fold_table(const float *blob, size_t n_floats, float *c, float *c0);
 
 xdtts_status xdtts_tacotron2_infer_ids(xdtts_tacotron2 *h, const int64_t *ids, size_t n,
                                        const size_t *splits, size_t n_splits,
diff --git a/xd-tts_amd/__init__.py b/xd-tts_amd/__init__.py
--- a/xd-tts_amd/__init__.py
+++ b/xd-tts_amd/__init__.py
@@ -58,6 +58,7 @@
     "xdtts_tensor_offset": (_SZ, [_I32]),
     "xdtts_tensor_total": (_SZ, []),
     "xdtts_tacotron2_get_tensor": (_I32, [_VP, _I32, _VP]),
+    "xdtts_prenet_fold_table": (_I32, [_VP, _SZ, _VP, _VP]),
     "xdtts_tacotron2_infer_ids": (_I32, [_VP, _VP, _SZ, _VP, _SZ, C.POINTER(InferOpts), C.POINTER(_PF), C.POINTER(_SZ)]),
     "xdtts_tacotron2_infer_batch": (_I32, [_VP, _VP, _VP, _I32, _I32, C.POINTER(InferOpts), _VP, C.POINTER(_PF), C.POINTER(_SZ)]),
     "xdtts_tacotron2_encoder": (_I32, [_VP, _VP, _I32, _VP, _VP]),
@@ -170,6 +171,13 @@
     return o
 
 
+def prenet_fold_table(blob):
+    b = np.ascontiguousarray(blob, dtype=np.float32)
+    c, c0 = np.empty((256, 1536), dtype=np.float32), np.empty(256, dtype=np.float32)
+    _check(lib.xdtts_prenet_fold_table(_ptr(b), b.size, _ptr(c), _ptr(c0)))
+    return c, c0
+
+
 def device_count():
     return lib.xdtts_device_count()
 
diff --git a/xd-tts_amd/csrc/api_tacotron2.cpp b/xd-tts_amd/csrc/api_tacotron2.cpp
--- a/xd-tts_amd/csrc/api_tacotron2.cpp
+++ b/xd-tts_amd/csrc/api_tacotron2.cpp
@@ -133,6 +133,17 @@
     if (!h || !out || i < 0 || i >= xdtts_tensor_count()) fail(XDTTS_ERR_BAD_ARG, "bad tensor request");
     const TensorInfo &t = tensor_table()[i];
     std::memcpy(out, h->blob.data() + t.offset, t.numel * sizeof(float));
+  });
+}
+
+xdtts_status xdtts_prenet_fold_table(const float *blob, size_t n_floats, float *c, float *c0) {
+  return guard([&] {
+    if (!blob || !c || !c0) fail(XDTTS_ERR_BAD_ARG, "null argument");
+    if (n_floats != tensor_total()) fail(XDTTS_ERR_BAD_ARG, "blob has %zu floats, expected %zu", n_floats, tensor_total());
+    std::vector<float> vc, vc0;
+    prenet_fold_table(std::vector<float>(blob, blob + n_floats), vc, vc0);
+    std::memcpy(c, vc.data(), vc.size() * sizeof(float));
+    std::memcpy(c0, vc0.data(), vc0.size() * sizeof(float));
   });
 }
 
diff --git a/xd-tts_amd/csrc/decoder_persistent.hip b/xd-tts_amd/csrc/decoder_persistent.hip
--- a/xd-tts_amd/csrc/decoder_persistent.hip
+++ b/xd-tts_amd/csrc/decoder_persistent.hip
@@ -14,11 +14,8 @@
 constexpr int P_NCU = ATT_RNN / 4;
 constexpr int TP = PERSIST_T_MAX;
 constexpr int ATTN_CU = 8, PRE_CU = 16;
-constexpr int EP_LD = TP, MEL_GL = 96;
-#ifndef XDTTS_MEL_ST
-#define XDTTS_MEL_ST 1
-#endif
-constexpr int MEL_ST = XDTTS_MEL_ST;
+constexpr int EP_LD = TP;
+constexpr int L1_GL = PRENET + 16;
 constexpr int GS = PERSIST_B_MAX;
 constexpr unsigned P_SPIN_LIMIT = 1u << 21;
 constexpr unsigned ACT_BIT = 0x80000000u;
@@ -112,7 +109,7 @@
 constexpr int persist_lds_floats(int pb) {
   const int common = pb * (PRENET + TP + ATT_RNN + DEC_RNN + 16) + 8 + 32 + 16 * pb;
   const int attn = 2 * TP * 16 + 2 * TP + 16 + NW * 64 + 2 * WPAD + 62 * 16 + 64 + 16 + 8 * PT * 4;
-  const int pre = N_MEL * PRENET + MEL_GL + 2 * PRENET + 8 + 6 * PT * 4;
+  const int pre = 8 * PT * 4 + L1_GL + 16 + 16 + 16 + 8 + 6 * PT * 4;
   return common + (attn > pre ? attn : pre);
 }
 
@@ -141,8 +138,8 @@
 #endif
 
 struct PersistWeights {
-  const float4 *att_w, *dec_w, *q_w, *proj_w;
-  const float *att_b, *dec_b, *v_w, *loc_fused, *proj_b, *pre0T, *pre1T;
+  const float4 *att_w, *dec_w, *q_w, *proj_w, *c_w;
+  const float *att_b, *dec_b, *v_w, *loc_fused, *proj_b, *c_b, *pre1T;
 };
 
 template <int PB, bool SKEW = false, bool GATE = false>
@@ -173,10 +170,12 @@
   float *s_cown = s_G + 62 * 16;
   float *s_vv = s_cown + 64;
   float *s_qw = s_vv + 16;
-  float *s_W0 = role;
-  float *s_mel = s_W0 + N_MEL * PRENET;
-  float *s_l1 = s_mel + MEL_GL;
-  float *s_pb = s_l1 + 2 * PRENET;
+  float *s_cw = role;
+  float *s_l1 = s_cw + 8 * PT * 4;
+  float *s_l1o = s_l1 + L1_GL;
+  float *s_xo = s_l1o + 16;
+  float *s_cb = s_xo + 16;
+  float *s_pb = s_cb + 16;
   float *s_pw = s_pb + 8;
 
   float4 wa[2][ATT_COLS / 256], wd[2][DEC_COLS / 256];
@@ -197,6 +196,7 @@
   const int rk = attn ? c % ATTN_CU : (c - ATTN_CU * PB) % PRE_CU;
   const int prow = rk + 16 * wave;
   const bool prow_ok = pre && wave < 6 && prow <= N_MEL;
+  constexpr bool ROLE_REGS = PB == 1;
 
   const int step0 = d.ctl[0];
   if (GATE && PB == 1 && !(step0 < d.nframes[0])) return;
@@ -247,7 +247,14 @@
         *reinterpret_cast<float4 *>(s_qw + 4 * ((4 * r + j) * PT + tid)) = w.q_w[(unsigned)((16 * rk + wave + NW * r) * (ATT_RNN / 4) + lane + 64 * j)];
   }
   if (pre) {
-    for (int i = tid; i < N_MEL * PRENET; i += PT) s_W0[(((i / PRENET) >> 2) * PRENET + i % PRENET) * 4 + ((i / PRENET) & 3)] = w.pre0T[i];
+    if (!ROLE_REGS) {
+#pragma unroll
+      for (int r = 0; r < 2; ++r)
+#pragma unroll
+        for (int j = 0; j < 4; ++j)
+          *reinterpret_cast<float4 *>(s_cw + 4 * ((4 * r + j) * PT + tid)) = w.c_w[(unsigned)((16 * rk + wave + NW * r) * (PROJ_IN / 4) + lane + 64 * j)];
+    }
+    if (tid < 16) s_cb[tid] = w.c_b[16 * rk + tid];
     if (prow_ok) {
       if (lane == 0) s_pb[wave] = w.proj_b[prow];
 #pragma unroll
@@ -256,25 +263,22 @@
     }
     nf_r = d.nframes[rb];
   }
-  constexpr bool ROLE_REGS = PB == 1;
-  float rw[ROLE_REGS ? 40 : 1];
+  float rw[ROLE_REGS ? 32 : 1];
   if (ROLE_REGS) {
 #pragma unroll
-    for (int k = 0; k < 40; ++k) rw[ROLE_REGS ? k : 0] = 0.f;
-    if (attn) {
+    for (int k = 0; k < 32; ++k) rw[ROLE_REGS ? k : 0] = 0.f;
+    if (attn || pre) {
 #pragma unroll
       for (int r = 0; r < 2; ++r)
 #pragma unroll
         for (int j = 0; j < 4; ++j) {
-          const float4 q = w.q_w[(unsigned)((16 * rk + wave + NW * r) * (ATT_RNN / 4) + lane + 64 * j)];
+          const float4 q = attn ? w.q_w[(unsigned)((16 * rk + wave + NW * r) * (ATT_RNN / 4) + lane + 64 * j)]
+                                : w.c_w[(unsigned)((16 * rk + wave + NW * r) * (PROJ_IN / 4) + lane + 64 * j)];
           rw[ROLE_REGS ? 16 * r + 4 * j + 0 : 0] = q.x;
           rw[ROLE_REGS ? 16 * r + 4 * j + 1 : 0] = q.y;
           rw[ROLE_REGS ? 16 * r + 4 * j + 2 : 0] = q.z;
           rw[ROLE_REGS ? 16 * r + 4 * j + 3 : 0] = q.w;
         }
-    } else if (pre) {
-#pragma unroll
-      for (int k = 0; k < N_MEL / 2; ++k) rw[ROLE_REGS ? k : 0] = w.pre0T[(unsigned)(((tid >> 8) * (N_MEL / 2) + k) * PRENET + (tid & 255))];
     }
   }
   float w1r[2][4];
@@ -285,7 +289,7 @@
   const uint32_t item = d.item_base + (uint32_t)rb;
   __syncthreads();
 
-  float pma[PB][2][2], pmd[PB][2][2], pmp[2] = {0.f, 0.f};
+  float pma[PB][2][2], pmd[PB][2][2], pmp[2] = {0.f, 0.f}, pmc[2][2] = {{0.f, 0.f}, {0.f, 0.f}};
   if (d.ctx_fold) {
 #pragma unroll
     for (int b = 0; b < PB; ++b)
@@ -300,6 +304,10 @@
           pmd[b][r][h] = t < T ? F[(size_t)(4 * ATT_RNN + row) * CTXF_LD] : 0.f;
         }
         if (prow_ok && b == rb) pmp[h] = t < T ? F[(size_t)(4 * ATT_RNN + 4 * DEC_RNN + prow) * CTXF_LD] : 0.f;
+        if (pre && b == rb) {
+#pragma unroll
+          for (int r = 0; r < 2; ++r) pmc[r][h] = t < T ? F[(size_t)(CTXF_L1 + 16 * rk + wave + NW * r) * CTXF_LD] : 0.f;
+        }
       }
   } else {
     float4 pw4 = make_float4(0.f, 0.f, 0.f, 0.f), pw5 = pw4;
@@ -307,12 +315,20 @@
       pw4 = lds4(s_pw + 4 * (4 * PT + tid));
       pw5 = lds4(s_pw + 4 * (5 * PT + tid));
     }
+    float4 cw4[2] = {pw4, pw4}, cw5[2] = {pw4, pw4};
+    if (pre) {
+#pragma unroll
+      for (int r = 0; r < 2; ++r) {
+        cw4[r] = w.c_w[(unsigned)((16 * rk + wave + NW * r) * (PROJ_IN / 4) + DEC_RNN / 4 + lane)];
+        cw5[r] = w.c_w[(unsigned)((16 * rk + wave + NW * r) * (PROJ_IN / 4) + DEC_RNN / 4 + 64 + lane)];
+      }
+    }
 #pragma unroll
     for (int b = 0; b < PB; ++b) {
       const float4 *m4 = reinterpret_cast<const float4 *>(d.memory + (size_t)b * T * EMB);
 #pragma unroll
       for (int h = 0; h < 2; ++h) {
-        float ra[2] = {0.f, 0.f}, rd[2] = {0.f, 0.f}, rp = 0.f;
+        float ra[2] = {0.f, 0.f}, rd[2] = {0.f, 0.f}, rp = 0.f, rc[2] = {0.f, 0.f};
         for (int tt = 0; tt < 64 && tt + 64 * h < T; ++tt) {
           const int t = tt + 64 * h;
           const float4 m0 = m4[(size_t)t * (EMB / 4) + lane], m1 = m4[(size_t)t * (EMB / 4) + 64 + lane];
@@ -328,6 +344,11 @@
           if (pre && b == rb) {
             const float vp = wave_sum(dot4(pw5, m1, dot4(pw4, m0, 0.f)));
             if (lane == tt) rp = vp;
+#pragma unroll
+            for (int r = 0; r < 2; ++r) {
+              const float vc = wave_sum(dot4(cw5[r], m1, dot4(cw4[r], m0, 0.f)));
+              if (lane == tt) rc[r] = vc;
+            }
           }
         }
 #pragma unroll
@@ -335,7 +356,11 @@
           pma[b][r][h] = ra[r];
           pmd[b][r][h] = rd[r];
         }
-        if (pre && b == rb) pmp[h] = rp;
+        if (pre && b == rb) {
+          pmp[h] = rp;
+          pmc[0][h] = rc[0];
+          pmc[1][h] = rc[1];
+        }
       }
     }
   }
@@ -411,6 +436,92 @@
   u64 prof_last = wall_clock64();
   __syncthreads();
 #endif
+  auto project = [&](int b, int s, int tid, float w0, float w1, bool marks) {
+    const int lane = tid & 63, wave = tid >> 6, prow = rk + 16 * wave;
+    const unsigned L4 = 4u * (unsigned)lane, TID = (unsigned)tid, want = (unsigned)(s + 1);
+    const float *hd = s_hdec + b * DEC_RNN;
+    u64 *l1 = g.l1 + (unsigned)(((s & 1) * GS + b) * L1_GL);
+    {
+      float a0 = 0.f, a1 = 0.f;
+#pragma unroll
+      for (int j = 0; j < 4; ++j) {
+        const float4 v = lds4(hd + 256 * j + L4);
+        if (ROLE_REGS) {
+          a0 = dot4(make_float4(rw[ROLE_REGS ? 4 * j : 0], rw[ROLE_REGS ? 4 * j + 1 : 0], rw[ROLE_REGS ? 4 * j + 2 : 0], rw[ROLE_REGS ? 4 * j + 3 : 0]), v, a0);
+          a1 = dot4(make_float4(rw[ROLE_REGS ? 16 + 4 * j : 0], rw[ROLE_REGS ? 17 + 4 * j : 0], rw[ROLE_REGS ? 18 + 4 * j : 0], rw[ROLE_REGS ? 19 + 4 * j : 0]), v, a1);
+        } else {
+          a0 = dot4(lds4(s_cw + 4 * (j * PT + TID)), v, a0);
+          a1 = dot4(lds4(s_cw + 4 * ((4 + j) * PT + TID)), v, a1);
+        }
+      }
+      a0 = wave_sum(fmaf(pmc[0][1], w1, fmaf(pmc[0][0], w0, a0)));
+      a1 = wave_sum(fmaf(pmc[1][1], w1, fmaf(pmc[1][0], w0, a1)));
+      if (lane == 0) {
+        s_l1o[wave] = a0 + s_cb[wave];
+        s_l1o[wave + NW] = a1 + s_cb[wave + NW];
+      }
+    }
+    __syncthreads();
+    if (tid < 16) publish(l1 + (unsigned)(16 * rk + tid), want, s_l1o[tid]);
+    if (marks) PROF_MARK(12);
+    if (wave < 6 && prow <= N_MEL) {
+      float a = 0.f;
+#pragma unroll
+      for (int j = 0; j < 4; ++j) a = dot4(lds4(s_pw + 4 * (j * PT + TID)), lds4(hd + 256 * j + L4), a);
+      a = wave_sum(fmaf(pmp[1], w1, fmaf(pmp[0], w0, a)));
+      if (lane == 0) {
+        a += s_pb[wave];
+        if (prow < N_MEL) {
+          d.frames[((size_t)b * d.max_steps + s) * N_MEL + prow] = a;
+        } else {
+          d.gates[(size_t)b * d.max_steps + s] = a;
+          publish(l1 + PRENET, want, a);
+        }
+      }
+    }
+    if (marks) PROF_MARK(13);
+  };
+  auto prenet = [&](auto PF, const u64 *pf, int b, int s, int tid, unsigned drop1, unsigned drop2, int mark, bool marks) {
+    const int lane = tid & 63, wave = tid >> 6, p = s & 1;
+    const unsigned want = (unsigned)(s + 1);
+    if (tid < PRENET + 1) {
+      const bool need[1] = {tid < PRENET || GATE || d.use_gate};
+      float v[1];
+      unsigned tg[1];
+      gather<1, decltype(PF)::value>(g.l1, (unsigned)((p * GS + b) * L1_GL + tid), 0, want, need, v, tg, pc, pf);
+      s_l1[tid] = v[0];
+    }
+    __syncthreads();
+    PROF_MARK(mark);
+    const float gate = s_l1[PRENET];
+    const bool fired = GATE ? gate_fires(gate, d.gate_lo, d.gate_hi, d.gate_threshold) : (d.use_gate && gate_sigmoid(gate) > d.gate_threshold);
+    if (fired) {
+      nf_r = s + 1;
+      if (rk == 0 && tid == 0) d.nframes[b] = s + 1;
+    }
+    const bool more = s + 1 < nf_r;
+    float xo[2] = {0.f, 0.f};
+    if (more) {
+      float pk[4];
+#pragma unroll
+      for (int k = 0; k < 4; ++k) {
+        const float v = fmaxf(s_l1[lane + 64 * k], 0.f);
+        pk[k] = (drop1 >> k) & 1u ? 0.f : (d.dropout_mode ? 2.f * v : v);
+      }
+#pragma unroll
+      for (int r = 0; r < 2; ++r) {
+        float a = 0.f;
+#pragma unroll
+        for (int k = 0; k < 4; ++k) a = fmaf(w1r[r][k], pk[k], a);
+        a = fmaxf(wave_sum(a), 0.f);
+        xo[r] = (drop2 >> r) & 1u ? 0.f : (d.dropout_mode ? 2.f * a : a);
+      }
+    }
+    if (marks) PROF_MARK(14);
+    if (lane < 2) s_xo[wave + NW * lane] = lane ? xo[1] : xo[0];
+    __syncthreads();
+    if (tid < 16) publish(g.x + (unsigned)(((p ^ 1) * GS + b) * PRENET + 16 * rk + tid), (want + 1u) | (more ? ACT_BIT : 0u), s_xo[tid]);
+  };
   int s = step0;
   const int s_stop = step0 + nsteps;
   if constexpr (SKEW) {
@@ -437,10 +548,10 @@
       pf[0] = t < T ? peek(g.ep + (unsigned)((((s & 1) * GS + b) * ATTN_CU + j) * EP_LD + t)) : 0ull;
       pf[1] = t < T ? peek(g.ep + (unsigned)((((s & 1) * GS + b) * ATTN_CU + j + 4) * EP_LD + t)) : 0ull;
     };
-    auto issue_mel = [&](auto B, int s) {
+    auto issue_l1 = [&](auto B, int s) {
       constexpr int b = decltype(B)::value;
       const int tid = tid_k + (int)opaque(0u);
-      pf[0] = (pre && rb == b && tid < N_MEL + 1) ? peek(g.mel + (unsigned)((((s & 1) * GS + b) * MEL_GL + tid) * MEL_ST)) : 0ull;
+      pf[0] = (pre && rb == b && tid < PRENET + 1) ? peek(g.l1 + (unsigned)(((s & 1) * GS + b) * L1_GL + tid)) : 0ull;
       pf[1] = 0ull;
     };
     auto I0 = std::integral_constant<int, 0>{};
@@ -648,8 +759,6 @@
       const int p = s & 1;
       const unsigned want = (unsigned)(s + 1);
       const bool mine = pre && rb == b;
-      const int prow = rk + 16 * wave;
-      const bool prow_ok = mine && wave < 6 && prow <= N_MEL;
       if (mine) {
         drop1 = 0u;
         drop2 = 0u;
@@ -671,14 +780,7 @@
         s_hdec[b * DEC_RNN + TID + PT] = v[1];
       }
       __syncthreads();
-      if (prow_ok) {
-        float a = 0.f;
-#pragma unroll
-        for (int j = 0; j < 4; ++j) a = dot4(lds4(s_pw + 4 * (j * PT + TID)), lds4(s_hdec + b * DEC_RNN + 256 * j + L4), a);
-        a = fmaf(pmp[1], wreg[b][1], fmaf(pmp[0], wreg[b][0], a));
-        a = wave_sum(a);
-        if (lane == 0) publish(g.mel + (unsigned)(((p * GS + b) * MEL_GL + prow) * MEL_ST), want, a + s_pb[wave]);
-      }
+      if (mine) project(b, s, tid, wreg[b][0], wreg[b][1], false);
       dec_bulk_h1(B, L4);
       nxt();
       if (attn && rb == b) location(tid);
@@ -693,64 +795,8 @@
         return;
       }
       PROF_MARK(10 + 3 * b);
-      const int tid = tid_k + (int)opaque(0u), lane = tid & 63, wave = tid >> 6;
-      const unsigned L4 = 4u * (unsigned)lane, TID = (unsigned)tid;
-      const int p = s & 1;
-      const unsigned want = (unsigned)(s + 1);
-      if (tid < N_MEL + 1) {
-        const bool need[1] = {true};
-        float v[1];
-        unsigned tg[1];
-        gather<1, true>(g.mel, (unsigned)(((p * GS + b) * MEL_GL + tid) * MEL_ST), 0, want, need, v, tg, pc, pf);
-        s_mel[tid] = v[0];
-      }
-      __syncthreads();
-      PROF_MARK(11 + 3 * b);
-      const float gate = s_mel[N_MEL];
-      const bool fired = GATE ? gate_fires(gate, d.gate_lo, d.gate_hi, d.gate_threshold) : (d.use_gate && gate_sigmoid(gate) > d.gate_threshold);
-      if (rk == 0) {
-        if (tid < N_MEL) d.frames[((size_t)b * d.max_steps + s) * N_MEL + tid] = s_mel[tid];
-        if (tid == 0) {
-          d.gates[(size_t)b * d.max_steps + s] = gate;
-          if (fired) d.nframes[b] = s + 1;
-        }
-      }
-      if (fired) nf_r = s + 1;
-      const bool more = s + 1 < nf_r;
-      float xo[2] = {0.f, 0.f};
-      if (more) {
-        const unsigned HM = (unsigned)((tid >> 8) * (N_MEL / 2));
-        float acc = 0.f;
-#pragma unroll
-        for (int k = 0; k < N_MEL / 2; k += 4) {
-          const float4 w4 = lds4(s_W0 + 4u * (((HM + k) >> 2) * PRENET + (TID & 255u))), m = lds4(s_mel + HM + k);
-          acc = fmaf(w4.x, m.x, acc);
-          acc = fmaf(w4.y, m.y, acc);
-          acc = fmaf(w4.z, m.z, acc);
-          acc = fmaf(w4.w, m.w, acc);
-        }
-        s_l1[TID] = acc;
-        __syncthreads();
-        float pk[4];
-#pragma unroll
-        for (int k = 0; k < 4; ++k) {
-          const float v = fmaxf(s_l1[(L4 >> 2) + 64 * k] + s_l1[PRENET + (L4 >> 2) + 64 * k], 0.f);
-          pk[k] = (drop1 >> k) & 1u ? 0.f : (d.dropout_mode ? 2.f * v : v);
-        }
-#pragma unroll
-        for (int r = 0; r < 2; ++r) {
-          float a = 0.f;
-#pragma unroll
-          for (int k = 0; k < 4; ++k) a = fmaf(w1r[r][k], pk[k], a);
-          a = fmaxf(wave_sum(a), 0.f);
-          xo[r] = (drop2 >> r) & 1u ? 0.f : (d.dropout_mode ? 2.f * a : a);
-        }
-      }
-      if (lane < 2) s_mel[MEL_GL - 16 + wave + NW * lane] = lane ? xo[1] : xo[0];
-      __syncthreads();
-      if (tid < 16)
-        publish(g.x + (unsigned)(((p ^ 1) * GS + b) * PRENET + 16 * rk + tid), (want + 1u) | (more ? ACT_BIT : 0u),
-                s_mel[MEL_GL - 16 + tid]);
+      const int tid = tid_k + (int)opaque(0u);
+      prenet(std::true_type{}, pf, b, s, tid, drop1, drop2, 11 + 3 * b, false);
       nxt();
       PROF_MARK(5 * b + 4);
     };
@@ -761,7 +807,7 @@
         bool a0 = s < s_stop;
         if (a0) a0 = ph1(I0, s, [&] { if (tail1) issue_h(g.hdec, I1, s - 1); else issue_h(g.hatt, I0, s); });
         if (tail1) ph4(I1, s - 1, [&] { if (a0) issue_h(g.hatt, I0, s); });
-        if (a0) ph2(I0, s, [&] { if (tail1) issue_mel(I1, s - 1); else issue_ep(I0, s); });
+        if (a0) ph2(I0, s, [&] { if (tail1) issue_l1(I1, s - 1); else issue_ep(I0, s); });
         if (tail1) {
           ph5(I1, s - 1, [&] { if (a0) issue_ep(I0, s); });
           tail1 = false;
@@ -770,8 +816,8 @@
         ph3(I0, s, [&] { issue_x(I1, s); });
         const bool a1 = ph1(I1, s, [&] { issue_h(g.hdec, I0, s); });
         if (!a1) issue_h(g.hdec, I0, s);
-        ph4(I0, s, [&] { if (a1) issue_h(g.hatt, I1, s); else issue_mel(I0, s); });
-        if (a1) ph2(I1, s, [&] { issue_mel(I0, s); });
+        ph4(I0, s, [&] { if (a1) issue_h(g.hatt, I1, s); else issue_l1(I0, s); });
+        if (a1) ph2(I1, s, [&] { issue_l1(I0, s); });
         ph5(I0, s, [&] { if (a1) issue_ep(I1, s); });
         if (!a1) {
           ++s;
@@ -789,8 +835,6 @@
     const unsigned L4 = 4u * (unsigned)lane, TID = (unsigned)tid;
     const int cb = tid >> 2, cu = tid & 3;
     const bool cell = tid < 4 * PB;
-    const int prow = rk + 16 * wave;
-    const bool prow_ok = pre && wave < 6 && prow <= N_MEL;
     const int p = s & 1;
     const unsigned want = (unsigned)(s + 1);
     const bool lag = g.slow && c == g.slow - 1;
@@ -1010,92 +1054,14 @@
     }
     __syncthreads();
     PROF_MARK(8);
-    if (prow_ok && act_r) {
-      float a = 0.f;
-#pragma unroll
-      for (int j = 0; j < 4; ++j) a = dot4(lds4(s_pw + 4 * (j * PT + TID)), lds4(s_hdec + rb * DEC_RNN + 256 * j + L4), a);
-      a = fmaf(pmp[1], wreg[rb][1], fmaf(pmp[0], wreg[rb][0], a));
-      a = wave_sum(a);
-      if (lane == 0) publish(g.mel + (unsigned)(((p * GS + rb) * MEL_GL + prow) * MEL_ST), want, a + s_pb[wave]);
-    }
+    if (pre && act_r) project(rb, s, tid, wreg[rb][0], wreg[rb][1], true);
     dec_bulk_h(L4, false);
     if (attn && act_r) location(tid);
     PROF_MARK(9);
     straggle(lag, s, 5);
     __builtin_amdgcn_sched_barrier(0);
-    if (pre && act_r) {
-      bool nxt = false;
-      if (act_r) {
-        if (tid < N_MEL + 1) {
-          const bool need[1] = {true};
-          float v[1];
-          unsigned tg[1];
-          gather<1>(g.mel, (unsigned)(((p * GS + rb) * MEL_GL + tid) * MEL_ST), 0, want, need, v, tg, pc);
-          s_mel[tid] = v[0];
-        }
-        __syncthreads();
-        PROF_MARK(11);
-        const float gate = s_mel[N_MEL];
-        const bool fired = GATE ? gate_fires(gate, d.gate_lo, d.gate_hi, d.gate_threshold) : (d.use_gate && gate_sigmoid(gate) > d.gate_threshold);
-        if (rk == 0) {
-          if (tid < N_MEL) d.frames[((size_t)rb * d.max_steps + s) * N_MEL + tid] = s_mel[tid];
-          if (tid == 0) {
-            d.gates[(size_t)rb * d.max_steps + s] = gate;
-            if (fired) d.nframes[rb] = s + 1;
-          }
-        }
-        if (fired) nf_r = s + 1;
-        nxt = s + 1 < nf_r;
-      }
-      float xo[2] = {0.f, 0.f};
-      if (nxt) {
-        const unsigned HM = (unsigned)((tid >> 8) * (N_MEL / 2));
-        float acc = 0.f;
-        if (ROLE_REGS) {
-#pragma unroll
-          for (int k = 0; k < N_MEL / 2; k += 4) {
-            const float4 m = lds4(s_mel + HM + k);
-            acc = fmaf(rw[ROLE_REGS ? k : 0], m.x, acc);
-            acc = fmaf(rw[ROLE_REGS ? k + 1 : 0], m.y, acc);
-            acc = fmaf(rw[ROLE_REGS ? k + 2 : 0], m.z, acc);
-            acc = fmaf(rw[ROLE_REGS ? k + 3 : 0], m.w, acc);
-          }
-        } else {
-#pragma unroll
-          for (int k = 0; k < N_MEL / 2; k += 4) {
-            const float4 w4 = lds4(s_W0 + 4u * (((HM + k) >> 2) * PRENET + (TID & 255u))), m = lds4(s_mel + HM + k);
-            acc = fmaf(w4.x, m.x, acc);
-            acc = fmaf(w4.y, m.y, acc);
-            acc = fmaf(w4.z, m.z, acc);
-            acc = fmaf(w4.w, m.w, acc);
-          }
-        }
-        PROF_MARK(12);
-        s_l1[TID] = acc;
-        __syncthreads();
-        PROF_MARK(13);
-        float pk[4];
-#pragma unroll
-        for (int k = 0; k < 4; ++k) {
-          const float v = fmaxf(s_l1[(L4 >> 2) + 64 * k] + s_l1[PRENET + (L4 >> 2) + 64 * k], 0.f);
-          pk[k] = (drop1 >> k) & 1u ? 0.f : (d.dropout_mode ? 2.f * v : v);
-        }
-#pragma unroll
-        for (int r = 0; r < 2; ++r) {
-          float a = 0.f;
-#pragma unroll
-          for (int k = 0; k < 4; ++k) a = fmaf(w1r[r][k], pk[k], a);
-          a = fmaxf(wave_sum(a), 0.f);
-          xo[r] = (drop2 >> r) & 1u ? 0.f : (d.dropout_mode ? 2.f * a : a);
-        }
-      }
-      PROF_MARK(14);
-      if (lane < 2) s_mel[MEL_GL - 16 + wave + NW * lane] = lane ? xo[1] : xo[0];
-      __syncthreads();
-      if (tid < 16)
-        publish(g.x + (unsigned)(((p ^ 1) * GS + rb) * PRENET + 16 * rk + tid), (want + 1u) | (nxt ? ACT_BIT : 0u),
-                s_mel[MEL_GL - 16 + tid]);
-    }
+    if (pre && act_r)
+      prenet(std::false_type{}, nullptr, rb, s, tid, drop1, drop2, 11, true);
     PROF_MARK(10);
     }
   }
@@ -1145,12 +1111,13 @@
 }
 
 __global__ void k_pack_ctx_rows(const float4 *__restrict__ att_w, const float4 *__restrict__ dec_w, const float4 *__restrict__ proj_w,
-                                float4 *__restrict__ out) {
+                                const float4 *__restrict__ c_w, float4 *__restrict__ out) {
   const int n = blockIdx.x, q = threadIdx.x;
   float4 v = make_float4(0.f, 0.f, 0.f, 0.f);
   if (n < 4 * ATT_RNN) v = att_w[(size_t)n * (ATT_COLS / 4) + PRENET / 4 + q];
   else if (n < 4 * ATT_RNN + 4 * DEC_RNN) v = dec_w[(size_t)(n - 4 * ATT_RNN) * (DEC_COLS / 4) + ATT_RNN / 4 + q];
   else if (n <= 4 * ATT_RNN + 4 * DEC_RNN + N_MEL) v = proj_w[(size_t)(n - 4 * ATT_RNN - 4 * DEC_RNN) * (PROJ_IN / 4) + DEC_RNN / 4 + q];
+  else if (n >= CTXF_L1) v = c_w[(size_t)(n - CTXF_L1) * (PROJ_IN / 4) + DEC_RNN / 4 + q];
   out[(size_t)n * (EMB / 4) + q] = v;
 }
 
@@ -1162,16 +1129,17 @@
 
 }
 
-void launch_pack_ctx_rows(const float *att_w, const float *dec_w, const float *proj_w, float *ctx_w, hipStream_t s) {
-  static_assert(CTXF_ROWS >= 4 * ATT_RNN + 4 * DEC_RNN + N_MEL + 1 && CTXF_LD >= PERSIST_T_MAX, "context-fold table shape");
+void launch_pack_ctx_rows(const float *att_w, const float *dec_w, const float *proj_w, const float *pre0_proj_w, float *ctx_w, hipStream_t s) {
+  static_assert(CTXF_L1 >= 4 * ATT_RNN + 4 * DEC_RNN + N_MEL + 1 && CTXF_ROWS == CTXF_L1 + PRENET && CTXF_LD >= PERSIST_T_MAX, "context-fold table shape");
   hipLaunchKernelGGL(k_pack_ctx_rows, dim3(CTXF_ROWS), dim3(EMB / 4), 0, s, reinterpret_cast<const float4 *>(att_w),
-                     reinterpret_cast<const float4 *>(dec_w), reinterpret_cast<const float4 *>(proj_w), reinterpret_cast<float4 *>(ctx_w));
+                     reinterpret_cast<const float4 *>(dec_w), reinterpret_cast<const float4 *>(proj_w), reinterpret_cast<const float4 *>(pre0_proj_w),
+                     reinterpret_cast<float4 *>(ctx_w));
   HIP_CHECK(hipGetLastError());
 }
 
 size_t persist_granule_words(int B) {
   (void)B;
-  return (size_t)2 * GS * (PRENET + ATT_RNN + ATTN_CU * EP_LD + DEC_RNN + MEL_GL * MEL_ST);
+  return (size_t)2 * GS * (PRENET + ATT_RNN + ATTN_CU * EP_LD + DEC_RNN + L1_GL);
 }
 
 PersistBufs persist_bufs(unsigned long long *base, int *err, int B) {
@@ -1181,7 +1149,7 @@
   g.hatt = g.x + (size_t)2 * GS * PRENET;
   g.ep = g.hatt + (size_t)2 * GS * ATT_RNN;
   g.hdec = g.ep + (size_t)2 * GS * ATTN_CU * EP_LD;
-  g.mel = g.hdec + (size_t)2 * GS * DEC_RNN;
+  g.l1 = g.hdec + (size_t)2 * GS * DEC_RNN;
   g.err = err;
   g.lazy = PERSIST_LAZY_DEFAULT;
   g.xlazy = 0;
@@ -1205,7 +1173,7 @@
   v.hatt += (size_t)b0 * ATT_RNN;
   v.ep += (size_t)b0 * ATTN_CU * EP_LD;
   v.hdec += (size_t)b0 * DEC_RNN;
-  v.mel += (size_t)b0 * MEL_GL * MEL_ST;
+  v.l1 += (size_t)b0 * L1_GL;
   return v;
 }
 
@@ -1243,7 +1211,8 @@
   pw.v_w = w.v_w.p;
   pw.loc_fused = w.loc_fused.p;
   pw.proj_b = w.proj_b.p;
-  pw.pre0T = w.pre0T.p;
+  pw.c_w = reinterpret_cast<const float4 *>(w.pre0_proj_w.p);
+  pw.c_b = w.pre0_proj_b.p;
   pw.pre1T = w.pre1T.p;
   switch (d.B) {
     case 1: launch_pb<1>(d, g, pw, nsteps, s); break;
diff --git a/xd-tts_amd/csrc/edge_floor.hip b/xd-tts_amd/csrc/edge_floor.hip
--- a/xd-tts_amd/csrc/edge_floor.hip
+++ b/xd-tts_amd/csrc/edge_floor.hip
@@ -4,11 +4,11 @@
 
 namespace xdtts_edge_floor {
 typedef unsigned long long u64;
-constexpr int NCU = 256, NT = 512, NATT = 8, NPRE = 16, EP_LD = 128;
+constexpr int NCU = 256, NT = 512, NATT = 8, NPRE = 16, EP_LD = 128, L1_GL = 272;
 constexpr unsigned SPIN_LIMIT = 1u << 20;
 
 struct Gran {
-  u64 *x, *hatt, *ep, *hdec, *mel;
+  u64 *x, *hatt, *ep, *hdec, *l1;
   int *err;
   float *sink;
 };
@@ -55,7 +55,7 @@
 }
 __global__ __launch_bounds__(NT) void k_skeleton5(Gran g, int nsteps, int T, Delays dl) {
   const int c = blockIdx.x, tid = threadIdx.x;
-  __shared__ float s_x[256], s_hatt[1024], s_hdec[1024], s_e[EP_LD], s_mel[96];
+  __shared__ float s_x[256], s_hatt[1024], s_hdec[1024], s_e[EP_LD], s_l1[L1_GL];
   const bool attn = c < NATT, pre = c >= NATT && c < NATT + NPRE;
   const int rk = attn ? c : c - NATT;
   float bad = 0.f;
@@ -102,15 +102,16 @@
     }
     __syncthreads();
     if (pre) {
-      if (tid < 6 && rk + 16 * tid < 81) publish(g.mel + p * 96 + rk + 16 * tid, s, expect(s, 4, rk + 16 * tid) + 0.f * s_hdec[tid]);
-      if (tid < 81) {
+      if (tid < 16) publish(g.l1 + p * L1_GL + 16 * rk + tid, s, expect(s, 4, 16 * rk + tid) + 0.f * s_hdec[tid]);
+      if (rk == 0 && tid == 320) publish(g.l1 + p * L1_GL + 256, s, expect(s, 4, 256) + 0.f * s_hdec[tid]);
+      if (tid < 257) {
         float v[1];
-        gather<1>(g.mel, p * 96 + tid, 0, s, v, g.err);
+        gather<1>(g.l1, p * L1_GL + tid, 0, s, v, g.err);
         bad += fabsf(v[0] - expect(s, 4, tid));
-        s_mel[tid] = v[0];
+        s_l1[tid] = v[0];
       }
       __syncthreads();
-      if (tid < 16) publish(g.x + (p ^ 1) * 256 + 16 * rk + tid, s + 1, expect(s + 1, 0, 16 * rk + tid) + 0.f * s_mel[tid]);
+      if (tid < 16) publish(g.x + (p ^ 1) * 256 + 16 * rk + tid, s + 1, expect(s + 1, 0, 16 * rk + tid) + 0.f * s_l1[tid]);
     }
   }
   if (bad != 0.f) atomicExch(g.err, 2);
@@ -130,7 +131,7 @@
   int per_cu = 0;
   EF_CK(hipOccupancyMaxActiveBlocksPerMultiprocessor(&per_cu, k_skeleton5, NT, 0));
   if (prop.multiProcessorCount < NCU || per_cu < 1 || T < 1 || T > EP_LD || nsteps < 1) return -1.0;
-  const size_t words = 2 * (256 + 1024 + NATT * EP_LD + 1024 + 96);
+  const size_t words = 2 * (256 + 1024 + NATT * EP_LD + 1024 + L1_GL);
   u64 *buf = nullptr;
   int *err = nullptr;
   float *sink = nullptr;
@@ -146,7 +147,7 @@
     g.hatt = g.x + 2 * 256;
     g.ep = g.hatt + 2 * 1024;
     g.hdec = g.ep + 2 * NATT * EP_LD;
-    g.mel = g.hdec + 2 * 1024;
+    g.l1 = g.hdec + 2 * 1024;
     g.err = err;
     g.sink = sink;
   }
diff --git a/xd-tts_amd/csrc/kernels.h b/xd-tts_amd/csrc/kernels.h
--- a/xd-tts_amd/csrc/kernels.h
+++ b/xd-tts_amd/csrc/kernels.h
@@ -64,12 +64,13 @@
 size_t decoder_pmel_floats(int B);
 void launch_decoder_init(const DecoderBufs &d, const int *limits_dev, hipStream_t s);
 
-constexpr int CTXF_ROWS = 2 * 4096 + 128, CTXF_LD = 128;
-void launch_pack_ctx_rows(const float *att_w, const float *dec_w, const float *proj_w, float *ctx_w, hipStream_t s);
+constexpr int CTXF_L1 = 2 * 4096 + 128;
+constexpr int CTXF_ROWS = CTXF_L1 + 256, CTXF_LD = 128;
+void launch_pack_ctx_rows(const float *att_w, const float *dec_w, const float *proj_w, const float *pre0_proj_w, float *ctx_w, hipStream_t s);
 constexpr int PERSIST_B_MAX = 2;
 constexpr int PERSIST_T_MAX = 128;
 struct PersistBufs {
-  unsigned long long *x, *hatt, *ep, *hdec, *mel;
+  unsigned long long *x, *hatt, *ep, *hdec, *l1;
   int *err;
   int spins, fault;
   int slow;
diff --git a/xd-tts_amd/csrc/weights.cpp b/xd-tts_amd/csrc/weights.cpp
--- a/xd-tts_amd/csrc/weights.cpp
+++ b/xd-tts_amd/csrc/weights.cpp
@@ -1,6 +1,7 @@
 #include "weights.h"
 #include "kernels.h"
 
+#include <algorithm>
 #include <cmath>
 #include <fstream>
 
@@ -265,6 +266,25 @@
   pack_lstm_mfma(blob, "decoder_rnn", DEC_RNN, DEC_IN, dec_wm, s);
 }
 
+void prenet_fold_table(const std::vector<float> &blob, std::vector<float> &c, std::vector<float> &c0) {
+  const float *w1 = T(blob, "prenet.0.weight"), *wp = T(blob, "linear_projection.weight"), *bp = T(blob, "linear_projection.bias");
+  c.resize((size_t)PRENET * PROJ_IN);
+  c0.resize(PRENET);
+  std::vector<double> acc(PROJ_IN);
+  for (int o = 0; o < PRENET; ++o) {
+    std::fill(acc.begin(), acc.end(), 0.0);
+    double b = 0.0;
+    for (int m = 0; m < N_MEL; ++m) {
+      const double a = (double)w1[(size_t)o * N_MEL + m];
+      const float *row = wp + (size_t)m * PROJ_IN;
+      for (int k = 0; k < PROJ_IN; ++k) acc[k] += a * (double)row[k];
+      b += a * (double)bp[m];
+    }
+    for (int k = 0; k < PROJ_IN; ++k) c[(size_t)o * PROJ_IN + k] = (float)acc[k];
+    c0[o] = (float)b;
+  }
+}
+
 void DeviceWeights::upload(const std::vector<float> &blob, hipStream_t s) {
   if (blob.size() != tensor_total())
     fail(XDTTS_ERR_BAD_ARG, "weight blob has %zu floats, expected %zu", blob.size(), tensor_total());
@@ -330,8 +350,15 @@
     proj_b.upload(pb.data(), pb.size(), s);
     HIP_CHECK(hipStreamSynchronize(s));
   }
+  {
+    std::vector<float> c, c0;
+    prenet_fold_table(blob, c, c0);
+    pre0_proj_w.upload(c.data(), c.size(), s);
+    pre0_proj_b.upload(c0.data(), c0.size(), s);
+    HIP_CHECK(hipStreamSynchronize(s));
+  }
   ctx_w.alloc((size_t)CTXF_ROWS * EMB);
-  launch_pack_ctx_rows(att_w.p, dec_w.p, proj_w.p, ctx_w.p, s);
+  launch_pack_ctx_rows(att_w.p, dec_w.p, proj_w.p, pre0_proj_w.p, ctx_w.p, s);
   for (int i = 0; i < POST_CONVS; ++i) {
     int ci = i == 0 ? N_MEL : POST_CH;
     int co = i == POST_CONVS - 1 ? N_MEL : POST_CH;
diff --git a/xd-tts_amd/csrc/weights.h b/xd-tts_amd/csrc/weights.h
--- a/xd-tts_amd/csrc/weights.h
+++ b/xd-tts_amd/csrc/weights.h
@@ -24,6 +24,7 @@
 std::string describe_onnx_dir(const std::string &dir);
 void load_model_dir(const std::string &dir, std::vector<float> &blob);
 void save_container(const std::string &dir, const std::vector<float> &blob);
+void prenet_fold_table(const std::vector<float> &blob, std::vector<float> &c, std::vector<float> &c0);
 
 struct ConvGemm {
   DevBuf<float> w, b;
@@ -51,6 +52,7 @@
   DevBuf<float> loc_fused;
   DevBuf<float> dec_w, dec_b;
   DevBuf<float> proj_w, proj_b;
+  DevBuf<float> pre0_proj_w, pre0_proj_b;
   DevBuf<float> ctx_w;
   DevBuf<float> q_w4;
   DevBuf<float> proj_wh4;
```

After: 130,900 (median of 6 runs). No clear change (+0.7%).
